# avabag01-ai/spectrogram-midi

Measured on AMD Instinct MI355X. Metric: audio-seconds transcribed/sec (44.1 kHz, n_fft=2048), higher is better.
Workload: dtype f64

## Files before the change

include/aegis_hip.h:

```cpp
#ifndef AEGIS_HIP_H
#define AEGIS_HIP_H

#include <stdint.h>

#ifdef __cplusplus
extern "C" {
#endif

#define AEGIS_ABI_VERSION 2

#define AEGIS_OK 0
#define AEGIS_ERR_INVALID (-22)
#define AEGIS_ERR_NOMEM (-12)
#define AEGIS_ERR_DEVICE (-5)
#define AEGIS_ERR_UNSUPPORTED (-95)

#define AEGIS_STAGE_MEL 0x1
#define AEGIS_STAGE_RAKE 0x2
#define AEGIS_STAGE_PYIN 0x4
#define AEGIS_STAGE_RMS 0x8
#define AEGIS_STAGE_ALL 0xF
#define AEGIS_OPT_CHECK_FINITE 0x10
#define AEGIS_OPT_F0_ZERO 0x20

// ... 101 lines not shown
                             aegis_stream_commit *commit);

#define AEGIS_TREND_SMA 1
#define AEGIS_TREND_EMA 2
#define AEGIS_TREND_BOLLINGER 3
#define AEGIS_TREND_ARTICULATION 4
#define AEGIS_TREND_MACD 5
#define AEGIS_TREND_SLIDES 6
#define AEGIS_TREND_RSI 7
#define AEGIS_TREND_SAVGOL 8
#define AEGIS_TREND_KALMAN 9
#define AEGIS_TREND_HOLT 10
#define AEGIS_TREND_CONSENSUS 11
#define AEGIS_TREND_PITCH_ANALYSIS 12
int aegis_trend(aegis_handle *h, int32_t op, const double *x, const int64_t *offsets, int32_t n_series,
                const double *params, int32_t n_params, void *const *outs, int32_t n_outs);

int aegis_ghost_rsi(aegis_handle *h, const int64_t *ev_a, const int64_t *ev_b, const int64_t *event_off, int32_t n_series,
                    const int64_t *track_len, int32_t period, double *avg_gain, double *avg_loss);

typedef struct aegis_event {
    int32_t clip, note, start, end, velocity;
    uint8_t track;
    uint8_t technique;
    uint8_t reserved0, reserved1;
    float rms_energy;
    int32_t reserved2;
    double confidence, slope;
} aegis_event;
typedef struct aegis_event_params {
    int32_t sample_rate, hop_length;
    double confidence_threshold;
    double sustain_ms, min_note_duration_ms;
} aegis_event_params;
typedef struct aegis_run_fit {
    int32_t clip, start, end;
    int32_t technique;
    double slope;
} aegis_run_fit;
typedef struct aegis_event_batch {
    int32_t n_clips;
    int32_t reserved;
    const int64_t *frame_off;
    const uint8_t *sounding;
    const double *semitones;
    const int16_t *pitch_bin;
    const double *bin_semitones;
    const float *rms_db;
    const double *probs;
    const aegis_run_fit *fits;
    int64_t n_fits;
} aegis_event_batch;
int64_t aegis_extract_events(const aegis_event_params *params, const aegis_event_batch *batch, aegis_event *events, int64_t cap,
                             int64_t *clip_event_off, aegis_run_fit *risky_runs, int64_t risky_cap, int64_t *n_risky);
int64_t aegis_render_smf(int32_t sample_rate, int32_t hop_length, int32_t midi_program, double vibrato_rate,
                         double vibrato_depth, int32_t n_clips, const aegis_event *events, const int64_t *clip_event_off,
                         uint8_t *out, int64_t cap, int64_t *clip_byte_off);
const char *aegis_events_last_error(void);

#define AEGIS_WAVE_SINE 0
#define AEGIS_WAVE_SAWTOOTH 1
#define AEGIS_WAVE_SQUARE 2
#define AEGIS_WAVE_TRIANGLE 3
typedef struct aegis_synth_note {
    double start, duration;
    int32_t note, velocity;
} aegis_synth_note;
typedef struct aegis_adsr_params {
    double attack_ms, decay_ms, sustain_level, release_ms;
    int32_t waveform;
    int32_t reserved;
} aegis_adsr_params;
int64_t aegis_synth_parse_smf(aegis_handle *h, const uint8_t *smf, int64_t n_bytes, aegis_synth_note *notes, int64_t cap,
                              double *length_seconds);
int64_t aegis_synth_samples_for(int32_t sample_rate, double length_seconds, const aegis_adsr_params *params);
int aegis_synth_adsr(aegis_handle *h, int32_t sample_rate, int32_t n_clips, const aegis_synth_note *notes, const int64_t *note_off,
                     const double *length_seconds, const aegis_adsr_params *params, int16_t *const *out, const int64_t *out_cap);

typedef struct aegis_synth_wheel {
    double time;
    int32_t track, value;
} aegis_synth_wheel;
int64_t aegis_synth_parse_smf_wheel(aegis_handle *h, const uint8_t *smf, int64_t n_bytes, aegis_synth_note *notes, int32_t *note_track,
                                    int64_t cap, aegis_synth_wheel *wheel, int64_t wheel_cap, int64_t *n_wheel, double *length_seconds);
int aegis_synth_adsr_bend(aegis_handle *h, int32_t sample_rate, int32_t n_clips, const aegis_synth_note *notes, const int64_t *note_off,
                          const double *length_seconds, const aegis_adsr_params *params, const int32_t *note_track,
                          const aegis_synth_wheel *wheel, const int64_t *wheel_off, const double *bend_range, int16_t *const *out,
                          const int64_t *out_cap);

typedef struct aegis_fit_note {
    int32_t clip, note;
    int64_t lo, hi;
    int32_t velocity, reserved;
    double duration;
} aegis_fit_note;
int aegis_note_fit(aegis_handle *h, int32_t sample_rate, int32_t n_clips, const float *const *audio, const int64_t *n_samples,
                   int32_t n_notes, const aegis_fit_note *notes, const aegis_adsr_params *cands, const int64_t *cand_off,
                   double *score, double *env, double *centroid, double *zcr, int32_t *best);
int aegis_compare_audio(aegis_handle *h, int32_t sample_rate, int32_t n_pairs, const double *const *orig, const int64_t *n_orig,
                        const double *const *synth, const int64_t *n_synth, double *out);
int64_t aegis_synth_one_note(aegis_handle *h, int32_t sample_rate, double freq, double duration, int32_t velocity,
                         const aegis_adsr_params *params, double *out, int64_t cap);
int64_t aegis_synth_notes_samples_for(int32_t sample_rate, double length_seconds, const aegis_adsr_params *params, int64_t n_notes);
int aegis_synth_adsr_notes(aegis_handle *h, int32_t sample_rate, int32_t n_clips, const aegis_synth_note *notes, const int64_t *note_off,
                           const double *length_seconds, const aegis_adsr_params *params, int16_t *const *out, const int64_t *out_cap);

typedef struct aegis_verify_event {
    int32_t clip, reserved;
    int64_t lo, hi;
} aegis_verify_event;
int aegis_verify_techniques(aegis_handle *h, int32_t sample_rate, int32_t n_clips, const float *const *audio,
                            const int64_t *n_samples, int32_t n_events, const aegis_verify_event *events,
                            const aegis_synth_note *notes, const int64_t *note_off, const double *length_seconds,
                            const aegis_adsr_params *params, const int32_t *note_track, const aegis_synth_wheel *wheel,
                            const int64_t *wheel_off, const double *bend_range,
                            double *sim , uint8_t *keep );

typedef struct aegis_salience_params {
    int32_t n_harm;
    double harmonics[8], weights[8];
    int32_t filter_peaks;
    float peak_floor;
    int32_t bin_lo, bin_hi, top_k;
} aegis_salience_params;
int aegis_salience(aegis_handle *h, const float *mag, const int64_t *n_frames, int32_t n_clips, int32_t n_bins, int32_t bins_per_octave,
                   const aegis_salience_params *p, float *sal_out , int32_t *cand_bin, float *cand_sal, float *cand_shift);
int aegis_cqt_salience(aegis_handle *h, const float *const *pcm, const int64_t *n_samples, int32_t n_clips, int32_t n_bins,
                       int32_t bins_per_octave, double fmin, double filter_scale, const aegis_salience_params *p,
                       float *mag_out , float *sal_out , int32_t *cand_bin, float *cand_sal, float *cand_shift);

#define AEGIS_PCM_F64 6
#define AEGIS_FX_DISTORTION 1
#define AEGIS_FX_REVERB     2
#define AEGIS_FX_DELAY      3
#define AEGIS_FX_CHORUS     4
typedef struct aegis_effect { int32_t kind; int32_t n_ir; double p0, p1; const double *ir; } aegis_effect;
int64_t aegis_reverb_ir(double room_size, int32_t sample_rate, double *dst, int64_t cap);
int aegis_effects(aegis_handle *h, int32_t sample_rate, int32_t n_clips, const void *const *in, int32_t in_format,
                  const int64_t *n_samples, const aegis_effect *fx, const int64_t *fx_off,
                  double *const *out_f64, int16_t *const *out_i16);


int64_t aegis_get_table(const aegis_handle *h, const char *name, void *dst, int64_t cap);

int aegis_set_table(aegis_handle *h, const char *name, const double *data, int64_t count);

int64_t aegis_get_param(const aegis_handle *h, const char *name);

int64_t aegis_debug_fetch(aegis_handle *h, const char *name, void *dst, int64_t cap);

int aegis_debug_rake_columns(aegis_handle *h, const float *mel_power, int64_t n_rows, int32_t n_mels, float clip_max,
                             double ratio, int32_t from_power, uint8_t *flags_out);

int aegis_debug_set_observations(aegis_handle *h, const double *logobs, const double *logunv, int64_t F);

int aegis_debug_set_difference(aegis_handle *h, const double *d, int64_t F);

#define AEGIS_PLAN_DEVICE 0
#define AEGIS_PLAN_CALLER_STREAM 1
#define AEGIS_PLAN_HOST_FED 2
#define AEGIS_PLAN_COOLING 4
#define AEGIS_PLAN_NO_PERSIST 8
#define AEGIS_PLAN_F_SPLIT 1
#define AEGIS_PLAN_F_SPLIT_AUTO 2
#define AEGIS_PLAN_F_WANT_HYBRID 4
#define AEGIS_PLAN_F_HYBRID 8
#define AEGIS_PLAN_F_HYBRID_PART 16
#define AEGIS_PLAN_F_BALANCED 32
#define AEGIS_PLAN_F_MAY_PERSIST 64
#define AEGIS_PLAN_F_PERSISTENT 128
#define AEGIS_PLAN_F_DENSE 256
#define AEGIS_PLAN_F_PROPORTIONAL 512
#define AEGIS_PLAN_F_TWO_FRAME_STREAMS 1024
#define AEGIS_PLAN_F_FRAME_B 2048
int64_t aegis_debug_plan(aegis_handle *h, const int64_t *n_samples, int32_t n_clips, int32_t entry, int32_t sync,
                         int32_t n_cus, int64_t *dst, int64_t cap);

int aegis_set_profiling(aegis_handle *h, int32_t on);
double aegis_last_kernel_ms(const aegis_handle *h, const char *name);
int aegis_last_kernel_launches(const aegis_handle *h, const char *name);

#ifdef __cplusplus
}
#endif
#endif
```

spectrogram-midi_amd/_abi.py:

```python
import ctypes as C
import os

import numpy as np

_HERE = os.path.dirname(os.path.abspath(__file__))
LIB_PATH = os.environ.get("AEGIS_HIP_LIB", os.path.join(_HERE, "libaegis_hip.so"))

STAGE_MEL, STAGE_RAKE, STAGE_PYIN, STAGE_RMS, STAGE_ALL = 0x1, 0x2, 0x4, 0x8, 0xF
OPT_CHECK_FINITE, OPT_F0_ZERO = 0x10, 0x20
(TREND_SMA, TREND_EMA, TREND_BOLLINGER, TREND_ARTICULATION, TREND_MACD, TREND_SLIDES, TREND_RSI, TREND_SAVGOL,
 TREND_KALMAN, TREND_HOLT, TREND_CONSENSUS, TREND_PITCH_ANALYSIS) = range(1, 13)
OK, ERR_INVALID, ERR_NOMEM, ERR_DEVICE, ERR_UNSUPPORTED = 0, -22, -12, -5, -95
PYIN_INIT_UNVOICED, PYIN_INIT_UNIFORM = 0, 1
ABI_VERSION = 2
PCM_S16, PCM_F64 = 2, 6
FX_DISTORTION, FX_REVERB, FX_DELAY, FX_CHORUS = 1, 2, 3, 4
EFFECT_KINDS = {"distortion": (FX_DISTORTION, (("drive", 0.5),)), "reverb": (FX_REVERB, (("room_size", 0.5),)),
                "delay": (FX_DELAY, (("delay_ms", 300), ("feedback", 0.3))), "chorus": (FX_CHORUS, (("depth", 0.003), ("rate", 1.5)))}
WAVEFORMS = {"sine": 0, "sawtooth": 1, "square": 2, "triangle": 3}
SYNTH_NOTE_DTYPE = np.dtype([("start", "<f8"), ("duration", "<f8"), ("note", "<i4"), ("velocity", "<i4")])
SYNTH_WHEEL_DTYPE = np.dtype([("time", "<f8"), ("track", "<i4"), ("value", "<i4")])

_P, _S, _I32, _I64, _U32, _F32, _F64 = C.c_void_p, C.c_char_p, C.c_int32, C.c_int64, C.c_uint32, C.c_float, C.c_double
_PP, _PI64 = C.POINTER(_P), C.POINTER(_I64)


class Config(C.Structure):
    _fields_ = [("sample_rate", _I32), ("hop_length", _I32), ("n_fft", _I32), ("n_mels", _I32), ("fmin", _F64), ("fmax", _F64),
                ("device", _I32), ("pyin_init", _I32), ("max_frames_per_pass", _I64)]


class Outputs(C.Structure):
    _fields_ = [("f0", _P), ("voiced_flag", _P), ("voiced_prob", _P), ("rms", _P), ("rake_mask", _P), ("S_dB", _P), ("pitch_bin", _P),
                ("sdb_col_means", _P)]


class PcmClip(C.Structure):
    _fields_ = [("data", _P), ("n_frames", _I64), ("format", _I32), ("channels", _I32), ("sample_rate", _I32), ("n_taps", _I32),
                ("taps", _P)]


class StreamFrames(C.Structure):
    _fields_ = [("rms", _P), ("voiced_prob", _P), ("live_state", _P)]


class StreamCommit(C.Structure):
    _fields_ = [("pitch_bin", _P), ("cap", _I64), ("first", _I64), ("count", _I64), ("frontier", _I64), ("walked", _I64),
                ("walked_wide", _I64)]


class Event(C.Structure):
    _fields_ = [("clip", _I32), ("note", _I32), ("start", _I32), ("end", _I32), ("velocity", _I32),
                ("track", C.c_uint8), ("technique", C.c_uint8), ("reserved0", C.c_uint8), ("reserved1", C.c_uint8),
                ("rms_energy", _F32), ("reserved2", _I32), ("confidence", _F64), ("slope", _F64)]


class EventParams(C.Structure):
    _fields_ = [("sample_rate", _I32), ("hop_length", _I32), ("confidence_threshold", _F64), ("sustain_ms", _F64),
                ("min_note_duration_ms", _F64)]


class RunFit(C.Structure):
    _fields_ = [("clip", _I32), ("start", _I32), ("end", _I32), ("technique", _I32), ("slope", _F64)]


class EventBatch(C.Structure):
    _fields_ = [("n_clips", _I32), ("reserved", _I32), ("frame_off", _P), ("sounding", _P), ("semitones", _P), ("pitch_bin", _P),
                ("bin_semitones", _P), ("rms_db", _P), ("probs", _P), ("fits", _P), ("n_fits", _I64)]


class SynthNote(C.Structure):
    _fields_ = [("start", _F64), ("duration", _F64), ("note", _I32), ("velocity", _I32)]


class AdsrParams(C.Structure):
    _fields_ = [("attack_ms", _F64), ("decay_ms", _F64), ("sustain_level", _F64), ("release_ms", _F64), ("waveform", _I32),
                ("reserved", _I32)]


class FitNote(C.Structure):
    _fields_ = [("clip", _I32), ("note", _I32), ("lo", _I64), ("hi", _I64), ("velocity", _I32), ("reserved", _I32), ("duration", _F64)]


class VerifyEvent(C.Structure):
    _fields_ = [("clip", _I32), ("reserved", _I32), ("lo", _I64), ("hi", _I64)]


class SalienceParams(C.Structure):
    _fields_ = [("n_harm", _I32), ("harmonics", _F64 * 8), ("weights", _F64 * 8), ("filter_peaks", _I32), ("peak_floor", _F32),
                ("bin_lo", _I32), ("bin_hi", _I32), ("top_k", _I32)]


class Effect(C.Structure):
    _fields_ = [("kind", _I32), ("n_ir", _I32), ("p0", _F64), ("p1", _F64), ("ir", _P)]


STRUCTS = {"aegis_config": Config, "aegis_outputs": Outputs, "aegis_pcm_clip": PcmClip, "aegis_stream_frames": StreamFrames,
           "aegis_stream_commit": StreamCommit, "aegis_event": Event, "aegis_event_params": EventParams, "aegis_run_fit": RunFit,
           "aegis_event_batch": EventBatch, "aegis_synth_note": SynthNote, "aegis_adsr_params": AdsrParams,
           "aegis_fit_note": FitNote, "aegis_verify_event": VerifyEvent, "aegis_salience_params": SalienceParams,
           "aegis_effect": Effect}

_OUT, _ADSR, _SAL = C.POINTER(Outputs), C.POINTER(AdsrParams), C.POINTER(SalienceParams)
_FRAMES = C.POINTER(StreamFrames)

PROTOTYPES = {
    "aegis_abi_version": (C.c_int, []),
    "aegis_create": (C.c_int, [C.POINTER(Config), _PP]),
    "aegis_destroy": (None, [_P]),
    "aegis_last_error": (_S, [_P]),
    "aegis_frames_for": (_I64, [_P, _I64]),
    "aegis_analyze_batch": (C.c_int, [_P, _PP, _PI64, _I32, _F64, _U32, _OUT]),
    "aegis_analyze_batch_device": (C.c_int, [_P, _P, _PI64, _I32, _F64, _U32, _OUT, _P, _I32]),
    "aegis_analyze_pcm": (C.c_int, [_P, C.POINTER(PcmClip), _I32, _F64, _U32, _OUT, _P]),
    "aegis_pcm_samples_for": (_I64, [_P, C.POINTER(PcmClip)]),
    "aegis_resample_taps": (_I64, [_I32, _I32, _P, _I64]),
    "aegis_rake_patterns": (C.c_int, [_P, _P, _I32, _I64, _F64, _P]),
    "aegis_cqt": (C.c_int, [_P, _PP, _PI64, _I32, _I32, _I32, _F64, _F64, _P]),
    "aegis_cqt_device": (C.c_int, [_P, _P, _PI64, _I32, _I32, _I32, _F64, _F64, _P, _P, _I32]),
    "aegis_chroma_cqt": (C.c_int, [_P, _PP, _PI64, _I32, _I32, _I32, _F64, _F64, _I32, _P, _P]),
    "aegis_estimate_tuning": (C.c_int, [_P, _PP, _PI64, _I32, _I32, _P, _P, _P]),
    "aegis_stream_open": (C.c_int, [_P, _I64, _PP]),
    "aegis_stream_push": (C.c_int, [_P, _P, _I64, _FRAMES, _PI64]),
    "aegis_stream_close": (C.c_int, [_P, _F64, _OUT, _PI64]),
    "aegis_stream_free": (None, [_P]),
    "aegis_stream_push_commit": (C.c_int, [_P, _P, _I64, _FRAMES, _PI64, C.POINTER(StreamCommit)]),
    "aegis_trend": (C.c_int, [_P, _I32, _P, _P, _I32, _P, _I32, _PP, _I32]),
    "aegis_ghost_rsi": (C.c_int, [_P, _P, _P, _P, _I32, _P, _I32, _P, _P]),
    "aegis_extract_events": (_I64, [C.POINTER(EventParams), C.POINTER(EventBatch), _P, _I64, _P, _P, _I64, _PI64]),
    "aegis_render_smf": (_I64, [_I32, _I32, _I32, _F64, _F64, _I32, _P, _P, _P, _I64, _P]),
    "aegis_events_last_error": (_S, []),
    "aegis_synth_parse_smf": (_I64, [_P, _S, _I64, _P, _I64, C.POINTER(_F64)]),
    "aegis_synth_samples_for": (_I64, [_I32, _F64, _ADSR]),
    "aegis_synth_adsr": (C.c_int, [_P, _I32, _I32, _P, _P, _P, _ADSR, _PP, _P]),
    "aegis_synth_parse_smf_wheel": (_I64, [_P, _S, _I64, _P, _P, _I64, _P, _I64, _PI64, C.POINTER(_F64)]),
    "aegis_synth_adsr_bend": (C.c_int, [_P, _I32, _I32, _P, _P, _P, _ADSR, _P, _P, _P, _P, _PP, _P]),
    "aegis_note_fit": (C.c_int, [_P, _I32, _I32, _PP, _P, _I32, C.POINTER(FitNote), _ADSR, _P, _P, _P, _P, _P, _P]),
    "aegis_compare_audio": (C.c_int, [_P, _I32, _I32, _PP, _P, _PP, _P, _P]),
    "aegis_synth_one_note": (_I64, [_P, _I32, _F64, _F64, _I32, _ADSR, _P, _I64]),
    "aegis_synth_notes_samples_for": (_I64, [_I32, _F64, _ADSR, _I64]),
    "aegis_synth_adsr_notes": (C.c_int, [_P, _I32, _I32, _P, _P, _P, _ADSR, _PP, _P]),
    "aegis_verify_techniques": (C.c_int, [_P, _I32, _I32, _PP, _P, _I32, C.POINTER(VerifyEvent), _P, _P, _P, _ADSR, _P, _P, _P, _P, _P, _P]),
    "aegis_salience": (C.c_int, [_P, _P, _P, _I32, _I32, _I32, _SAL, _P, _P, _P, _P]),
    "aegis_cqt_salience": (C.c_int, [_P, _PP, _PI64, _I32, _I32, _I32, _F64, _F64, _SAL, _P, _P, _P, _P, _P]),
    "aegis_reverb_ir": (_I64, [_F64, _I32, _P, _I64]),
    "aegis_effects": (C.c_int, [_P, _I32, _I32, _PP, _I32, _P, C.POINTER(Effect), _P, _PP, _PP]),
    "aegis_get_table": (_I64, [_P, _S, _P, _I64]),
    "aegis_set_table": (C.c_int, [_P, _S, _P, _I64]),
    "aegis_get_param": (_I64, [_P, _S]),
    "aegis_debug_fetch": (_I64, [_P, _S, _P, _I64]),
    "aegis_debug_rake_columns": (C.c_int, [_P, _P, _I64, _I32, _F32, _F64, _I32, _P]),
    "aegis_debug_set_observations": (C.c_int, [_P, _P, _P, _I64]),
    "aegis_debug_set_difference": (C.c_int, [_P, _P, _I64]),
    "aegis_debug_plan": (_I64, [_P, _PI64, _I32, _I32, _I32, _I32, _P, _I64]),
    "aegis_set_profiling": (C.c_int, [_P, _I32]),
    "aegis_last_kernel_ms": (_F64, [_P, _S]),
    "aegis_last_kernel_launches": (C.c_int, [_P, _S]),
}
EXPORTS = tuple(PROTOTYPES)

_loaded = None


def load():
    global _loaded
    if _loaded is not None:
        return _loaded
    if not os.path.exists(LIB_PATH):
        raise ImportError(
            f"{LIB_PATH} is missing: the HIP extension must be built (make -C {_HERE}/csrc, or "
            "__graft_entry__.build()).  There is no CPU fallback for the analyze path.")
    lib = C.CDLL(LIB_PATH)
    got = int(lib.aegis_abi_version())
    if got != ABI_VERSION:
        raise ImportError(f"{LIB_PATH} has ABI version {got}, this binding was written for {ABI_VERSION} "
                          "(include/aegis_hip.h AEGIS_ABI_VERSION): rebuild the library or update the binding")
    for name, (restype, argtypes) in PROTOTYPES.items():
        fn = getattr(lib, name, None)
        if fn is not None:
            fn.restype = restype
            fn.argtypes = argtypes
    _loaded = lib
    return lib
```

spectrogram-midi_amd/_lib.py:

```python
import atexit
import ctypes as C
import sys
import weakref

import numpy as np

from . import _marshal
from ._abi import *

_PYIN_INIT = {"unvoiced": 0, "uniform": 1, 0: 0, 1: 1}


class AegisError(RuntimeError):
    def __init__(self, code, msg):
        super().__init__(f"libaegis_hip error {code}: {msg}")
        self.code = code


_TABLE_DTYPES = {"mel_dense": np.float32}
_DEBUG_DTYPES = {"persistent_fallbacks": np.int64, "obs_cycles": np.int64, "cqt_cycles": np.int64, "viterbi_cycles": np.int64, "viterbi_spans": np.int64, "split_verify": np.int64, "split_flags": np.int64, "seg_lock": np.int64, "frame_cycles": np.int64, "states": np.int32, "melpow": np.float32, "rake_raw": np.uint8,
                 "tuning_pitch": np.float32, "tuning_mag": np.float32, "tuning_median": np.float32, "tuning_peak_off": np.int64}


_live_handles = weakref.WeakSet()


@atexit.register
def _close_live_handles():
    for h in list(_live_handles):
        try:
            h.close()
        except Exception:
            pass


class Handle:

    def __init__(self, sample_rate=44100, hop_length=512, n_fft=2048, n_mels=128, fmin=0.0, fmax=0.0,
                 device=0, max_frames_per_pass=0, scipy_tables=True, pyin_init="unvoiced"):
        self.lib = load()
        if pyin_init not in _PYIN_INIT:
            raise ValueError("pyin_init must be 'unvoiced' (librosa's p_init) or 'uniform'")
        self.pyin_init = "uniform" if _PYIN_INIT[pyin_init] else "unvoiced"
        cfg = Config(sample_rate, hop_length, n_fft, n_mels, fmin, fmax, device, _PYIN_INIT[pyin_init], max_frames_per_pass)
        h = C.c_void_p()
        rc = self.lib.aegis_create(C.byref(cfg), C.byref(h))
        if rc != OK:
            raise AegisError(rc, self.lib.aegis_last_error(None).decode())
        self._h = h
        _live_handles.add(self)
        self.sr, self.hop, self.n_fft, self.n_mels, self.device = sample_rate, hop_length, n_fft, n_mels, device
        if scipy_tables:
            self._load_scipy_tables()

    def _load_scipy_tables(self):
        import scipy.stats
        thresholds = np.linspace(0, 1, 101)
        self.set_table("beta_probs", np.diff(scipy.stats.beta.cdf(thresholds, 2, 18)))
        n = len(self.table("boltz_fact"))
        lam, idx = 2.0, np.arange(n)
        with np.errstate(divide="ignore", invalid="ignore"):
            fact = (1 - np.exp(-lam)) / (1 - np.exp(-lam * idx))
        fact[0] = 0.0
        self.set_table("boltz_fact", fact)
        self.set_table("boltz_exp", np.exp(-lam * idx))
        fmin, nb = self.table("freqs")[0], self.param("n_pitch_bins")
        self.set_table("freqs", fmin * 2 ** (np.arange(nb) / 120))

    def set_table(self, name, values):
        v = np.ascontiguousarray(values, dtype=np.float64)
        self._check(self.lib.aegis_set_table(self._h, name.encode(), v.ctypes.data, len(v)))

    def close(self):
        if getattr(self, "_h", None):
            h, self._h = self._h, None
            self.lib.aegis_destroy(h)

    def __del__(self):
        if not sys.is_finalizing():
            self.close()

    def _error(self, rc, invalid=None):
        msg = self.lib.aegis_last_error(self._h).decode()
        return invalid(msg) if invalid and rc == ERR_INVALID else AegisError(rc, msg)

    def _check(self, rc, invalid=None):
        if rc != OK:
            raise self._error(rc, invalid)

    def frames_for(self, n_samples):
        return int(self.lib.aegis_frames_for(self._h, int(n_samples)))

    def param(self, name):
        v = int(self.lib.aegis_get_param(self._h, name.encode()))
        if v < 0:
            raise AegisError(v, f"unknown parameter {name}")
        return v

    def table(self, name):
        return _marshal.sized(lambda dst, cap: self.lib.aegis_get_table(self._h, name.encode(), dst, cap),
                              _TABLE_DTYPES.get(name, np.float64), lambda rc: AegisError(rc, f"unknown table {name}"))

    def debug_fetch(self, name):
        return _marshal.sized(lambda dst, cap: self.lib.aegis_debug_fetch(self._h, name.encode(), dst, cap),
                              _DEBUG_DTYPES.get(name, np.float64), self._error)

    def rake_columns(self, mel_power, clip_max, ratio, from_power):
        rows = np.ascontiguousarray(mel_power, dtype=np.float32)
        out = np.empty(rows.shape[0], dtype=np.uint8)
        self._check(self.lib.aegis_debug_rake_columns(self._h, rows.ctypes.data, rows.shape[0], rows.shape[1], float(clip_max),
                                                      float(ratio), int(bool(from_power)), out.ctypes.data))
        return out.astype(bool)

    def set_observations(self, logobs, logunv=None):
        fn = self.lib.aegis_debug_set_observations
        if logobs is None:
            self._check(fn(self._h, None, None, 0))
            return
        rows = np.ascontiguousarray(logobs, dtype=np.float64)
        unv = np.ascontiguousarray(logunv, dtype=np.float64)
        if rows.ndim != 2 or rows.shape[1] != self.param("n_pitch_bins") or unv.shape != (rows.shape[0],):
            raise ValueError("logobs must be [F, n_pitch_bins] and logunv [F]")
        self._check(fn(self._h, rows.ctypes.data, unv.ctypes.data, rows.shape[0]))

    def set_difference(self, d):
        fn = self.lib.aegis_debug_set_difference
        if d is None:
            self._check(fn(self._h, None, 0))
            return
        rows = np.ascontiguousarray(d, dtype=np.float64)
        if rows.ndim != 2 or rows.shape[1] != self.param("max_period") + 1:
            raise ValueError("d must be [F, max_period + 1]")
        self._check(fn(self._h, rows.ctypes.data, rows.shape[0]))

    PLAN_ENTRIES = {"device": 0, "caller_stream": 1, "host_fed": 2}
    PLAN_FLAGS = ("split", "split_auto", "want_hybrid", "hybrid", "hyb_part", "balanced", "may_persist", "persistent",
                  "dense", "proportional", "two_fs", "use_fb")
    PLAN_FIELDS = ("n_clips", "fp", "maxF", "flags", "seglen", "hyb_S", "n_seg", "n_lock", "nk", "ramp_k", "lanes", "hash")

    def plan(self, n_samples, entry="device", sync=1, n_cus=256, cooling=False, persistent=True):
        ns = np.ascontiguousarray(n_samples, dtype=np.int64)
        kind = self.PLAN_ENTRIES[entry] | (4 if cooling else 0) | (0 if persistent else 8)
        args = (self._h, ns.ctypes.data_as(C.POINTER(C.c_int64)), len(ns), kind, int(sync), int(n_cus))
        v = _marshal.sized(lambda dst, cap: self.lib.aegis_debug_plan(*args, dst, cap), np.int64, self._error)
        passes, at = [], 1
        for _ in range(int(v[0])):
            d = {k: int(x) for k, x in zip(self.PLAN_FIELDS, v[at:at + len(self.PLAN_FIELDS)])}
            at += len(self.PLAN_FIELDS)
            d["hash"] &= (1 << 64) - 1
            d.update({f: bool(d["flags"] >> i & 1) for i, f in enumerate(self.PLAN_FLAGS)})
            d["cb"] = [int(x) for x in v[at:at + d["nk"] + 1]]
            at += d["nk"] + 1
            passes.append(d)
        return passes

    def set_profiling(self, on=True):
        self._check(self.lib.aegis_set_profiling(self._h, 1 if on else 0))

    def kernel_ms(self, name):
        return float(self.lib.aegis_last_kernel_ms(self._h, name.encode()))

    def kernel_launches(self, name):
        return int(self.lib.aegis_last_kernel_launches(self._h, name.encode()))

    def viterbi_stats(self, reset=True):
        if self.device < 0:
            return None
        v = np.zeros(3, np.int64)
        n = int(self.lib.aegis_debug_fetch(self._h, b"viterbi_stats" if reset else b"viterbi_stats_peek", v.ctypes.data, 3))
        if n < 0:
            return None
        return {"wave_steps": int(v[0]), "list_only": int(v[1]), "skipped": int(v[2])}

    def analyze_batch(self, clips, rake_sensitivity=0.6, stages=STAGE_ALL, want_sdb=True, check_finite=False,
                      f0_zero=False, views=False, concatenated=False, want_col_means=False):
        clips, ptrs, lens = _marshal.clips(clips, np.float32)
        n = len(clips)
        if n == 0:
            return ([], {}, np.zeros(1, np.int64)) if concatenated else []
        frames = [1 + len(c) // self.hop for c in clips]
        bufs, out, flags = self._outputs(frames, stages, want_sdb, check_finite, f0_zero, concatenated, want_col_means)
        rc = self.lib.aegis_analyze_batch(self._h, ptrs, lens, n, float(rake_sensitivity), flags, C.byref(out))
        self._check_analyze(rc, check_finite)
        return self._split(bufs, frames, views, concatenated)

    def _outputs(self, frames, stages, want_sdb, check_finite, f0_zero, concatenated, want_col_means):
        F = sum(frames)
        if stages & STAGE_RAKE:
            stages |= STAGE_MEL
        bufs = {}
        out = Outputs()
        if stages & STAGE_PYIN:
            bufs["f0"] = np.empty(F, np.float64)
            bufs["voiced_flag"] = np.empty(F, np.uint8)
            bufs["voiced_prob"] = np.empty(F, np.float64)
            if concatenated:
                bufs["pitch_bin"] = np.empty(F, np.int16)
        if stages & STAGE_RMS:
            bufs["rms"] = np.empty(F, np.float32)
        if stages & STAGE_RAKE:
            bufs["rake_mask"] = np.empty(F, np.uint8)
        if (stages & STAGE_MEL) and want_sdb:
            bufs["S_dB"] = np.empty(F * self.n_mels, np.float32)
        if (stages & STAGE_MEL) and want_col_means:
            bufs["sdb_col_means"] = np.empty(3 * F, np.float32)
        for k, v in bufs.items():
            setattr(out, k, v.ctypes.data)
        flags = int(stages) | (OPT_CHECK_FINITE if check_finite else 0) | (OPT_F0_ZERO if f0_zero else 0)
        return bufs, out, flags

    def _check_analyze(self, rc, check_finite):
        if rc == ERR_INVALID and check_finite:
            msg = self.lib.aegis_last_error(self._h).decode()
            if msg.startswith("Audio buffer is not finite"):
                raise ValueError(msg)
        self._check(rc)

    def _split(self, bufs, frames, views, concatenated):
        for k in ("voiced_flag", "rake_mask"):
            if k in bufs:
                bufs[k] = bufs[k].view(bool)
        res, fo = [], 0
        for Fc in frames:
            d = {}
            for k, v in bufs.items():
                if k in ("pitch_bin", "sdb_col_means"):
                    continue
                if k == "S_dB":
                    a = v[fo * self.n_mels:(fo + Fc) * self.n_mels].reshape(self.n_mels, Fc)
                else:
                    a = v[fo:fo + Fc]
                d[k] = a if views else a.copy()
            res.append(d)
            fo += Fc
        if concatenated:
            return res, bufs, _marshal.offsets(frames)
        return res

    def pcm_clips(self, sources, builtin_taps=False):
        from . import audio_io
        arr = (PcmClip * max(len(sources), 1))()
        keep, taps = [], {}
        for i, src in enumerate(sources):
            data = np.ascontiguousarray(src.data, dtype=np.uint8)
            keep.append(data)
            fb = audio_io.PCM_WIDTH[src.format] * src.channels
            c = arr[i]
            c.data, c.n_frames, c.format, c.channels, c.sample_rate = data.ctypes.data, len(data) // fb, src.format, src.channels, src.sample_rate
            if src.sample_rate != self.sr and not builtin_taps:
                if src.sample_rate not in taps:
                    taps[src.sample_rate] = audio_io.resample_taps(src.sample_rate, self.sr)[2]
                h = taps[src.sample_rate]
                c.n_taps, c.taps = len(h), h.ctypes.data
        keep.append(taps)
        return arr, keep

    def pcm_samples_for(self, source):
        arr, keep = self.pcm_clips([source], builtin_taps=True)
        n = int(self.lib.aegis_pcm_samples_for(self._h, arr))
        if n < 0:
            raise AegisError(n, "invalid PCM clip")
        return n

    def analyze_pcm(self, sources, rake_sensitivity=0.6, stages=STAGE_ALL, want_sdb=True, check_finite=False, f0_zero=False,
                    views=False, concatenated=False, want_col_means=False, want_y=True, builtin_taps=False):
# ... 417 lines not shown
```

spectrogram-midi_amd/csrc/aegis_api.hip:

```cpp
#include "aegis_internal.h"

#include <climits>
#include <cmath>
#include <numeric>

#include "pcm.h"

using namespace aegis;

RakeBounds aegis::rake_frame_bounds(const Tables &t) {
    const double ms_per_frame = ((double)t.hop / (double)t.sr) * 1000;
    return {(int)(10 / ms_per_frame), (int)(30 / ms_per_frame)};
}

PassParams aegis::base_params(const Tables &t) {
    PassParams p{};
    p.sr = t.sr; p.hop = t.hop; p.n_mels = t.n_mels;
    p.min_period = t.min_period; p.max_period = t.max_period; p.n_lags = t.n_lags;
    p.n_bins = t.n_bins; p.half_width = t.half_width; p.width = t.width; p.n_cls = t.n_cls;
    p.f0_unvoiced = NAN;
    p.fmin = t.fmin; p.log_tiny = t.log_tiny; p.log_pinit_v = t.log_pinit[0]; p.log_pinit_u = t.log_pinit[1];
    const RakeBounds rb = rake_frame_bounds(t);
    p.rake_min_frames = rb.min_frames; p.rake_max_frames = rb.max_frames;
    return p;
}

int aegis::cmnd_in_frame(const aegis_handle *h) {
    return (!h->cmnd_off && !h->debug_stages && frame_cmnd_supported(h->tab.max_period)) ? 1 : 0;
}
int aegis::troughs_in_frame(const aegis_handle *h) { return (cmnd_in_frame(h) && !h->troughs_off) ? 1 : 0; }

const OutField aegis::kOutFields[8] = {
    {AEGIS_STAGE_PYIN, 8, false, offsetof(aegis_outputs, f0), &aegis_handle::io_f0, &aegis_stream::o_f0},
    {AEGIS_STAGE_PYIN, 1, false, offsetof(aegis_outputs, voiced_flag), &aegis_handle::io_voiced, &aegis_stream::o_voiced},
    {AEGIS_STAGE_MEL, 12, false, offsetof(aegis_outputs, sdb_col_means), &aegis_handle::io_colmean, nullptr},
    {AEGIS_STAGE_PYIN, 2, false, offsetof(aegis_outputs, pitch_bin), &aegis_handle::io_bin, nullptr},
    {AEGIS_STAGE_PYIN, 8, false, offsetof(aegis_outputs, voiced_prob), &aegis_handle::io_vprob, &aegis_stream::o_vprob},
    {AEGIS_STAGE_RMS, 4, false, offsetof(aegis_outputs, rms), &aegis_handle::io_rms, &aegis_stream::o_rms},
    {AEGIS_STAGE_RAKE, 1, false, offsetof(aegis_outputs, rake_mask), &aegis_handle::io_rake, &aegis_stream::o_rake},
    {AEGIS_STAGE_MEL, 4, true, offsetof(aegis_outputs, S_dB), &aegis_handle::io_sdb, &aegis_stream::o_sdb},
};

DevTables aegis::rule_tables(const aegis_handle *h) {
    DevTables dt = h->dt;
    if (h->device < 0 && !h->tab.log_trans_pack.empty()) dt.lt_pack = h->tab.log_trans_pack.data();
    return dt;
}

PlanInput aegis::plan_input(aegis_handle *h, const int64_t *sample_offsets, int32_t n_clips, uint32_t stages, bool feed,
                            bool caller_stream, int32_t sync, int n_cus, std::function<bool(int)> masked) {
    const Tables &t = h->tab;
    PlanInput in;
    in.sample_offsets.assign(sample_offsets, sample_offsets + n_clips + 1);
    in.max_frames_per_pass = h->max_frames_per_pass;
    in.n_cus = n_cus; in.hop = t.hop; in.half_width = t.half_width;
    in.py = stages & AEGIS_STAGE_PYIN;
    in.feed = feed; in.caller_stream = caller_stream; in.sync = sync;
    const DevTables dt = rule_tables(h);
    in.band_applies = viterbi_band_applies(base_params(t), dt);
    in.split_applies = viterbi_split_applies(base_params(t), dt);
    in.masked_streams = std::move(masked);
    in.knobs = h->knobs;
    in.persistent = h->persist.on;
    if (split_allowed(in) && in.knobs.split_seglen < 0 && h->tsplit.cooldown > 0) in.cooling = true;
    return in;
}

static int64_t pcm_width(int32_t fmt) {
    return fmt == AEGIS_PCM_U8 ? 1 : fmt == AEGIS_PCM_S16 ? 2 : fmt == AEGIS_PCM_S24 ? 3 : fmt == AEGIS_PCM_S32 || fmt == AEGIS_PCM_F32 ? 4 : 0;
}

extern "C" {

struct PcmFeed {
    const aegis_pcm_clip *src;
    std::vector<PcmClipDev> clips;
    std::vector<int64_t> done_in;
    std::vector<std::vector<PcmRange>> tables;
    int64_t range_cap = 0, range_used = 0;
    float *y_out = nullptr;
};

struct HostFeed {
    const float *const *pcm;
    float *dst;
    std::vector<int64_t> copied;
    PcmFeed *raw = nullptr;
};

static int pcm_feed(aegis_handle *h, HostFeed &feed, const std::vector<int32_t> &cis, const std::vector<int64_t> &need) {
    PcmFeed &pf = *feed.raw;
    std::vector<PcmRange> tab;
    int64_t tiles = 0;
    for (size_t i = 0; i < cis.size(); ++i) {
        const int ci = cis[i];
        int64_t &done = feed.copied[(size_t)ci];
        if (need[i] <= done) continue;
        const PcmClipDev &c = pf.clips[(size_t)ci];
        const int64_t fb = (int64_t)c.ch * pcm_width(c.fmt);
        const int64_t in_hi = pcm_inputs_needed(c, need[i]);
        int64_t &din = pf.done_in[(size_t)ci];
        if (in_hi > din) {
            HIPCHK(h, hipMemcpyAsync(static_cast<uint8_t *>(h->pcm_raw.p) + c.byte_off + din * fb,
                                     static_cast<const uint8_t *>(pf.src[ci].data) + din * fb, (size_t)((in_hi - din) * fb),
                                     hipMemcpyHostToDevice, h->stream3));
            din = in_hi;
        }
        tab.push_back(PcmRange{done, need[i], tiles, ci, 0});
        tiles += (need[i] - done + c.tile - 1) / c.tile;
        done = need[i];
    }
    if (tab.empty()) return AEGIS_OK;
    if (pf.range_used + (int64_t)tab.size() > pf.range_cap) {
        HIPCHK(h, hipStreamSynchronize(h->stream3));
        pf.range_used = 0;
    }
    PcmRange *d_tab = static_cast<PcmRange *>(h->pcm_ranges.p) + pf.range_used;
    pf.range_used += (int64_t)tab.size();
    pf.tables.push_back(std::move(tab));
    const std::vector<PcmRange> &t = pf.tables.back();
    HIPCHK(h, hipMemcpyAsync(d_tab, t.data(), t.size() * sizeof(PcmRange), hipMemcpyHostToDevice, h->stream3));
    launch_pcm_decode(static_cast<const uint8_t *>(h->pcm_raw.p), static_cast<const PcmClipDev *>(h->pcm_clips.p), d_tab,
                      (int)t.size(), tiles, static_cast<const float *>(h->pcm_taps.p), feed.dst, h->stream3);
    HIPCHK(h, hipGetLastError());
    return AEGIS_OK;
}

static int persistent_check(aegis_handle *h) {
    if (!h->persist.pending) return AEGIS_OK;
    h->persist.pending = false;
    uint32_t aborted = 0;
    HIPCHK(h, hipMemcpy(&aborted, h->abort_flag.p, 4, hipMemcpyDeviceToHost));
    if (aborted) {
        HIPCHK(h, hipMemset(h->abort_flag.p, 0, 4));
        h->err = "the Viterbi kernel gave up waiting for the frame stage (AEGIS_VITERBI_PERSISTENT=0 launches it per chunk)";
        h->persist.gave_up = true;
        return AEGIS_ERR_DEVICE;
    }
    return AEGIS_OK;
}

static int finite_result(aegis_handle *h, uint32_t opts, const int64_t *sample_offsets, int32_t n_clips) {
    if (!(opts & AEGIS_OPT_CHECK_FINITE) || !h->finite_flag.p) return AEGIS_OK;
    unsigned long long bad = ~0ull;
    HIPCHK(h, hipMemcpy(&bad, h->finite_flag.p, 8, hipMemcpyDeviceToHost));
    if (bad == ~0ull) return AEGIS_OK;
    const int64_t idx = sample_offsets[0] + (int64_t)bad;
    int clip = 0;
    while (clip + 1 < n_clips && sample_offsets[clip + 1] <= idx) ++clip;
    h->err = "Audio buffer is not finite everywhere (clip " + std::to_string(clip) + ", sample " + std::to_string(idx - sample_offsets[clip]) + ")";
    return AEGIS_ERR_INVALID;
}

static int split_check(aegis_handle *h, const aegis_handle::SplitCheck &sc, hipStream_t s) {
    const Tables &t = h->tab;
    const PassPlan &m = h->plan.passes[sc.pass];
    const int nc = m.nc();
    std::vector<uint32_t> flags((size_t)nc);
    HIPCHK(h, hipMemcpy(flags.data(), sc.p.clip_flag, (size_t)nc * 4, hipMemcpyDeviceToHost));
    std::vector<int32_t> redo;
    h->tsplit.last_flags.assign(flags.begin(), flags.end());
    for (int i = 0; i < nc; ++i)
        if (flags[i]) { redo.push_back(i); if (flags[i] & 1u) ++h->tsplit.stats[3]; }
    uint32_t counts[2] = {0, 0};
    HIPCHK(h, hipMemcpy(counts, sc.p.tube_count, 8, hipMemcpyDeviceToHost));
    h->tsplit.last_carried_steps = counts[1];
    bool last_split = true;
    for (size_t j = (size_t)sc.pass + 1; j < h->plan.passes.size(); ++j) last_split = last_split && !h->plan.passes[j].tsplit;
    if (m.split_auto && last_split) {
        float ms = 0.f;
        if (hipEventElapsedTime(&ms, h->split_ev[0], h->split_ev[1]) == hipSuccess) {
            h->tsplit.last_viterbi_ms = ms;
            if (!split_clock_pays(h->plan, ms)) { if (++h->tsplit.bad >= 2) { h->tsplit.cooldown = 32; h->tsplit.bad = 0; } }
            else h->tsplit.bad = 0;
        }
    }
    if (redo.empty()) return AEGIS_OK;
    h->tsplit.stats[2] += (int64_t)redo.size();
    if (m.split_auto) {
        int64_t redoF = 0;
        for (int i : redo) redoF = std::max(redoF, m.frames(i));
        if (!split_redo_pays(m, redoF, t.half_width)) h->tsplit.cooldown = 32;
    }
    aegis_handle::Work &w = h->work[sc.pass & 1];
    HIPCHK(h, hipMemcpy(w.flag_order.p, redo.data(), redo.size() * 4, hipMemcpyHostToDevice));
    PassParams q = sc.p;
    q.order = static_cast<const int32_t *>(w.flag_order.p);
    q.n_clips = (int32_t)redo.size();
    q.vt_begin = 0; q.vt_end = INT64_MAX; q.clip_t0 = nullptr; q.clip_t1 = nullptr; q.chunk_flag = nullptr; q.dense = 0;
    hipError_t ve = launch_viterbi(q, h->dt, t.log_trans_band.data(), s);
    if (ve != hipSuccess) { h->err = std::string("viterbi launch: ") + hipGetErrorString(ve); return AEGIS_ERR_DEVICE; }
    launch_decode(sc.p, h->dt, s);
    HIPCHK(h, hipStreamSynchronize(s));
    return AEGIS_OK;
}

static aegis_handle::SplitSet *split_streams(aegis_handle *h, int n_clips) {
    if (!masked_streams_fit(h->knobs, h->n_cus, n_clips)) return nullptr;
    const int idx = n_clips <= 64 ? 0 : 1;
    aegis_handle::SplitSet &ss = h->split[idx];
    if (!ss.tried) {
        ss.tried = true;
        const int v = idx == 0 ? 64 : 128;
        uint32_t fm[8], vm[8];
        for (int w = 0; w < 8; ++w) { fm[w] = 0; vm[w] = 0; }
        for (int i = 0; i < 256; ++i) {
            if (i < 256 - v) fm[i >> 5] |= 1u << (i & 31);
            if (i >= 256 - v) vm[i >> 5] |= 1u << (i & 31);
        }
        if (hipExtStreamCreateWithCUMask(&ss.frame_a, 8, fm) != hipSuccess || hipExtStreamCreateWithCUMask(&ss.frame_b, 8, fm) != hipSuccess ||
            hipExtStreamCreateWithCUMask(&ss.viterbi, 8, vm) != hipSuccess) {
            (void)hipGetLastError();
            for (hipStream_t *q : {&ss.frame_a, &ss.frame_b, &ss.viterbi}) { if (*q) (void)hipStreamDestroy(*q); *q = nullptr; }
        }
    }
    return ss.viterbi ? &ss : nullptr;
}

static int ensure_pass(aegis_handle *h, aegis_handle::Work &w, const PassPlan &m, uint32_t stages) {
    const int64_t nc = m.nc(), nk = m.nk(), fp = m.fp, S = 2 * h->tab.n_bins, nchunks = m.chunk_off[nc];
    int rc;
#define ENS(buf, bytes) if ((rc = ensure(h, w.buf, (size_t)(bytes))) != AEGIS_OK) return rc
    ENS(sample_off, nc * 8); ENS(sample_len, nc * 8); ENS(out_off, nc * 8); ENS(frame_off, (nc + 1) * 8);
    ENS(order, nc * 4); ENS(chunk_off, (nc + 1) * 8); ENS(sel_off, (size_t)nk * (nc + 1) * 8);
    if (stages & AEGIS_STAGE_PYIN) {
        ENS(dfn, fp * h->lag_stride * 8); if (h->debug_stages) ENS(yin, fp * h->yin_stride * 8);
        ENS(logobs, fp * h->obs_stride * 8); ENS(logunv, fp * 8); ENS(obs_seg, fp * 4);
        ENS(ptr, fp * S * 2); ENS(cmap, (nchunks + 1) * S * 2); ENS(bnd, (nchunks + 1) * 4);
        ENS(states, fp * 4); ENS(vstate, (size_t)nc * S * 8);
        ENS(chunk_lo, (size_t)nk * 8); ENS(chunk_flag, (size_t)nk * 4);
        if (m.proportional) ENS(clip_tb, (size_t)(nk + 1) * nc * 8);
        if (m.tsplit) {
            const int64_t n_seg = m.n_seg;
            ENS(seg64, m.seg64.size() * 8); ENS(seg32, m.seg32.size() * 4);
            ENS(seg_col, (size_t)2 * n_seg * S * 8); ENS(seg_map, (size_t)n_seg * S * 2); ENS(seg_i32, ((size_t)n_seg * 3 + 2 * nc) * 4);
            ENS(colhist, (size_t)fp * S * 8); ENS(colG, (size_t)fp * 8); ENS(colkg, (size_t)fp * 4); ENS(clip_flag, (size_t)nc * 4);
            ENS(flag_order, (size_t)nc * 4);
            ENS(tube_buf, (size_t)m.tube_cap * viterbi_tube_record_ints() * 4); ENS(tube_at, (size_t)fp * 4); ENS(tube_count, 8);
        }
    }
    if (stages & AEGIS_STAGE_MEL) { ENS(melpow, fp * h->tab.n_mels * 4); ENS(clipmax, nc * 4); ENS(rake_raw, fp); }
#undef ENS
    return AEGIS_OK;
}

static int upload_pass(aegis_handle *h, aegis_handle::Work &w, const PassPlan &m, uint32_t stages, hipStream_t fa) {
    const size_t nc = m.nc(), nk = m.nk();
    auto up = [&](DevBuf &b, const auto &v) { return hipMemcpyAsync(b.p, v.data(), v.size() * sizeof(v[0]), hipMemcpyHostToDevice, fa); };
    HIPCHK(h, up(w.sample_off, m.sample_off)); HIPCHK(h, up(w.sample_len, m.sample_len)); HIPCHK(h, up(w.out_off, m.out_off));
    HIPCHK(h, up(w.frame_off, m.frame_off)); HIPCHK(h, up(w.chunk_off, m.chunk_off)); HIPCHK(h, up(w.order, m.order));
    HIPCHK(h, up(w.sel_off, m.sel_off));
    if (m.proportional) HIPCHK(h, up(w.clip_tb, m.clip_tb));
    if (stages & AEGIS_STAGE_MEL) HIPCHK(h, hipMemsetAsync(w.clipmax.p, 0, nc * 4, fa));
    if (m.tsplit) {
        HIPCHK(h, up(w.seg64, m.seg64)); HIPCHK(h, up(w.seg32, m.seg32));
        HIPCHK(h, hipMemsetAsync(w.seg_i32.p, 0, ((size_t)m.n_seg * 3 + 2 * nc) * 4, fa));
        HIPCHK(h, hipMemsetAsync(w.clip_flag.p, 0, nc * 4, fa));
        HIPCHK(h, hipMemsetAsync(w.tube_at.p, 0, (size_t)m.fp * 4, fa));
        HIPCHK(h, hipMemsetAsync(w.tube_count.p, 0, 8, fa));
    }
    if (m.persistent) {
        if (!h->abort_flag.p) {
            int rc;
            if ((rc = ensure(h, h->abort_flag, 4)) != AEGIS_OK) return rc;
            HIPCHK(h, hipMemsetAsync(h->abort_flag.p, 0, 4, fa));
        }
        HIPCHK(h, up(w.chunk_lo, m.chunk_lo));
        HIPCHK(h, hipMemsetAsync(w.chunk_flag.p, 0, nk * 4, fa));
    }
    return AEGIS_OK;
}

static PassParams bind_pass(const aegis_handle *h, const PassPlan &m, const aegis_handle::Work &w, const float *d_pcm,
                            uint32_t stages, uint32_t opts, const aegis_outputs *dout, double rake_sensitivity) {
    const Tables &t = h->tab;
    const bool py = stages & AEGIS_STAGE_PYIN, mel = stages & AEGIS_STAGE_MEL;
    const int nc = m.nc(), n_seg = m.n_seg, S = 2 * t.n_bins;
    PassParams p = base_params(t);
    p.stages = stages;
    p.pcm = d_pcm;
    p.sample_off = static_cast<const int64_t *>(w.sample_off.p);
    p.sample_len = static_cast<const int64_t *>(w.sample_len.p);
    p.frame_off = static_cast<const int64_t *>(w.frame_off.p);
    p.out_off = static_cast<const int64_t *>(w.out_off.p);
    p.order = static_cast<const int32_t *>(w.order.p);
    p.n_clips = nc; p.n_frames = m.fp;
    p.dfn = static_cast<double *>(w.dfn.p); p.lag_stride = h->lag_stride;
    p.yin = (py && h->debug_stages) ? static_cast<double *>(w.yin.p) : nullptr; p.yin_stride = h->yin_stride;
    p.cmnd_in_frame = cmnd_in_frame(h); p.troughs = troughs_in_frame(h);
    p.logobs = static_cast<double *>(w.logobs.p); p.obs_stride = h->obs_stride;
    p.logunv = static_cast<double *>(w.logunv.p);
    p.obs_seg = static_cast<int32_t *>(w.obs_seg.p);
    p.ptr = static_cast<uint16_t *>(w.ptr.p);
    p.cmap = static_cast<uint16_t *>(w.cmap.p);
    p.chunk_off = static_cast<int64_t *>(w.chunk_off.p);
    p.bnd = static_cast<int32_t *>(w.bnd.p);
    p.states = static_cast<int32_t *>(w.states.p);
    p.melpow = static_cast<float *>(w.melpow.p);
    p.clipmax = static_cast<uint32_t *>(w.clipmax.p);
    p.rake_raw = static_cast<uint8_t *>(w.rake_raw.p);
    p.vstate = static_cast<double *>(w.vstate.p);
    p.vstats = static_cast<unsigned long long *>(h->vstats.p);
    p.out_f0 = py ? dout->f0 : nullptr;
    p.out_voiced = py ? dout->voiced_flag : nullptr;
    p.out_vprob = py ? dout->voiced_prob : nullptr;
    p.out_bin = py ? dout->pitch_bin : nullptr;
    p.out_rms = (stages & AEGIS_STAGE_RMS) ? dout->rms : nullptr;
    p.out_rake = (stages & AEGIS_STAGE_RAKE) ? dout->rake_mask : nullptr;
    p.out_sdb = mel ? dout->S_dB : nullptr;
    p.out_colmean = mel ? dout->sdb_col_means : nullptr;
    p.out_total = h->plan.total_frames;
    p.rake_ratio = rake_sensitivity;
    if (opts & AEGIS_OPT_F0_ZERO) p.f0_unvoiced = 0.0;
    p.dense = m.dense ? 1 : 0;
    if (m.tsplit) {
        const int64_t *g64 = static_cast<const int64_t *>(w.seg64.p);
        const int32_t *g32 = static_cast<const int32_t *>(w.seg32.p);
        p.seg_f0 = g64; p.seg_ch0 = g64 + n_seg;
        p.vf_off = g64 + 2 * n_seg; p.vf_total = m.seg64.back();
        p.seg_T = g32; p.seg_store = g32 + n_seg; p.seg_prev = g32 + 2 * n_seg; p.seg_clip = g32 + 3 * n_seg;
        p.clip_seg0 = g32 + 4 * n_seg;
        p.seg_col = static_cast<double *>(w.seg_col.p); p.seg_col2 = p.seg_col + (size_t)n_seg * S;
        p.seg_map = static_cast<uint16_t *>(w.seg_map.p);
        p.seg_kg = static_cast<int32_t *>(w.seg_i32.p); p.seg_lock = p.seg_kg + n_seg; p.seg_end = p.seg_kg + 2 * n_seg; p.clip_first = p.seg_kg + 3 * n_seg; p.clip_dirty = p.clip_first + nc;
        p.colhist = static_cast<double *>(w.colhist.p); p.colG = static_cast<double *>(w.colG.p); p.colkg = static_cast<int32_t *>(w.colkg.p);
        p.clip_flag = static_cast<uint32_t *>(w.clip_flag.p);
        p.tube_buf = static_cast<int32_t *>(w.tube_buf.p); p.tube_cap = m.tube_cap; p.tube_count = static_cast<uint32_t *>(w.tube_count.p);
        p.tube_at = static_cast<int32_t *>(w.tube_at.p);
        p.n_seg = n_seg;
    }
    if (m.persistent) {
        p.chunk_flag = static_cast<const uint32_t *>(w.chunk_flag.p);
        p.chunk_lo = static_cast<const int64_t *>(w.chunk_lo.p);
        p.n_chunks = m.nk();
        if (m.hybrid) { int ks = 0; while (ks < m.nk() && m.cb[ks] <= m.hyb_S) ++ks; p.n_chunks = ks; }
        p.abort_flag = static_cast<uint32_t *>(h->abort_flag.p);
        p.wait_ticks = (uint64_t)std::min<int64_t>(150000000, 10000000 + m.fp * 10);
    }
    return p;
}

static hipStream_t lane_stream(const aegis_handle *h, Lane l, hipStream_t s, const aegis_handle::SplitSet *ss) {
    switch (l) {
    case Lane::main: return s;
    case Lane::frame2: return h->stream4;
    case Lane::viterbi2: return h->stream2;
    case Lane::masked_frame_a: return ss->frame_a;
    case Lane::masked_frame_b: return ss->frame_b;
    case Lane::masked_viterbi: return ss->viterbi;
    default: return nullptr;
    }
}

#define VCHK(expr) do { hipError_t ve__ = (expr); if (ve__ != hipSuccess) { h->err = std::string("viterbi launch: ") + hipGetErrorString(ve__); return AEGIS_ERR_DEVICE; } } while (0)

static int analyze_device_locked(aegis_handle *h, const float *d_pcm, const int64_t *sample_offsets,
                                 int32_t n_clips, double rake_sensitivity, uint32_t stages,
                                 aegis_outputs *dout, void *stream_v, int32_t sync, HostFeed *feed = nullptr) {
    if (!h) return AEGIS_ERR_INVALID;
    if (n_clips < 0 || (n_clips > 0 && (!sample_offsets || !dout))) { h->err = "null argument"; return AEGIS_ERR_INVALID; }
    if (n_clips == 0) return AEGIS_OK;
    if (stages & AEGIS_STAGE_RAKE) stages |= AEGIS_STAGE_MEL;
    const uint32_t opts = stages & (AEGIS_OPT_CHECK_FINITE | AEGIS_OPT_F0_ZERO);
    stages &= AEGIS_STAGE_ALL;
    if ((opts & AEGIS_OPT_CHECK_FINITE) && sync == 0) {
        h->err = "AEGIS_OPT_CHECK_FINITE needs sync != 0 (the verdict is reported by the call that synchronises)";
        return AEGIS_ERR_INVALID;
    }
    const Tables &t = h->tab;
    DEVICE_ONLY(h);
    HIPCHK(h, hipSetDevice(h->device));
    hipStream_t s = stream_v ? static_cast<hipStream_t>(stream_v) : h->stream;
    for (int i = 0; i < n_clips; ++i) {
        const int64_t n = sample_offsets[i + 1] - sample_offsets[i];
        if (n < 0) { h->err = "sample_offsets must be non-decreasing"; return AEGIS_ERR_INVALID; }
        if (n > 0 && !d_pcm) { h->err = "d_pcm == NULL"; return AEGIS_ERR_INVALID; }
        if (1 + n / t.hop > h->max_frames_per_pass) {
            h->err = "clip of " + std::to_string(1 + n / t.hop) + " frames exceeds max_frames_per_pass=" +
                     std::to_string(h->max_frames_per_pass);
            return AEGIS_ERR_INVALID;
        }
    }
    if (h->inject.armed) {
        int64_t F = 0;
        for (int i = 0; i < n_clips; ++i) F += 1 + (sample_offsets[i + 1] - sample_offsets[i]) / t.hop;
        if (!(stages & AEGIS_STAGE_PYIN) || F != h->inject.F) {
            h->err = "injected observations: the call needs the PYIN stage and exactly " + std::to_string(h->inject.F) + " frames (it has " +
                     std::to_string(F) + ")";
            return AEGIS_ERR_INVALID;
        }
    }
    if (h->inject_d.armed) {
        int64_t F = 0;
        for (int i = 0; i < n_clips; ++i) F += 1 + (sample_offsets[i + 1] - sample_offsets[i]) / t.hop;
        if (!(stages & AEGIS_STAGE_PYIN) || F != h->inject_d.F) {
            h->err = "injected difference rows: the call needs the PYIN stage and exactly " + std::to_string(h->inject_d.F) + " frames (it has " +
                     std::to_string(F) + ")";
            return AEGIS_ERR_INVALID;
        }
    }
    if (h->plan_in_flight) { HIPCHK(h, hipStreamSynchronize(s)); h->plan_in_flight = false; }
    h->tsplit.checks.clear();
    drop_events(h);

    const PlanInput in = plan_input(h, sample_offsets, n_clips, stages, feed != nullptr, stream_v != nullptr, sync, h->n_cus,
                                    [h](int n) { return split_streams(h, n) != nullptr; });
    if (in.cooling) --h->tsplit.cooldown;
    h->plan = plan_call(in);
    h->plan_in_flight = true;
    const bool py = in.py;

    enum { EV_START = 0, EV_DONE0 = 1, EV_DONE1 = 2, EV_FB = 3, EV_FA = 4, EV_META = 5, EV_CHUNK0 = 6 };
    for (const PassPlan &m : h->plan.passes)
        while ((int)h->sync_events.size() < EV_CHUNK0 + m.nk()) {
            hipEvent_t e;
            const int rc = new_event(h, &e, hipEventDisableTiming);
            if (rc != AEGIS_OK) return rc;
            h->sync_events.push_back(e);
        }
    bool done_recorded[2] = {false, false}, split_started = false;
    std::vector<hipStream_t> joined;
    for (int pi = 0; pi < (int)h->plan.passes.size(); ++pi) {
        const PassPlan &m = h->plan.passes[pi];
        const int nc = m.nc(), nk = m.nk();
        aegis_handle::Work &w = h->work[pi & 1];
        int rc;
        if (!h->tsplit.checks.empty() && h->tsplit.checks.front().pass == pi - 2) {
            HIPCHK(h, hipEventSynchronize(h->sync_events[EV_DONE0 + (pi & 1)]));
            const aegis_handle::SplitCheck sc = h->tsplit.checks.front();
            h->tsplit.checks.erase(h->tsplit.checks.begin());
            if ((rc = split_check(h, sc, s)) != AEGIS_OK) return rc;
        }
        const aegis_handle::SplitSet *ss = m.fa == Lane::masked_frame_a ? split_streams(h, nc) : nullptr;
        hipStream_t fa = lane_stream(h, m.fa, s, ss), fb = lane_stream(h, m.fb, s, ss), sv = lane_stream(h, m.sv, s, ss);
        hipStream_t sd = lane_stream(h, m.sd, s, ss), sa = lane_stream(h, m.sa, s, ss);
        auto join_later = [&](hipStream_t q) { if (q != s && std::find(joined.begin(), joined.end(), q) == joined.end()) joined.push_back(q); };
        if (pi == 0) HIPCHK(h, hipEventRecord(h->sync_events[EV_START], s));
        for (hipStream_t q : {fa, fb, sv, sd, sa}) {
            if (q == s || q == nullptr) continue;
            if (std::find(joined.begin(), joined.end(), q) == joined.end())
                HIPCHK(h, hipStreamWaitEvent(q, h->sync_events[EV_START], 0));
            if (done_recorded[pi & 1]) HIPCHK(h, hipStreamWaitEvent(q, h->sync_events[EV_DONE0 + (pi & 1)], 0));
// ... 387 lines not shown
```

spectrogram-midi_amd/csrc/aegis_handle.hip:

```cpp
#include "aegis_internal.h"
#include "effects.h"

#include <chrono>
#include <cmath>
#include <cstdio>
#include <cstdlib>
#include <new>
#include <stdexcept>
#include <thread>

using namespace aegis;

static std::string g_create_error;

int aegis::grow_buf(aegis_handle *h, std::vector<DevBuf *> &owner, DevBuf &b, size_t bytes) {
    if (h->fail_allocs > 0) {
        --h->fail_allocs;
        h->err = "hipMalloc(" + std::to_string(bytes) + " bytes): out of memory (test hook)";
        return AEGIS_ERR_NOMEM;
    }
    if (b.p) {
        HIPCHK(h, hipDeviceSynchronize());
        HIPCHK(h, hipFree(b.p));
        b.p = nullptr; b.cap = 0;
    }
    if (!b.listed) { owner.push_back(&b); b.listed = true; }
    const size_t want = bytes + bytes / 8 + 256;
    hipError_t e = hipMalloc(&b.p, want);
    if (e != hipSuccess) {
        b.p = nullptr;
        h->err = "hipMalloc(" + std::to_string(want) + " bytes): " + hipGetErrorString(e);
        return AEGIS_ERR_NOMEM;
    }
    b.cap = want;
    return AEGIS_OK;
}

void aegis::free_bufs(std::vector<DevBuf *> &owner) noexcept {
    for (DevBuf *b : owner) {
        if (b->p) (void)hipFree(b->p);
        *b = DevBuf{};
    }
    owner.clear();
}

int aegis::new_event(aegis_handle *h, hipEvent_t *e, unsigned flags) {
    HIPCHK(h, hipEventCreateWithFlags(e, flags));
    h->owned_events.push_back(*e);
    return AEGIS_OK;
}

static int create_events(aegis_handle *h) {
    int rc = new_event(h, &h->copy_event, hipEventDisableTiming);
    h->sync_events.assign(8, nullptr);
    for (hipEvent_t &e : h->sync_events) if (rc == AEGIS_OK) rc = new_event(h, &e, hipEventDisableTiming);
    for (hipEvent_t &e : h->split_ev) if (rc == AEGIS_OK) rc = new_event(h, &e, hipEventDefault);
    for (hipEvent_t &e : h->hyb_ev) if (rc == AEGIS_OK) rc = new_event(h, &e, hipEventDisableTiming);
    for (hipEvent_t &e : h->fin_ev) if (rc == AEGIS_OK) rc = new_event(h, &e, hipEventDisableTiming);
    return rc;
}

template <typename T>
static int upload_table(aegis_handle *h, const std::vector<T> &v, const T **dst) {
    void *d = nullptr;
    const size_t bytes = std::max<size_t>(v.size() * sizeof(T), 16);
    HIPCHK(h, hipMalloc(&d, bytes));
    h->table_allocs.push_back(d);
    if (!v.empty()) HIPCHK(h, hipMemcpy(d, v.data(), v.size() * sizeof(T), hipMemcpyHostToDevice));
    *dst = static_cast<const T *>(d);
    return AEGIS_OK;
}

void aegis::begin_event(aegis_handle *h, const char *name, hipStream_t s) {
    if (!h->profiling) return;
    hipEvent_t a, b;
    if (hipEventCreate(&a) != hipSuccess || hipEventCreate(&b) != hipSuccess) return;
    (void)hipEventRecord(a, s);
    h->events.push_back({name, {a, b}});
}
void aegis::end_event(aegis_handle *h, hipStream_t s) {
    if (!h->profiling || h->events.empty()) return;
    (void)hipEventRecord(h->events.back().second.second, s);
}
void aegis::drop_events(aegis_handle *h) noexcept {
    for (auto &ev : h->events) { (void)hipEventDestroy(ev.second.first); (void)hipEventDestroy(ev.second.second); }
    h->events.clear();
}
void aegis::collect_events(aegis_handle *h) {
    h->last_ms.clear();
    h->last_count.clear();
    double total = 0;
    for (auto &ev : h->events) {
        float ms = 0;
        if (hipEventElapsedTime(&ms, ev.second.first, ev.second.second) == hipSuccess) {
            h->last_ms[ev.first] += ms;
            h->last_count[ev.first] += 1;
            total += ms;
        }
    }
    drop_events(h);
    h->last_ms["total"] = total;
}

int aegis::abi_fail(aegis_handle *h) noexcept {
    int code = AEGIS_ERR_DEVICE;
    const char *msg = "unknown C++ exception";
    std::string what;
    try { throw; }
    catch (const std::bad_alloc &) { code = AEGIS_ERR_NOMEM; msg = "out of host memory"; }
    catch (const std::length_error &) { code = AEGIS_ERR_NOMEM; msg = "request too large for a host container"; }
    catch (const std::exception &e) { try { what = e.what(); msg = what.c_str(); } catch (...) {} }
    catch (...) {}
    try { (h ? h->err : g_create_error) = msg; } catch (...) {}
    return code;
}

static const PassPlan *last_pass(const aegis_handle *h) { return h->plan.passes.empty() ? nullptr : &h->plan.passes.back(); }
static int last_work(const aegis_handle *h) { return h->plan.passes.empty() ? 0 : (int)((h->plan.passes.size() - 1) & 1); }

extern "C" {

int aegis_abi_version(void) { return AEGIS_ABI_VERSION; }

const char *aegis_last_error(const aegis_handle *h) { return h ? h->err.c_str() : g_create_error.c_str(); }

int aegis_create(const aegis_config *cfg, aegis_handle **out) {
    aegis_handle *h = nullptr;
    try {
    if (!out) { g_create_error = "out == NULL"; return AEGIS_ERR_INVALID; }
    *out = nullptr;
    aegis_config c{};
    if (cfg) c = *cfg;
    if (c.sample_rate == 0) c.sample_rate = 44100;
    if (c.hop_length == 0) c.hop_length = 512;
    if (c.n_fft == 0) c.n_fft = 2048;
    if (c.n_mels == 0) c.n_mels = 128;
    if (!(c.fmin > 0)) c.fmin = 82.4068892282175;
    if (!(c.fmax > 0)) c.fmax = 1046.5022612023945;
    const bool auto_pass = c.max_frames_per_pass <= 0;
    if (auto_pass) c.max_frames_per_pass = (int64_t)1 << 21;

    h = new (std::nothrow) aegis_handle();
    if (!h) { g_create_error = "out of host memory"; return AEGIS_ERR_NOMEM; }
    const std::string terr = h->tab.build(c.sample_rate, c.hop_length, c.n_fft, c.n_mels, c.fmin, c.fmax);
    if (!terr.empty()) { g_create_error = terr; delete h; return AEGIS_ERR_INVALID; }
    if (!h->tab.set_pyin_init(c.pyin_init)) { g_create_error = "pyin_init must be AEGIS_PYIN_INIT_UNVOICED (0) or AEGIS_PYIN_INIT_UNIFORM (1)"; delete h; return AEGIS_ERR_INVALID; }
    h->device = c.device;
    h->max_frames_per_pass = c.max_frames_per_pass;
    h->knobs.read_env();
    h->persist.on = h->knobs.persistent_wanted;

    h->lag_stride = (h->tab.max_period + 1 + 7) & ~7;
    h->lag_stride = std::max<int32_t>(h->lag_stride, (trough_row_doubles_host(h->tab.n_lags) + 7) & ~7);
    h->yin_stride = (h->tab.n_lags + 7) & ~7;
    h->obs_stride = (h->tab.n_bins + 7) & ~7;
    if (const char *e = std::getenv("AEGIS_DEBUG_STAGES")) h->debug_stages = (e[0] == '1');
    if (const char *e = std::getenv("AEGIS_CMND_IN_FRAME")) h->cmnd_off = (e[0] == '0');
    if (const char *e = std::getenv("AEGIS_TROUGHS_IN_FRAME")) h->troughs_off = (e[0] == '0');
    if (const char *e = std::getenv("AEGIS_CQT_BANKS")) { const int v = std::atoi(e); if (v >= 1 && v <= 32) h->cqt_bank_cap = v; }
    h->tuning_edges.resize(kTunCells + 1);
    tuning_edges(h->tuning_edges.data());
    if (c.device == -1) { *out = h; return AEGIS_OK; }

    int ndev = 0;
    hipError_t e = hipGetDeviceCount(&ndev);
    if (e != hipSuccess || ndev <= 0) {
        g_create_error = std::string("no HIP device available: ") + hipGetErrorString(e);
        delete h; return AEGIS_ERR_DEVICE;
    }
    if (c.device < 0 || c.device >= ndev) { g_create_error = "device ordinal out of range"; delete h; return AEGIS_ERR_INVALID; }
    auto fail = [&](int code) { g_create_error = h->err; aegis_destroy(h); return code; };
#define CRT(expr) do { int rc__ = (expr); if (rc__ != AEGIS_OK) return fail(rc__); } while (0)
#define CRTHIP(expr) do { hipError_t e__ = (expr); if (e__ != hipSuccess) { h->err = std::string(#expr) + ": " + hipGetErrorString(e__); return fail(AEGIS_ERR_DEVICE); } } while (0)
    CRTHIP(hipSetDevice(c.device));
    CRTHIP(hipStreamCreateWithFlags(&h->stream, hipStreamNonBlocking));
    CRTHIP(hipStreamCreateWithFlags(&h->stream4, hipStreamNonBlocking));
    CRTHIP(hipStreamCreateWithFlags(&h->stream2, hipStreamNonBlocking));
    CRTHIP(hipStreamCreateWithFlags(&h->stream3, hipStreamNonBlocking));
    if (const char *e = std::getenv("AEGIS_NOTEFIT_STORE")) h->notefit_store = (e[0] == '1');
    if (const char *e = std::getenv("AEGIS_TEST_DROP_CHUNK_SIGNAL")) h->test_drop_signal = std::atoi(e);
    CRTHIP(hipDeviceGetAttribute(&h->n_cus, hipDeviceAttributeMultiprocessorCount, c.device));
    if (auto_pass) {
        size_t free_b = 0, total_b = 0;
        if (hipMemGetInfo(&free_b, &total_b) == hipSuccess) {
            const int64_t per_frame = (int64_t)h->lag_stride * 8 + (int64_t)h->obs_stride * 8 + 8 + 2 * h->tab.n_bins * 2 +
                                      2 * h->tab.n_bins * 2 / kViterbiChunk + h->tab.n_mels * 4 + 16;
            const int64_t fit = (int64_t)(free_b / 3) / per_frame;
            h->max_frames_per_pass = std::min<int64_t>((int64_t)1 << 24, std::max<int64_t>((int64_t)1 << 21, fit));
        }
    }
    CRT(create_events(h));
    CRTHIP(configure_lds_limits());
    CRT(ensure(h, h->vstats, 32));
    CRTHIP(hipMemset(h->vstats.p, 0, 32));
    CRTHIP(cqt_configure());

    const Tables &t = h->tab;
    CRT(upload_table(h, t.hann, &h->dt.hann));
    CRT(upload_table(h, t.mel_start, &h->dt.mel_start));
    CRT(upload_table(h, t.mel_len, &h->dt.mel_len));
    CRT(upload_table(h, t.mel_off, &h->dt.mel_off));
    CRT(upload_table(h, t.mel_w, &h->dt.mel_w));
    CRT(upload_table(h, t.mel_chunk_bin, &h->dt.mel_chunk_bin));
    CRT(upload_table(h, t.mel_chunk_w, &h->dt.mel_chunk_w));
    CRT(upload_table(h, t.mel_band_chunk, &h->dt.mel_band_chunk));
    h->dt.mel_chunks = (int32_t)t.mel_chunk_bin.size();
    CRT(upload_table(h, t.thresholds, &h->dt.thresholds));
    CRT(upload_table(h, t.beta_probs, &h->dt.beta_probs));
    CRT(upload_table(h, t.beta_cumsum, &h->dt.beta_cumsum));
    CRT(upload_table(h, t.beta_suffix, &h->dt.beta_suffix));
    CRT(upload_table(h, t.boltz_fact, &h->dt.boltz_fact));
    CRT(upload_table(h, t.boltz_exp, &h->dt.boltz_exp));
    CRT(upload_table(h, t.log_trans_band, &h->dt.lt_band));
    if (!t.log_trans_pack.empty()) CRT(upload_table(h, t.log_trans_pack, &h->dt.lt_pack));
    CRT(upload_table(h, t.freqs, &h->dt.freqs));
    {
        const double *tw = nullptr;
        CRT(upload_table(h, t.twiddle, &tw));
        h->dt.twiddle = reinterpret_cast<const double2 *>(tw);
    }
    CRT(upload_table(h, h->tuning_edges, &h->d_tuning_edges));
#undef CRT
#undef CRTHIP
    *out = h;
    return AEGIS_OK;
    } catch (...) {
        const int code = abi_fail(nullptr);
        if (h) { if (out) *out = nullptr; aegis_destroy(h); }
        return code;
    }
}

void aegis_destroy(aegis_handle *h) {
    if (!h) return;
    {
        std::lock_guard<std::mutex> lock(h->mu);
        if (h->open_streams > 0) { h->destroy_requested = true; return; }
    }
    destroy_now(h);
}

}

void aegis::destroy_now(aegis_handle *h) noexcept {
    if (h->device < 0) { delete h; return; }
    const bool trace = std::getenv("AEGIS_TRACE_DESTROY") != nullptr;
    auto T = [&](const char *what) { if (trace) { std::fprintf(stderr, "[aegis destroy] %s\n", what); std::fflush(stderr); } };
    T("hipSetDevice");
    (void)hipSetDevice(h->device);
    {
        std::vector<hipStream_t> all{h->stream, h->stream2, h->stream3, h->stream4};
        for (auto &ss : h->split) for (hipStream_t q : {ss.frame_a, ss.frame_b, ss.viterbi}) all.push_back(q);
        const auto t0 = std::chrono::steady_clock::now();
        for (;;) {
            bool busy = false;
            for (hipStream_t q : all) if (q && hipStreamQuery(q) == hipErrorNotReady) busy = true;
            if (!busy) break;
            if (std::chrono::steady_clock::now() - t0 > std::chrono::seconds(10)) {
                std::fprintf(stderr, "libaegis_hip: aegis_destroy: work still running on the handle's streams after 10 s; its device memory and streams are leaked\n");
                (void)hipGetLastError();
                delete h;
                return;
            }
            std::this_thread::sleep_for(std::chrono::milliseconds(1));
        }
        (void)hipGetLastError();
    }
    T("device sync");
    (void)hipDeviceSynchronize();
    for (auto &ss : h->split)
        for (hipStream_t q : {ss.frame_a, ss.frame_b, ss.viterbi})
            if (q) { T("destroy masked stream"); (void)hipStreamDestroy(q); }
    T("sync stream"); if (h->stream) (void)hipStreamSynchronize(h->stream);
    T("sync stream2"); if (h->stream2) (void)hipStreamSynchronize(h->stream2);
    T("sync stream3"); if (h->stream3) (void)hipStreamSynchronize(h->stream3);
    T("sync stream4"); if (h->stream4) (void)hipStreamSynchronize(h->stream4);
    T("events");
    drop_events(h);
    for (hipEvent_t e : h->owned_events) (void)hipEventDestroy(e);
    T("free tables");
    for (void *p : h->table_allocs) (void)hipFree(p);
    for (auto &cb : h->cqt_banks) if (cb.bank.dev) (void)hipFree(cb.bank.dev);
    h->cqt_banks.clear();
    T("free workspaces and staging");
    free_bufs(h->bufs);
    T("destroy streams");
    for (hipStream_t q : {h->stream, h->stream2, h->stream3, h->stream4}) if (q) (void)hipStreamDestroy(q);
    T("done");
    delete h;
}

extern "C" {

int64_t aegis_frames_for(const aegis_handle *h, int64_t n_samples) {
    try {
    if (!h || n_samples < 0) return AEGIS_ERR_INVALID;
    return 1 + n_samples / h->tab.hop;
    } catch (...) { return abi_fail(const_cast<aegis_handle *>(h)); }
}

int aegis_set_profiling(aegis_handle *h, int32_t on) {
    try {
    if (!h) return AEGIS_ERR_INVALID;
    h->profiling = on != 0;
    return AEGIS_OK;
    } catch (...) { return abi_fail(h); }
}

int aegis_last_kernel_launches(const aegis_handle *h, const char *name) {
    if (!h || !name) return -1;
    auto it = h->last_count.find(name);
    return it == h->last_count.end() ? 0 : it->second;
}

double aegis_last_kernel_ms(const aegis_handle *h, const char *name) {
    if (!h || !name) return -1.0;
    auto it = h->last_ms.find(name);
    return it == h->last_ms.end() ? -1.0 : it->second;
}

int aegis_set_table(aegis_handle *h, const char *name, const double *data, int64_t count) {
    try {
    if (!h || !name || !data) return AEGIS_ERR_INVALID;
    Tables &t = h->tab;
    const std::string n(name);
    struct Slot { std::vector<double> *host; const double *dev; };
    auto slot = [&](const std::string &nm) -> Slot {
        if (nm == "beta_probs") return {&t.beta_probs, h->dt.beta_probs};
        if (nm == "beta_cumsum") return {&t.beta_cumsum, h->dt.beta_cumsum};
        if (nm == "beta_suffix") return {&t.beta_suffix, h->dt.beta_suffix};
        if (nm == "boltz_fact") return {&t.boltz_fact, h->dt.boltz_fact};
        if (nm == "boltz_exp") return {&t.boltz_exp, h->dt.boltz_exp};
        if (nm == "freqs") return {&t.freqs, h->dt.freqs};
        return {nullptr, nullptr};
    };
    auto push = [&](const std::string &nm) -> int {
        Slot s = slot(nm);
        if (h->device < 0) return AEGIS_OK;
        HIPCHK(h, hipSetDevice(h->device));
        HIPCHK(h, hipStreamSynchronize(h->stream));
        HIPCHK(h, hipMemcpy(const_cast<double *>(s.dev), s.host->data(), s.host->size() * 8, hipMemcpyHostToDevice));
        return AEGIS_OK;
    };
    Slot s = slot(n);
    if (!s.host || n == "beta_cumsum" || n == "beta_suffix") { h->err = "unknown or derived table: " + n; return AEGIS_ERR_INVALID; }
    if (count != (int64_t)s.host->size()) {
        h->err = "table " + n + " needs " + std::to_string(s.host->size()) + " entries";
        return AEGIS_ERR_INVALID;
    }
    std::copy(data, data + count, s.host->begin());
    int rc = push(n);
    if (rc != AEGIS_OK) return rc;
    if (n == "beta_probs") {
        for (int k = 0; k <= kNThresholds; ++k) t.beta_cumsum[k] = np_pairwise_sum(t.beta_probs.data(), k);
        t.beta_suffix.assign(kNThresholds + 1, 0.0);
        for (int k = kNThresholds - 1; k >= 0; --k) t.beta_suffix[k] = t.beta_suffix[k + 1] + t.beta_probs[k];
        if ((rc = push("beta_cumsum")) != AEGIS_OK) return rc;
        if ((rc = push("beta_suffix")) != AEGIS_OK) return rc;
    }
    return AEGIS_OK;
    } catch (...) { return abi_fail(h); }
}

int64_t aegis_get_param(const aegis_handle *h, const char *name) {
    try {
    if (!h || !name) return AEGIS_ERR_INVALID;
    const Tables &t = h->tab;
    const std::string n(name);
    if (n == "min_period") return t.min_period;
    if (n == "max_period") return t.max_period;
    if (n == "n_lags") return t.n_lags;
    if (n == "n_pitch_bins") return t.n_bins;
    if (n == "transition_width") return t.width;
    if (n == "n_trans_classes") return t.n_cls;
    if (n == "max_frames_per_pass") return h->max_frames_per_pass;
    if (n == "lag_stride") return h->lag_stride;
    if (n == "yin_stride") return h->yin_stride;
    if (n == "obs_stride") return h->obs_stride;
    const PassPlan *lp = last_pass(h);
    if (n == "last_frames") return lp ? lp->fp : 0;
    if (n == "last_passes") return (int64_t)h->plan.passes.size();
    if (n == "last_split_segments") { int64_t v = 0; for (const PassPlan &q : h->plan.passes) v += q.tsplit ? q.n_seg : 0; return v; }
    if (n == "split_passes") return h->tsplit.stats[0];
    if (n == "split_segments") return h->tsplit.stats[1];
    if (n == "split_flagged_clips") return h->tsplit.stats[2];
    if (n == "split_unlocked_clips") return h->tsplit.stats[3];
    if (n == "split_rounds") return h->tsplit.last_carried_steps;
    if (n == "split_viterbi_us") return (int64_t)(h->tsplit.last_viterbi_ms * 1e3);
    if (n == "split_cooldown") return h->tsplit.cooldown;
    if (n == "last_chunks") return lp ? lp->nk() : 0;
    if (n == "last_dense") return lp ? lp->dense : 0;
    if (n == "last_proportional") return lp ? lp->proportional : 0;
    if (n == "last_balanced") return lp ? lp->balanced : 0;
    if (n == "last_hybrid_step") return lp ? lp->hyb_S : 0;
    if (n == "last_persistent") return lp ? lp->persistent : 0;
    if (n == "pyin_init") return t.pyin_init;
    if (n == "cqt_bank_builds") return h->cqt_bank_builds;
    if (n == "cqt_banks") return (int64_t)h->cqt_banks.size();
    if (n == "cqt_bank_cap") return h->cqt_bank_cap;
    if (n == "cqt_bank_bytes") return h->cqt_bank_bytes;
    if (n == "cqt_bank_build_us") return h->cqt_bank_build_us;
    if (n == "cmnd_in_frame") return cmnd_in_frame(h);
    if (n == "troughs_in_frame") return troughs_in_frame(h);
    if (n == "frame_fpw") return frame_batch_fpw(t.max_period);
    if (n == "obs_waves") { PassParams q = base_params(t); q.n_sel = 4096; return pyin_obs_waves(q); }
    if (n == "viterbi_kernel") { const int k = viterbi_kernel_choice(base_params(t), rule_tables(h)); return k < 0 ? AEGIS_ERR_UNSUPPORTED : k; }
    if (n == "split_applies") return viterbi_split_applies(base_params(t), rule_tables(h)) ? 1 : 0;
    if (n == "fx_tile") return kFxRevTile;
    if (n == "fx_chunk") return kFxChunk;
    if (n == "fx_max_taps") return kFxMaxTaps;
    return AEGIS_ERR_INVALID;
    } catch (...) { return abi_fail(const_cast<aegis_handle *>(h)); }
}

int64_t aegis_get_table(const aegis_handle *h, const char *name, void *dst, int64_t cap) {
    try {
    if (!h || !name) return AEGIS_ERR_INVALID;
    const Tables &t = h->tab;
    const std::string n(name);
    const void *src = nullptr;
    int64_t count = 0;
    size_t esz = 8;
    auto setd = [&](const std::vector<double> &v) { src = v.data(); count = (int64_t)v.size(); esz = 8; };
    if (n == "hann") setd(t.hann);
    else if (n == "thresholds") setd(t.thresholds);
    else if (n == "beta_probs") setd(t.beta_probs);
    else if (n == "beta_cumsum") setd(t.beta_cumsum);
    else if (n == "beta_suffix") setd(t.beta_suffix);
    else if (n == "boltz_fact") setd(t.boltz_fact);
    else if (n == "boltz_exp") setd(t.boltz_exp);
    else if (n == "log_trans_band") setd(t.log_trans_band);
    else if (n == "log_trans_pack") setd(t.log_trans_pack);
    else if (n == "freqs") setd(t.freqs);
    else if (n == "twiddle") setd(t.twiddle);
    else if (n == "tuning_edges") setd(h->tuning_edges);
    else if (n == "mel_dense") { src = t.mel_dense.data(); count = (int64_t)t.mel_dense.size(); esz = 4; }
    else return AEGIS_ERR_INVALID;
    if (dst && cap > 0) std::memcpy(dst, src, (size_t)std::min(count, cap) * esz);
    return count;
    } catch (...) { return abi_fail(const_cast<aegis_handle *>(h)); }
}

int64_t aegis_debug_plan(aegis_handle *h, const int64_t *n_samples, int32_t n_clips, int32_t entry, int32_t sync,
                         int32_t n_cus, int64_t *dst, int64_t cap) {
    try {
    if (!h || n_clips < 0 || (n_clips > 0 && !n_samples) || cap < 0 || (cap > 0 && !dst)) return AEGIS_ERR_INVALID;
    std::lock_guard<std::mutex> lock(h->mu);
    std::vector<int64_t> off((size_t)n_clips + 1, 0);
    for (int i = 0; i < n_clips; ++i) {
        if (n_samples[i] < 0 || 1 + n_samples[i] / h->tab.hop > h->max_frames_per_pass) { h->err = "bad clip " + std::to_string(i); return AEGIS_ERR_INVALID; }
        off[i + 1] = off[i] + n_samples[i];
    }
    const int kind = entry & 3;
    const PlanKnobs &kn = h->knobs;
    PlanInput in = plan_input(h, off.data(), n_clips, AEGIS_STAGE_ALL, kind == AEGIS_PLAN_HOST_FED, kind == AEGIS_PLAN_CALLER_STREAM,
                              sync, n_cus, [&kn, n_cus](int n) { return masked_streams_fit(kn, n_cus, n); });
    if (entry & AEGIS_PLAN_COOLING) in.cooling = split_allowed(in) && kn.split_seglen < 0;
    if (entry & AEGIS_PLAN_NO_PERSIST) in.persistent = false;
    const CallPlan c = plan_call(in);
    std::vector<int64_t> v{(int64_t)c.passes.size()};
    for (const PassPlan &m : c.passes) {
        const int64_t flags = m.tsplit * AEGIS_PLAN_F_SPLIT | m.split_auto * AEGIS_PLAN_F_SPLIT_AUTO | m.want_hybrid * AEGIS_PLAN_F_WANT_HYBRID |
                              m.hybrid * AEGIS_PLAN_F_HYBRID | m.hyb_part * AEGIS_PLAN_F_HYBRID_PART | m.balanced * AEGIS_PLAN_F_BALANCED |
                              m.may_persist * AEGIS_PLAN_F_MAY_PERSIST | m.persistent * AEGIS_PLAN_F_PERSISTENT | m.dense * AEGIS_PLAN_F_DENSE |
                              m.proportional * AEGIS_PLAN_F_PROPORTIONAL | m.two_fs * AEGIS_PLAN_F_TWO_FRAME_STREAMS | m.use_fb * AEGIS_PLAN_F_FRAME_B;
        const int64_t lanes = (int64_t)m.fa | (int64_t)m.fb << 4 | (int64_t)m.sv << 8 | (int64_t)m.sd << 12 | (int64_t)m.sa << 16;
        uint64_t hash = 1469598103934665603ull;
        auto mix = [&hash](const void *p, size_t n) {
            for (size_t i = 0; i < n; ++i) { hash ^= static_cast<const unsigned char *>(p)[i]; hash *= 1099511628211ull; }
        };
        auto table = [&mix](const auto &t) { const uint64_t n = t.size(); mix(&n, 8); mix(t.data(), n * sizeof(t[0])); };
        table(m.seg32); table(m.seg64); table(m.sel_off); table(m.clip_tb);
        for (int64_t x : {(int64_t)m.nc(), m.fp, m.maxF, flags, m.seglen, m.hyb_S, (int64_t)m.n_seg, (int64_t)m.n_lock, (int64_t)m.nk(),
                          (int64_t)m.ramp_k, lanes, (int64_t)hash}) v.push_back(x);
        v.insert(v.end(), m.cb.begin(), m.cb.end());
    }
    if (cap > 0) std::memcpy(dst, v.data(), (size_t)std::min<int64_t>(cap, (int64_t)v.size()) * 8);
    return (int64_t)v.size();
    } catch (...) { return abi_fail(h); }
}

struct Counter { const char *name; int count; hipError_t (*fetch)(long long *); bool always_sync; };
static const Counter kCounters[] = {
    {"obs_cycles", 16, obs_debug_fetch, false},
    {"frame_cycles", 24, frame_debug_fetch, false},
    {"split_verify", 16, [](long long *v) { return viterbi_verify_fetch(v, true); }, false},
    {"viterbi_cycles", 128, [](long long *v) { return viterbi_debug_fetch(v, true); }, false},
    {"viterbi_spans", 272, viterbi_span_fetch, false},
    {"cqt_cycles", 16, cqt_debug_fetch, true},
};

int64_t aegis_debug_fetch(aegis_handle *h, const char *name, void *dst, int64_t cap) {
    try {
    if (!h || !name) return AEGIS_ERR_INVALID;
    const std::string n(name);
    if (n == "throw_bad_alloc") throw std::bad_alloc();
    if (n == "throw_length_error") throw std::length_error("test hook");
    if (n == "throw_runtime_error") throw std::runtime_error("test hook: runtime_error");
    if (n == "throw_int") throw 42;
    if (n == "fail_allocs") { h->fail_allocs = (int)std::max<int64_t>(0, cap); return 0; }
    for (const Counter &c : kCounters) {
        if (n != c.name) continue;
        if (h->device < 0) return AEGIS_ERR_INVALID;
        if (c.always_sync || (dst && cap > 0)) {
            long long v[272];
            HIPCHK(h, hipSetDevice(h->device));
            HIPCHK(h, hipDeviceSynchronize());
            HIPCHK(h, c.fetch(v));
            if (dst && cap > 0) std::memcpy(dst, v, (size_t)std::min<int64_t>(cap, c.count) * 8);
        }
        return c.count;
    }
    const PassPlan *lp = last_pass(h);
    const int64_t F = lp ? lp->fp : 0;
    const int last_pass_segments = lp && lp->tsplit ? lp->n_seg : 0;
    const void *src = nullptr;
    int64_t count = 0;
    size_t esz = 8;
    const aegis_handle::Work &lw = h->work[last_work(h)];
    if (n == "dfn") { src = lw.dfn.p; count = F * h->lag_stride; }
    else if (n == "yin") { src = lw.yin.p; count = F * h->yin_stride; }
    else if (n == "logobs") {
        count = F * h->obs_stride;
        if (h->device < 0 || !lw.logobs.p || !lw.obs_seg.p) { h->err = "stage was not run"; return AEGIS_ERR_INVALID; }
        if (dst && cap > 0) {
            HIPCHK(h, hipSetDevice(h->device));
            HIPCHK(h, hipStreamSynchronize(h->stream));
            std::vector<double> rows((size_t)count);
            std::vector<int32_t> seg((size_t)F);
            HIPCHK(h, hipMemcpy(rows.data(), lw.logobs.p, (size_t)count * 8, hipMemcpyDeviceToHost));
            HIPCHK(h, hipMemcpy(seg.data(), lw.obs_seg.p, (size_t)F * 4, hipMemcpyDeviceToHost));
            const double log_tiny = h->tab.log_tiny;
            for (int64_t f = 0; f < F; ++f)
                for (int b = 0; b < h->obs_stride; ++b)
                    if (!(seg[(size_t)f] & (0x40000000 | (1 << (b >> 6))))) rows[(size_t)(f * h->obs_stride + b)] = log_tiny;
            std::memcpy(dst, rows.data(), (size_t)std::min(count, cap) * 8);
        }
        return count;
    }
    else if (n == "logunv") { src = lw.logunv.p; count = F; }
    else if (n == "states") { src = lw.states.p; count = F; esz = 4; }
    else if (n == "melpow") { src = lw.melpow.p; count = F * h->tab.n_mels; esz = 4; }
    else if (n == "rake_raw") { src = lw.rake_raw.p; count = F; esz = 1; }
    else if (n == "tuning_peak_off") {
        const std::vector<int64_t> &po = h->tn_last_peak_off;
        if (dst && cap > 0) std::memcpy(dst, po.data(), (size_t)std::min<int64_t>(cap, (int64_t)po.size()) * 8);
        return (int64_t)po.size();
    }
    else if (n == "tuning_pitch" || n == "tuning_mag" || n == "tuning_median") {
        if (h->tn_last_peak_off.empty()) return 0;
        if (n == "tuning_median") { src = h->tn_median.p; count = (int64_t)h->tn_last_peak_off.size() - 1; }
        else { src = n == "tuning_pitch" ? h->tn_pitch.p : h->tn_mag.p; count = h->tn_last_peak_off.back(); }
        esz = 4;
    }
    else if (n == "persistent_fallbacks") {
        if (dst && cap > 0) *static_cast<int64_t *>(dst) = h->persist.fallbacks;
        return 1;
    }
    else if (n == "viterbi_stats" || n == "viterbi_stats_peek") {
        if (h->device < 0 || !h->vstats.p) return AEGIS_ERR_INVALID;
        if (dst && cap > 0) {
            long long v[3];
            std::lock_guard<std::mutex> lock(h->mu);
            HIPCHK(h, hipSetDevice(h->device));
            HIPCHK(h, hipDeviceSynchronize());
            HIPCHK(h, hipMemcpy(v, h->vstats.p, 24, hipMemcpyDeviceToHost));
            if (n == "viterbi_stats") HIPCHK(h, hipMemset(h->vstats.p, 0, 24));
            std::memcpy(dst, v, (size_t)std::min<int64_t>(cap, 3) * 8);
        }
        return 3;
    }
    else if (n == "seg_lock") {
        if (h->device < 0 || last_pass_segments <= 0) return 0;
        const int ns = last_pass_segments;
        if (dst && cap > 0) {
            std::vector<int32_t> v((size_t)ns), st((size_t)ns);
            HIPCHK(h, hipSetDevice(h->device));
            HIPCHK(h, hipDeviceSynchronize());
            HIPCHK(h, hipMemcpy(v.data(), static_cast<const int32_t *>(lw.seg_i32.p) + ns, (size_t)ns * 4, hipMemcpyDeviceToHost));
            HIPCHK(h, hipMemcpy(st.data(), static_cast<const int32_t *>(lw.seg32.p) + ns, (size_t)ns * 4, hipMemcpyDeviceToHost));
            int64_t *o = static_cast<int64_t *>(dst);
            for (int i = 0; i < std::min<int64_t>(cap, ns); ++i) o[i] = v[i] > 0 ? v[i] - st[i] : v[i];
        }
        return ns;
    }
    else if (n == "split_flags") {
        if (dst && cap > 0) std::memcpy(dst, h->tsplit.last_flags.data(), (size_t)std::min<int64_t>(cap, (int64_t)h->tsplit.last_flags.size()) * 8);
        return (int64_t)h->tsplit.last_flags.size();
    }
    else return AEGIS_ERR_INVALID;
    if (h->device < 0 || !src) { h->err = "stage was not run"; return AEGIS_ERR_INVALID; }
    if (dst && cap > 0) {
        HIPCHK(h, hipSetDevice(h->device));
        HIPCHK(h, hipStreamSynchronize(h->stream));
        HIPCHK(h, hipMemcpy(dst, src, (size_t)std::min(count, cap) * esz, hipMemcpyDeviceToHost));
    }
    return count;
    } catch (...) { return abi_fail(h); }
}

int aegis_debug_rake_columns(aegis_handle *h, const float *mel_power, int64_t n_rows, int32_t n_mels, float clip_max,
                             double ratio, int32_t from_power, uint8_t *flags_out) {
    try {
    if (!h) return AEGIS_ERR_INVALID;
    if (n_rows < 0 || n_mels <= 0 || n_mels > 128 || (n_rows > 0 && (!mel_power || !flags_out))) { h->err = "bad argument"; return AEGIS_ERR_INVALID; }
    if (n_rows == 0) return AEGIS_OK;
    DEVICE_ONLY(h);
    std::lock_guard<std::mutex> lock(h->mu);
    HIPCHK(h, hipSetDevice(h->device));
    int rc;
    const size_t bytes = (size_t)n_rows * n_mels * 4;
    if ((rc = ensure(h, h->io_sdb, bytes)) != AEGIS_OK) return rc;
    if ((rc = ensure(h, h->rk_raw, n_rows)) != AEGIS_OK) return rc;
    if ((rc = ensure(h, h->io_rake, 32)) != AEGIS_OK) return rc;
    hipStream_t s = h->stream;
    struct { int64_t frame_off[2]; uint32_t clipmax; } geo = {{0, n_rows}, 0};
    std::memcpy(&geo.clipmax, &clip_max, 4);
    HIPCHK(h, hipMemcpyAsync(h->io_sdb.p, mel_power, bytes, hipMemcpyHostToDevice, s));
    HIPCHK(h, hipMemcpyAsync(h->io_rake.p, &geo, sizeof geo, hipMemcpyHostToDevice, s));
    PassParams p{};
    p.n_mels = n_mels; p.n_clips = 1; p.n_frames = n_rows; p.stages = AEGIS_STAGE_MEL;
    p.frame_off = static_cast<const int64_t *>(h->io_rake.p);
    p.clipmax = reinterpret_cast<uint32_t *>(static_cast<char *>(h->io_rake.p) + 16);
    p.melpow = static_cast<float *>(h->io_sdb.p);
    p.rake_raw = static_cast<uint8_t *>(h->rk_raw.p);
    p.rake_ratio = ratio;
    launch_rake_columns(p, from_power != 0, s);
    HIPCHK(h, hipGetLastError());
    HIPCHK(h, hipMemcpyAsync(flags_out, h->rk_raw.p, n_rows, hipMemcpyDeviceToHost, s));
    HIPCHK(h, hipStreamSynchronize(s));
    return AEGIS_OK;
    } catch (...) { return abi_fail(h); }
}

int aegis_debug_set_observations(aegis_handle *h, const double *logobs, const double *logunv, int64_t F) {
    try {
    if (!h) return AEGIS_ERR_INVALID;
    std::lock_guard<std::mutex> lock(h->mu);
    h->inject.armed = false;
    if (!logobs) return AEGIS_OK;
    if (!logunv || F <= 0) { h->err = "bad argument"; return AEGIS_ERR_INVALID; }
    if (h->inject_d.armed) { h->err = "injected observations: injected difference rows are armed already (one hook per call)"; return AEGIS_ERR_INVALID; }
    const int B = h->tab.n_bins;
    const double log_tiny = h->tab.log_tiny, easy_min = std::log(std::ldexp(1.0, -53) / B);
    auto reject = [&](int64_t f, const char *why) {
        h->err = "injected observations, frame " + std::to_string(f) + ": " + why;
        return AEGIS_ERR_INVALID;
    };
    for (int64_t f = 0; f < F; ++f) {
        const double u = logunv[f];
        const bool hard = u == log_tiny;
        if (u != u) return reject(f, "logunv is NaN");
        if (!hard && !(u >= easy_min && u <= 0.0)) return reject(f, "logunv must be log(tiny) or within [log(2^-53 / n_pitch_bins), 0]");
        const double *row = logobs + f * B;
        bool observed = false;
        for (int b = 0; b < B; ++b) {
            if (row[b] != row[b]) return reject(f, "logobs is NaN");
            if (!(row[b] >= log_tiny && row[b] <= 0.0)) return reject(f, "logobs must be within [log(tiny), 0]");
            observed = observed || row[b] != log_tiny;
        }
        if (hard && !observed) return reject(f, "a hard frame (logunv == log(tiny)) needs a bin above log(tiny)");
    }
    DEVICE_ONLY(h);
    HIPCHK(h, hipSetDevice(h->device));
    HIPCHK(h, hipDeviceSynchronize());
    int rc;
    if ((rc = ensure(h, h->inject.obs, (size_t)F * B * 8)) != AEGIS_OK) return rc;
    if ((rc = ensure(h, h->inject.unv, (size_t)F * 8)) != AEGIS_OK) return rc;
    HIPCHK(h, hipMemcpy(h->inject.obs.p, logobs, (size_t)F * B * 8, hipMemcpyHostToDevice));
    HIPCHK(h, hipMemcpy(h->inject.unv.p, logunv, (size_t)F * 8, hipMemcpyHostToDevice));
    h->inject.F = F;
    h->inject.armed = true;
    return AEGIS_OK;
    } catch (...) { return abi_fail(h); }
}

int aegis_debug_set_difference(aegis_handle *h, const double *d, int64_t F) {
    try {
    if (!h) return AEGIS_ERR_INVALID;
    std::lock_guard<std::mutex> lock(h->mu);
    h->inject_d.armed = false;
    if (!d) return AEGIS_OK;
    if (F <= 0) { h->err = "bad argument"; return AEGIS_ERR_INVALID; }
    if (h->inject.armed) { h->err = "injected difference rows: injected observations are armed already (one hook per call)"; return AEGIS_ERR_INVALID; }
    const int64_t W = (int64_t)h->tab.max_period + 1;
    for (int64_t f = 0; f < F; ++f)
        for (int64_t tau = 0; tau < W; ++tau)
            if (!std::isfinite(d[f * W + tau])) {
                h->err = "injected difference rows, frame " + std::to_string(f) + ": d[" + std::to_string(tau) + "] is not finite";
                return AEGIS_ERR_INVALID;
            }
    DEVICE_ONLY(h);
    HIPCHK(h, hipSetDevice(h->device));
    HIPCHK(h, hipDeviceSynchronize());
    int rc;
    if ((rc = ensure(h, h->inject_d.d, (size_t)F * W * 8)) != AEGIS_OK) return rc;
    HIPCHK(h, hipMemcpy(h->inject_d.d.p, d, (size_t)F * W * 8, hipMemcpyHostToDevice));
    h->inject_d.F = F;
    h->inject_d.armed = true;
    return AEGIS_OK;
    } catch (...) { return abi_fail(h); }
}

}
```

spectrogram-midi_amd/csrc/aegis_internal.h:

```cpp
#pragma once
#include <hip/hip_runtime.h>

#include <algorithm>
#include <cstdint>
#include <cstring>
#include <functional>
#include <list>
#include <map>
#include <mutex>
#include <string>
#include <vector>

#include "../../include/aegis_hip.h"
#include "kernels.h"
#include "plan.h"
#include "cqt.h"
#include "tables.h"
#include "tuning.h"

struct DevBuf {
    void *p = nullptr;
    size_t cap = 0;
    bool listed = false;
};

struct aegis_handle {
    aegis::Tables tab;
    aegis::DevTables dt{};
    int device = 0;
    hipStream_t stream = nullptr;
    hipStream_t stream2 = nullptr;
    bool troughs_off = false;
    bool cmnd_off = false;
    bool debug_stages = false;
    hipStream_t stream4 = nullptr;
    hipStream_t stream3 = nullptr;
    struct SplitSet { hipStream_t frame_a = nullptr, frame_b = nullptr, viterbi = nullptr; bool tried = false; } split[2];
    int n_cus = 0;
    std::vector<hipEvent_t> owned_events;
    hipEvent_t copy_event = nullptr;
    std::vector<hipEvent_t> sync_events;
    hipEvent_t split_ev[2] = {nullptr, nullptr};
    hipEvent_t hyb_ev[3] = {nullptr, nullptr, nullptr};
    hipEvent_t fin_ev[2] = {nullptr, nullptr};
    int64_t max_frames_per_pass = 0;
    int fail_allocs = 0;
    mutable std::string err;
    std::vector<void *> table_allocs;
    std::vector<DevBuf *> bufs;
    struct Work {
        DevBuf dfn, yin, logobs, logunv, obs_seg, ptr, cmap, chunk_off, bnd, states, melpow, clipmax, rake_raw;
        DevBuf sample_off, sample_len, out_off, frame_off, order, sel_off, vstate, chunk_lo, chunk_flag, clip_tb;
        DevBuf seg64, seg32, seg_col, seg_map, seg_i32, colhist, colG, colkg, clip_flag, flag_order, tube_buf, tube_at, tube_count;
    } work[2];
    DevBuf vstats, rk_raw, abort_flag, finite_flag;
    struct Inject { bool armed = false; int64_t F = 0; DevBuf obs, unv; } inject;
    struct InjectD { bool armed = false; int64_t F = 0; DevBuf d; } inject_d;
    uint32_t chunk_gen = 0;
    int test_drop_signal = -1;
    struct Persistent {
        bool on = true;
        bool pending = false;
        bool gave_up = false;
        int cooldown = 0;
        int64_t fallbacks = 0;
    } persist;
    struct SplitCheck { int pass; aegis::PassParams p; };
    struct TimeSplit {
        std::vector<SplitCheck> checks;
        int bad = 0;
        int cooldown = 0;
        int64_t stats[4] = {0, 0, 0, 0};
        double last_viterbi_ms = 0.0;
        int64_t last_carried_steps = 0;
        std::vector<int64_t> last_flags;
    } tsplit;
    aegis::PlanKnobs knobs;
    struct CachedBank { aegis::CqtBank bank; size_t bytes = 0; };
    std::list<CachedBank> cqt_banks;
    int cqt_bank_cap = 8;
    int64_t cqt_bank_builds = 0;
    int64_t cqt_bank_bytes = 0, cqt_bank_build_us = 0;
    DevBuf q_pcm, q_soff, q_foff, q_toff, q_out, q_chroma, q_cls;
    std::vector<double> tuning_edges;
    const double *d_tuning_edges = nullptr;
    DevBuf tn_meta, tn_pitch, tn_mag, tn_count, tn_median, tn_cells, tn_tuning;
    std::vector<int64_t> tn_last_peak_off;
    DevBuf t_x, t_off, t_a, t_b, t_c, t_d, t_e, t_i8, t_i64a, t_i64b;
    DevBuf t_pa;
    DevBuf io_pcm, io_f0, io_voiced, io_vprob, io_rms, io_rake, io_sdb, io_bin, io_colmean;
    DevBuf pcm_raw, pcm_clips, pcm_ranges, pcm_taps;
    DevBuf sy_oscs, sy_notes, sy_tiles, sy_tile_notes, sy_osc_peak, sy_clip_peak, sy_mix, sy_out;
    DevBuf sy_bends, sy_segs;
    DevBuf fx_a, fx_b, fx_recs, fx_tiles, fx_peak, fx_taps, fx_i16;
    DevBuf nf_audio, nf_oscs, nf_cands, nf_notes, nf_boff, nf_peak, nf_cnum, nf_cden, nf_zc, nf_rms, nf_out, nf_best;
    DevBuf nf_sig, nf_sigoff, nf_cands2;
    DevBuf vf_audio, vf_events, vf_boff, vf_mel, vf_max, vf_sim, vf_keep;
    struct VerifyBank { aegis::MelBank host; int32_t n_used = 0; bool uploaded = false; DevBuf start, len, off, w; };
    std::map<int32_t, VerifyBank> vf_banks;
    DevBuf sl_mag, sl_foff, sl_img, sl_bin, sl_sal, sl_shift;
    bool notefit_store = false;
    int32_t lag_stride = 0, yin_stride = 0, obs_stride = 0;
    aegis::CallPlan plan;
    bool plan_in_flight = false;
    bool profiling = false;
    std::vector<std::pair<std::string, std::pair<hipEvent_t, hipEvent_t>>> events;
    std::map<std::string, double> last_ms;
    std::map<std::string, int> last_count;
    std::mutex mu;
    int open_streams = 0;
    bool destroy_requested = false;
};

struct aegis_stream {
    aegis_handle *h = nullptr;
    int64_t cap_samples = 0, cap_frames = 0;
    int64_t n_samples = 0;
    int64_t frames_done = 0;
    bool closed = false;
    std::vector<DevBuf *> bufs;
    DevBuf pcm, dfn, logobs, logunv, obs_seg, ptr, cmap, bnd, states, live, melpow, clipmax, rake_raw, vstate, meta;
    DevBuf o_f0, o_voiced, o_vprob, o_rms, o_rake, o_sdb;
    std::vector<int64_t> host_meta;
    DevBuf ctl, g_staging, g_result;
    float *pin_samples = nullptr;
    unsigned char *pin_result = nullptr;
    hipGraph_t graph[2] = {nullptr, nullptr};
    hipGraphExec_t graph_exec[2] = {nullptr, nullptr};
    int64_t graph_push[2] = {0, 0};
    bool graph_failed = false;
    DevBuf c_bins, c_result;
    unsigned char *pin_commit = nullptr;
    unsigned char commit_host[aegis::kCommitResultBytes] = {};
    int64_t c_frontier = -1;
    int64_t c_newest = -1;
    int64_t c_delivered = 0;
    int64_t c_walked = 0, c_walked_wide = 0;
};

#define HIPCHK(h, expr)                                                                         \
    do {                                                                                        \
        hipError_t e__ = (expr);                                                                \
        if (e__ != hipSuccess) {                                                                \
            (h)->err = std::string(#expr) + ": " + hipGetErrorString(e__);                      \
            return AEGIS_ERR_DEVICE;                                                            \
        }                                                                                       \
    } while (0)
#define HIPCHK_SYNC(h, s, expr)                                                                 \
    do {                                                                                        \
        hipError_t e__ = (expr);                                                                \
        if (e__ != hipSuccess) {                                                                \
            (h)->err = std::string(#expr) + ": " + hipGetErrorString(e__);                      \
            (void)hipStreamSynchronize(s);                                                      \
            return AEGIS_ERR_DEVICE;                                                            \
        }                                                                                       \
    } while (0)
#define ENSURE(h, buf, bytes)                                                                               \
    do {                                                                                                    \
        const int rc__ = aegis::ensure(h, (h)->buf, std::max<size_t>((size_t)(bytes), 8));                 \
        if (rc__ != AEGIS_OK) return rc__;                                                                  \
    } while (0)
#define DEVICE_ONLY(h) \
    do { if ((h)->device < 0) { (h)->err = "handle was created with device=-1 (host tables only)"; return AEGIS_ERR_DEVICE; } } while (0)

namespace aegis {

int grow_buf(aegis_handle *h, std::vector<DevBuf *> &owner, DevBuf &b, size_t bytes);
inline int ensure(aegis_handle *h, DevBuf &b, size_t bytes) { return bytes <= b.cap ? AEGIS_OK : grow_buf(h, h->bufs, b, bytes); }
inline int ensure(aegis_stream *st, DevBuf &b, size_t bytes) { return bytes <= b.cap ? AEGIS_OK : grow_buf(st->h, st->bufs, b, bytes); }
inline hipError_t upload(DevBuf &b, const void *src, size_t bytes, hipStream_t s) {
    return bytes ? hipMemcpyAsync(b.p, src, bytes, hipMemcpyHostToDevice, s) : hipSuccess;
}
void free_bufs(std::vector<DevBuf *> &owner) noexcept;
int new_event(aegis_handle *h, hipEvent_t *e, unsigned flags);
void destroy_now(aegis_handle *h) noexcept;
int abi_fail(aegis_handle *h) noexcept;

void begin_event(aegis_handle *h, const char *name, hipStream_t s);
void end_event(aegis_handle *h, hipStream_t s);
void drop_events(aegis_handle *h) noexcept;
void collect_events(aegis_handle *h);

template <class F>
int run_halving(aegis_handle *h, int32_t n, F &&group) {
    int32_t size = n;
    for (int32_t i0 = 0; i0 < n;) {
        const int32_t i1 = std::min(n, i0 + size);
        const int rc = group(i0, i1);
        if (rc == AEGIS_ERR_NOMEM && size > 1) {
            (void)hipDeviceSynchronize();
            (void)hipGetLastError();
            size = (size + 1) / 2;
            continue;
        }
        if (rc != AEGIS_OK) { drop_events(h); return rc; }
        i0 = i1;
    }
    return AEGIS_OK;
}

struct AdsrBatch;
int check_bend_request(aegis_handle *h, int32_t sample_rate, int32_t n_clips, const aegis_synth_note *notes, const int64_t *note_off,
                       const double *length_seconds, const aegis_adsr_params *params, const int32_t *note_track,
                       const aegis_synth_wheel *wheel, const int64_t *wheel_off, const double *bend_range, int16_t *const *out,
                       const int64_t *out_cap);
int fill_bend_batch(aegis_handle *h, int32_t sr, int32_t c0, int32_t c1, const aegis_synth_note *notes, const int64_t *note_off,
                    const double *length_seconds, const aegis_adsr_params *params, const int32_t *note_track,
                    const aegis_synth_wheel *wheel, const int64_t *wheel_off, const double *bend_range, AdsrBatch &B);
// ... 29 lines not shown
```

spectrogram-midi_amd/csrc/aegis_stream.hip:

```cpp
#include "aegis_internal.h"

#include <cstdlib>
#include <new>

using namespace aegis;

extern "C" {

static PassParams stream_params(aegis_stream *st, const int64_t *dm) {
    aegis_handle *h = st->h;
    const Tables &t = h->tab;
    PassParams p = base_params(t);
    p.stages = AEGIS_STAGE_ALL;
    p.pcm = static_cast<const float *>(st->pcm.p);
    p.sample_off = dm; p.sample_len = dm + 1; p.frame_off = dm + 2; p.out_off = dm + 2; p.sel_off = dm + 4;
    p.chunk_off = const_cast<int64_t *>(dm + 6);
    p.order = reinterpret_cast<const int32_t *>(dm + 8);
    p.n_clips = 1;
    p.dfn = static_cast<double *>(st->dfn.p); p.lag_stride = h->lag_stride;
    p.yin = nullptr; p.yin_stride = h->yin_stride;
    p.cmnd_in_frame = cmnd_in_frame(h); p.troughs = troughs_in_frame(h);
    p.logobs = static_cast<double *>(st->logobs.p); p.obs_stride = h->obs_stride;
    p.logunv = static_cast<double *>(st->logunv.p);
    p.obs_seg = static_cast<int32_t *>(st->obs_seg.p);
    p.ptr = static_cast<uint16_t *>(st->ptr.p); p.cmap = static_cast<uint16_t *>(st->cmap.p);
    p.bnd = static_cast<int32_t *>(st->bnd.p); p.states = static_cast<int32_t *>(st->states.p);
    p.live_states = static_cast<int32_t *>(st->live.p);
    p.melpow = static_cast<float *>(st->melpow.p); p.clipmax = static_cast<uint32_t *>(st->clipmax.p);
    p.rake_raw = static_cast<uint8_t *>(st->rake_raw.p);
    p.vstate = static_cast<double *>(st->vstate.p);
    p.out_vprob = static_cast<double *>(st->o_vprob.p);
    p.out_rms = static_cast<float *>(st->o_rms.p);
    p.out_f0 = static_cast<double *>(st->o_f0.p); p.out_voiced = static_cast<uint8_t *>(st->o_voiced.p);
    p.out_rake = static_cast<uint8_t *>(st->o_rake.p); p.out_sdb = static_cast<float *>(st->o_sdb.p);
    p.rake_ratio = 0.6;
    return p;
}

static StreamCommitCtl *stream_commit_ctl(aegis_stream *st) {
    return reinterpret_cast<StreamCommitCtl *>(static_cast<unsigned char *>(st->ctl.p) + sizeof(StreamCtl));
}

static bool stream_build_graph(aegis_stream *st, int64_t n_push, hipStream_t s, int commit) {
    aegis_handle *h = st->h;
    const Tables &t = h->tab;
    if (!st->pin_samples || !st->pin_result || (commit && !st->pin_commit) || n_push > 8192 || n_push % t.hop != 0 || n_push / t.hop + 1 > 8) return false;
    StreamCtl *ctl = static_cast<StreamCtl *>(st->ctl.p);
    PassParams p = stream_params(st, ctl->meta);
    p.ctl = ctl;
    p.n_frames = st->cap_frames;
    p.n_sel = n_push / t.hop + 1;
    if (hipStreamBeginCapture(s, hipStreamCaptureModeThreadLocal) != hipSuccess) return false;
    bool ok = true;
    ok &= hipMemcpyAsync(st->g_staging.p, st->pin_samples, n_push * 4, hipMemcpyHostToDevice, s) == hipSuccess;
    launch_stream_advance(ctl, static_cast<const float *>(st->g_staging.p), (int)n_push, static_cast<float *>(st->pcm.p), t.hop, s);
    launch_frame(p, h->dt, s);
    launch_pyin_obs(p, h->dt, s);
    ok &= launch_viterbi(p, h->dt, t.log_trans_band.data(), s) == hipSuccess;
    if (commit)
        ok &= launch_stream_commit(ctl, 0, stream_commit_ctl(st), p.ptr, p.vstate, t.n_bins, static_cast<int16_t *>(st->c_bins.p),
                                   st->c_result.p, s) == hipSuccess;
    launch_stream_gather(ctl, p.out_rms, p.out_vprob, p.live_states, st->g_result.p, s);
    ok &= hipMemcpyAsync(st->pin_result, st->g_result.p, 256, hipMemcpyDeviceToHost, s) == hipSuccess;
    if (commit) ok &= hipMemcpyAsync(st->pin_commit, st->c_result.p, kCommitResultBytes, hipMemcpyDeviceToHost, s) == hipSuccess;
    hipGraph_t g = nullptr;
    ok &= hipStreamEndCapture(s, &g) == hipSuccess && g != nullptr;
    if (!ok) { if (g) (void)hipGraphDestroy(g); (void)hipGetLastError(); return false; }
    hipGraphExec_t ex = nullptr;
    if (hipGraphInstantiate(&ex, g, nullptr, nullptr, 0) != hipSuccess) { (void)hipGraphDestroy(g); (void)hipGetLastError(); return false; }
    st->graph[commit] = g; st->graph_exec[commit] = ex; st->graph_push[commit] = n_push;
    return true;
}

static int stream_run(aegis_stream *st, int64_t f_lo, int64_t f_hi, bool final_pass, hipStream_t s) {
    aegis_handle *h = st->h;
    const Tables &t = h->tab;
    const int S = 2 * t.n_bins;
    const int64_t Ftot = final_pass ? f_hi : st->cap_frames;
    st->host_meta.assign(9, 0);
    st->host_meta[1] = st->n_samples;
    st->host_meta[3] = Ftot;
    st->host_meta[5] = f_hi - f_lo;
    st->host_meta[7] = (Ftot - 1 + kViterbiChunk - 1) / kViterbiChunk;
    HIPCHK(h, hipMemcpyAsync(st->meta.p, st->host_meta.data(), 9 * 8, hipMemcpyHostToDevice, s));
    const int64_t *dm = static_cast<const int64_t *>(st->meta.p);
    PassParams p = stream_params(st, dm);
    p.n_frames = Ftot;
    p.t_begin = f_lo; p.n_sel = f_hi - f_lo;
    p.vt_begin = f_lo; p.vt_end = final_pass ? INT64_MAX : f_hi;
    (void)S;
    if (p.n_sel > 0) {
        launch_frame(p, h->dt, s);
        launch_pyin_obs(p, h->dt, s);
    }
    if (p.n_sel > 0 || final_pass) {
        hipError_t ve = launch_viterbi(p, h->dt, t.log_trans_band.data(), s);
        if (ve != hipSuccess) { h->err = std::string("viterbi launch: ") + hipGetErrorString(ve); return AEGIS_ERR_DEVICE; }
    }
    HIPCHK(h, hipGetLastError());
    return AEGIS_OK;
}

static void stream_release(aegis_stream *st) noexcept {
    if (st->h && st->h->device >= 0) { (void)hipSetDevice(st->h->device); (void)hipStreamSynchronize(st->h->stream); }
    for (int k = 0; k < 2; ++k) {
        if (st->graph_exec[k]) (void)hipGraphExecDestroy(st->graph_exec[k]);
        if (st->graph[k]) (void)hipGraphDestroy(st->graph[k]);
    }
    if (st->pin_samples) (void)hipHostFree(st->pin_samples);
    if (st->pin_result) (void)hipHostFree(st->pin_result);
    if (st->pin_commit) (void)hipHostFree(st->pin_commit);
    free_bufs(st->bufs);
    delete st;
}

static int stream_open_locked(aegis_handle *h, int64_t max_samples, aegis_stream *st) {
    HIPCHK(h, hipSetDevice(h->device));
    st->h = h;
    const Tables &t = h->tab;
    st->cap_samples = max_samples;
    st->cap_frames = 1 + max_samples / t.hop;
    const int64_t F = st->cap_frames, S = 2 * t.n_bins;
    const int64_t nch = (F - 1 + kViterbiChunk - 1) / kViterbiChunk + 1;
    int rc = AEGIS_OK;
    auto need = [&](DevBuf &b, size_t bytes) { if (rc == AEGIS_OK) rc = ensure(st, b, bytes); };
    need(st->pcm, max_samples * 4); need(st->dfn, F * h->lag_stride * 8);
    need(st->logobs, F * h->obs_stride * 8); need(st->logunv, F * 8); need(st->obs_seg, F * 4); need(st->ptr, F * S * 2);
    need(st->cmap, nch * S * 2); need(st->bnd, nch * 4); need(st->states, F * 4); need(st->live, F * 4);
    need(st->melpow, F * t.n_mels * 4); need(st->clipmax, 16); need(st->rake_raw, F); need(st->vstate, S * 8);
    need(st->meta, 9 * 8); need(st->ctl, sizeof(StreamCtl) + sizeof(StreamCommitCtl)); need(st->g_staging, 8192 * 4); need(st->g_result, 256);
    need(st->c_bins, F * 2); need(st->c_result, kCommitResultBytes);
    need(st->o_f0, F * 8); need(st->o_voiced, F); need(st->o_vprob, F * 8); need(st->o_rms, F * 4); need(st->o_rake, F);
    need(st->o_sdb, F * t.n_mels * 4);
    if (rc != AEGIS_OK) return rc;
    HIPCHK(h, hipMemsetAsync(st->clipmax.p, 0, 16, h->stream));
    HIPCHK(h, hipMemsetAsync(st->ptr.p, 0, (size_t)F * S * 2, h->stream));
    {
        struct { StreamCtl ctl; StreamCommitCtl commit; } c0{};
        static_assert(sizeof(c0) == sizeof(StreamCtl) + sizeof(StreamCommitCtl), "the commit block sits right behind the control block");
        c0.ctl.meta[3] = st->cap_frames;
        c0.ctl.meta[7] = (st->cap_frames - 1 + kViterbiChunk - 1) / kViterbiChunk;
        c0.commit.frontier = -1; c0.commit.newest = -1;
        HIPCHK(h, hipMemcpyAsync(st->ctl.p, &c0, sizeof(c0), hipMemcpyHostToDevice, h->stream));
    }
    HIPCHK(h, hipStreamSynchronize(h->stream));
    if (hipHostMalloc(reinterpret_cast<void **>(&st->pin_samples), 8192 * 4, hipHostMallocDefault) != hipSuccess) st->pin_samples = nullptr;
    if (hipHostMalloc(reinterpret_cast<void **>(&st->pin_result), 256, hipHostMallocDefault) != hipSuccess) st->pin_result = nullptr;
    if (hipHostMalloc(reinterpret_cast<void **>(&st->pin_commit), kCommitResultBytes, hipHostMallocDefault) != hipSuccess) st->pin_commit = nullptr;
    if (const char *e = std::getenv("AEGIS_STREAM_GRAPH")) st->graph_failed = (e[0] == '0');
    else {
        const char *tool = std::getenv("ROCP_TOOL_LIBRARIES"), *pre = std::getenv("LD_PRELOAD");
        if ((tool && tool[0]) || (pre && std::strstr(pre, "rocprofiler"))) st->graph_failed = true;
    }
    return AEGIS_OK;
}

int aegis_stream_open(aegis_handle *h, int64_t max_samples, aegis_stream **out) {
    aegis_stream *st = nullptr;
    try {
    if (!h || !out || max_samples <= 0) { if (h) h->err = "bad argument"; return AEGIS_ERR_INVALID; }
    *out = nullptr;
    DEVICE_ONLY(h);
    std::lock_guard<std::mutex> lock(h->mu);
    if (h->destroy_requested) { h->err = "handle was destroyed"; return AEGIS_ERR_INVALID; }
    st = new (std::nothrow) aegis_stream();
    if (!st) { h->err = "out of host memory"; return AEGIS_ERR_NOMEM; }
    const int rc = stream_open_locked(h, max_samples, st);
    if (rc != AEGIS_OK) { stream_release(st); st = nullptr; return rc; }
    ++h->open_streams;
    *out = st;
    return AEGIS_OK;
    } catch (...) {
        const int code = abi_fail(h);
        if (st) stream_release(st);
// ... 181 lines not shown
```

spectrogram-midi_amd/csrc/kernels.h:

```cpp
#pragma once
#include <hip/hip_runtime.h>

#include <cstdint>

#include "plan.h"

namespace aegis {

struct DevTables {
    const double *hann;
    const int32_t *mel_start;
    const int32_t *mel_len;
    const int32_t *mel_off;
    const float *mel_w;
    const int32_t *mel_chunk_bin;
    const float *mel_chunk_w;
    const int32_t *mel_band_chunk;
    int32_t mel_chunks;
    const double *thresholds;
    const double *beta_probs;
    const double *beta_cumsum;
    const double *beta_suffix;
    const double *boltz_fact;
    const double *boltz_exp;
    const double *lt_band;
    const double *lt_pack;
    const double *freqs;
    const double2 *twiddle;
};

struct StreamCtl {
    int64_t n_samples;
    int64_t frames_done;
    int64_t t_begin, n_sel;
    int64_t vt_begin, vt_end;
    int64_t meta[9];
};

struct StreamCommitCtl {
    int64_t frontier;
    int64_t newest;
};
constexpr int kCommitStage = 240;
constexpr int kCommitResultBytes = 32 + 2 * kCommitStage;

struct PassParams {
    int32_t sr, hop, n_mels;
    int32_t min_period, max_period, n_lags;
    int32_t n_bins, half_width, width, n_cls;
    double fmin;
    double log_tiny;
    double log_pinit_v, log_pinit_u;
    uint32_t stages;
    const float *pcm;
    const int64_t *sample_off;
    const int64_t *sample_len;
    const int64_t *frame_off;
    const int64_t *out_off;
    const int32_t *order;
    int32_t n_clips;
    int64_t n_frames;
    const int64_t *sel_off;
    int64_t t_begin;
    const int64_t *clip_t0, *clip_t1;
    int32_t dense;
    int64_t n_sel;
    int64_t vt_begin, vt_end;
    double *vstate;
    int32_t *live_states;
    const StreamCtl *ctl;
    unsigned long long *vstats;
    const uint32_t *chunk_flag;
    const int64_t *chunk_lo;
    int32_t n_chunks;
    uint32_t chunk_gen;
    uint32_t *abort_flag;
    uint64_t wait_ticks;
    const int64_t *seg_f0;
    const int32_t *seg_T;
    const int64_t *seg_ch0;
    const int32_t *seg_store;
    const int32_t *seg_prev;
    const int32_t *seg_clip;
    const int32_t *clip_seg0;
    double *seg_col;
    double *seg_col2;
    int32_t *clip_first;
    int32_t *clip_dirty;
    const int64_t *vf_off;
    int64_t vf_total;
    int32_t clip_sel;
    int32_t *seg_kg;
    int32_t *seg_lock;
    int32_t *seg_end;
    uint16_t *seg_map;
    double *colhist;
    double *colG; int32_t *colkg;
    int32_t *tube_buf; int32_t tube_cap; uint32_t *tube_count;
    int32_t *tube_at;
    uint32_t *clip_flag;
    int32_t split_phase;
    int32_t n_seg;
    int32_t split_hybrid;
    int32_t hybrid_step;
    double *dfn;   int32_t lag_stride;
    int32_t cmnd_in_frame;
    int32_t troughs;
    double *yin;   int32_t yin_stride;
    double *logobs; int32_t obs_stride;
    double *logunv;
    int32_t *obs_seg;
    uint16_t *ptr;
    uint16_t *cmap;
    int64_t *chunk_off;
    int32_t *bnd;
    int32_t *states;
    float *melpow;
    uint32_t *clipmax;
    uint8_t *rake_raw;
    double *out_f0; uint8_t *out_voiced; double *out_vprob; float *out_rms;
    uint8_t *out_rake; float *out_sdb;
    int16_t *out_bin;
    float *out_colmean; int64_t out_total;
    double rake_ratio;
    int32_t rake_min_frames, rake_max_frames;
    double f0_unvoiced;
};

void launch_frame(const PassParams &p, const DevTables &t, hipStream_t s, const double *inject_d = nullptr);
bool frame_cmnd_supported(int max_period);
int frame_batch_fpw(int max_period);
int trough_row_doubles_host(int n_lags);
void launch_pyin_obs(const PassParams &p, const DevTables &t, hipStream_t s);
void launch_inject_obs(const PassParams &p, const double *src_obs, const double *src_unv, hipStream_t s);
int pyin_obs_waves(const PassParams &p);
hipError_t launch_viterbi(const PassParams &p, const DevTables &t, const double *host_lt_band, hipStream_t s);
hipError_t launch_viterbi_split(const PassParams &p, const DevTables &t, const double *host_lt_band, const int32_t *seg_order, int n_spec,
                                const int32_t *lock_order, int n_lock, hipStream_t s, hipStream_t aux = nullptr, hipEvent_t *ev = nullptr);
hipError_t launch_viterbi_split_spec(const PassParams &p, const DevTables &t, const double *host_lt_band, const int32_t *seg_order, int n_spec, hipStream_t s);
bool viterbi_split_applies(const PassParams &p, const DevTables &t);
hipError_t viterbi_verify_fetch(long long *dst, bool reset);
int viterbi_tube_record_ints();
int viterbi_kernel_choice(const PassParams &p, const DevTables &t);
bool viterbi_band_applies(const PassParams &p, const DevTables &t);
void launch_chunk_signal(uint32_t *flag, uint32_t gen, hipStream_t s);
void launch_decode(const PassParams &p, const DevTables &t, hipStream_t s);
void launch_finite_check(const float *pcm, int64_t n, unsigned long long *first_bad, hipStream_t s);
void launch_finalize_mel(const PassParams &p, const DevTables &t, hipStream_t s);
void launch_rake_columns(const PassParams &p, bool from_power, hipStream_t s);
void launch_rake_from_db(const float *sdb, int n_mels, int64_t F, double ratio, int min_frames, int max_frames,
                         uint8_t *raw, uint8_t *out, hipStream_t s);
void launch_stream_advance(StreamCtl *ctl, const float *staging, int n_push, float *pcm, int hop, hipStream_t s);
void launch_stream_gather(const StreamCtl *ctl, const float *rms, const double *vprob, const int32_t *live, void *result,
                          hipStream_t s);
hipError_t launch_stream_commit(const StreamCtl *ctl, int64_t frames_done, StreamCommitCtl *cc, const uint16_t *ptr,
                                const double *vstate, int n_bins, int16_t *bins, void *result, hipStream_t s);
hipError_t obs_debug_fetch(long long *dst);
hipError_t frame_debug_fetch(long long *dst);
hipError_t viterbi_debug_fetch(long long *dst, bool reset);
hipError_t viterbi_span_fetch(long long *dst);
hipError_t frame_set_lds_limits(), obs_set_lds_limits(), viterbi_set_lds_limits();
inline hipError_t configure_lds_limits() {
    hipError_t e = frame_set_lds_limits();
    if (e == hipSuccess) e = obs_set_lds_limits();
    return e == hipSuccess ? viterbi_set_lds_limits() : e;
}

}
```

spectrogram-midi_amd/csrc/obs.hip:

```cpp
#include "kernels.h"
#include "frame_walk.h"
#include "pass_geometry.h"
#include "wave_ops.h"

#include <algorithm>
#include <cfloat>
#include <cmath>
#include <type_traits>

namespace aegis {

constexpr int kKMax = 512;
constexpr int kMaxRounds = 8;

#define AEGIS_OBS_LDS_LAYOUT(nl, B, mp, MAX)                                \
    const int KM = (nl) / 2 + 2;                                            \
    const int YN = (MAX(nl, B) + 1) & ~1;                                   \
    const int DN = ((mp) + 1 + 32 + 1) & ~1;                                \
    const int UN = (MAX(DN, 2 * KM + (4 * KM + 7) / 8) + 1) & ~1;           \
    const int TN = (2 * (KM + 1) + 101 + 1) & ~1;
#if defined(AEGIS_ABLATE) && (AEGIS_ABLATE & 256)
__device__ long long g_obs_dbg[16];
#define OBS_TICK(k) { const long long now__ = clock64(); oacc[k] += now__ - olast; olast = now__; }
#else
#define OBS_TICK(k)
#endif
__global__ __launch_bounds__(512, 4) void pyin_obs_kernel(PassParams p, DevTables tb, int frames_per_wave) {
    extern __shared__ __align__(16) unsigned char osm[];
    const int nl = p.n_lags, B = p.n_bins;
    AEGIS_OBS_LDS_LAYOUT(nl, B, p.max_period, max)
    const int lane = threadIdx.x & 63;
    const int wid = __builtin_amdgcn_readfirstlane((int)(threadIdx.x >> 6)), nwaves = (int)(blockDim.x >> 6);
    double *bfact = reinterpret_cast<double *>(osm);
    double *bexp = bfact + (KM + 1);
    double *bcum = bexp + (KM + 1);
    double *y = bfact + TN + (size_t)wid * (YN + UN);
    double *row = y;
    double *dd = y + YN;
    double *th = dd;
    double *tp = th + KM;
    int16_t *ti = reinterpret_cast<int16_t *>(tp + KM);
    int16_t *tbin = ti + KM;
    __shared__ double beta_s[104];

#if defined(AEGIS_ABLATE) && (AEGIS_ABLATE & 256)
    long long oacc[12] = {0, 0, 0, 0, 0, 0, 0, 0, 0, 0, 0, 0}, olast = clock64();
#endif
    for (int i = threadIdx.x; i < 100; i += blockDim.x) beta_s[i] = tb.beta_probs[i];
    for (int i = threadIdx.x; i <= KM; i += blockDim.x) { bfact[i] = tb.boltz_fact[i]; bexp[i] = tb.boltz_exp[i]; }
    for (int i = threadIdx.x; i <= 100; i += blockDim.x) bcum[i] = tb.beta_cumsum[i];
    __syncthreads();

    int64_t f = 0, fo = 0, sel_end = 0;
    int Kn = -1;
    const int64_t n_sel = geo_n_sel(p);
    for (int it = 0; it < frames_per_wave; ++it) {
    const int64_t fsel = ((int64_t)blockIdx.x * nwaves + wid) * frames_per_wave + it;
    if (fsel >= n_sel) break;
    if (it > 0 && fsel < sel_end) { ++f; ++fo; }
    else {
        int c;
        int64_t t;
        map_frame(p, fsel, c, t, f);
        fo = out_index(p, c, t);
        sel_end = p.sel_off[c + 1];
    }
    const int mp = p.max_period, minp = p.min_period;
    const double *__restrict__ dr = p.dfn + f * (int64_t)p.lag_stride;
    wave_sync();
    int K = 0;
    double *tsh = y;
    if (p.troughs) {
        const int KMt = trough_km(nl);
        if (Kn >= 0) K = Kn;
        else {
        K = __builtin_amdgcn_readfirstlane((int)__double_as_longlong(dr[0]));
        const int16_t *__restrict__ tiv = reinterpret_cast<const int16_t *>(dr + 8 + 2 * KMt);
        for (int k = lane; k < K; k += 64) {
            const double h = dr[8 + k], sh = dr[8 + KMt + k];
            const int16_t ix = tiv[k];
            th[k] = h; tsh[k] = sh; ti[k] = ix;
        }
        }
        wave_sync();
        OBS_TICK(0)
    } else {
    if (p.cmnd_in_frame) {
        for (int base = lane; base < nl; base += 320) {
            double t5[5];
#pragma unroll
            for (int u = 0; u < 5; ++u) t5[u] = dr[minp + min(base + 64 * u, nl - 1)];
#pragma unroll
            for (int u = 0; u < 5; ++u) if (base + 64 * u < nl) y[base + 64 * u] = t5[u];
        }
        wave_sync();
        OBS_TICK(0)
    } else {
    for (int base = lane; base <= mp; base += 320) {
        double t5[5];
#pragma unroll
        for (int u = 0; u < 5; ++u) t5[u] = dr[min(base + 64 * u, mp)];
#pragma unroll
        for (int u = 0; u < 5; ++u) if (base + 64 * u <= mp) dd[base + 64 * u] = t5[u];
    }
    wave_sync();
    OBS_TICK(0)
    if (lane == 0) {
        double cs = dd[1];
        if (minp <= 1) y[1 - minp] = cs;
        int tau = 2;
        constexpr int GL = 8;
        double2 ra[GL / 2], rb[GL / 2];
        auto request = [&](double2 (&r)[GL / 2], int t0) {
#pragma unroll
            for (int i = 0; i < GL / 2; ++i) r[i] = *reinterpret_cast<const double2 *>(dd + t0 + 2 * i);
        };
        auto group = [&](auto all_tag, double2 (&cur)[GL / 2], double2 (&nxt)[GL / 2], int t0) {
            constexpr bool ALL = decltype(all_tag)::value;
            request(nxt, t0 + GL);
            double *yo = y + (t0 - minp);
#pragma unroll
            for (int i = 0; i < GL / 2; ++i) {
                cs = cs + cur[i].x; if (ALL || t0 + 2 * i >= minp) yo[2 * i] = cs;
                cs = cs + cur[i].y; if (ALL || t0 + 2 * i + 1 >= minp) yo[2 * i + 1] = cs;
            }
        };
        request(ra, tau);
        bool in_a = true;
        for (; tau < minp && tau + GL - 1 <= mp; tau += GL, in_a = !in_a) {
            if (in_a) group(std::false_type{}, ra, rb, tau); else group(std::false_type{}, rb, ra, tau);
        }
        if (!in_a && tau + GL - 1 <= mp) { group(std::true_type{}, rb, ra, tau); tau += GL; }
        for (; tau + 2 * GL - 1 <= mp; tau += 2 * GL) { group(std::true_type{}, ra, rb, tau); group(std::true_type{}, rb, ra, tau + GL); }
        if (tau + GL - 1 <= mp) { group(std::true_type{}, ra, rb, tau); tau += GL; }
        for (; tau <= mp; ++tau) { cs = cs + dd[tau]; if (tau >= minp) y[tau - minp] = cs; }
    }
    wave_sync();
    OBS_TICK(1)
    for (int i = lane; i < nl; i += 64) {
        const int tau = i + minp;
        y[i] = dd[tau] / (y[i] / (double)tau + DBL_MIN);
    }
    if (p.yin != nullptr) {
        wave_sync();
        double *__restrict__ yo = p.yin + f * (int64_t)p.yin_stride;
        for (int i = lane; i < nl; i += 64) yo[i] = y[i];
    }
    wave_sync();
    }

    OBS_TICK(2)
    const int CH = (nl + 63) >> 6;
    unsigned mask = 0;
    int cnt = 0;
    for (int r = 0; r < CH; ++r) {
        const int i = lane * CH + r;
        if (i < nl) {
            const double yi = y[i];
            bool tr;
            if (i == 0) tr = yi < y[1];
            else if (i == nl - 1) tr = yi < y[i - 1];
            else tr = (yi < y[i - 1]) && (yi <= y[i + 1]);
            if (tr) { mask |= 1u << r; ++cnt; }
        }
    }
    const int incl = wave_incl_scan(cnt, lane);
    K = __shfl(incl, 63);
    {
        int k = incl - cnt;
        for (int r = 0; r < CH; ++r)
            if (mask & (1u << r)) { const int i = lane * CH + r; th[k] = y[i]; ti[k] = (int16_t)i; ++k; }
    }
    wave_sync();
    }

    OBS_TICK(3)
    double vp = 0.0;
    unsigned segm = 0;
    const int rounds = (K + 63) >> 6;
    const bool ahead = p.troughs && it + 1 < frames_per_wave && fsel + 1 < sel_end;
    double nK = 0.0, nh[2] = {0.0, 0.0}, nsh[2] = {0.0, 0.0};
    int16_t nix[2] = {0, 0};
    auto tail = [&](auto maxr_tag) {
        constexpr int MAXR = decltype(maxr_tag)::value;
        if (K > 0) {
            int jk[MAXR];
            double acc[MAXR];
            const double blo = beta_s[lane], bhi = beta_s[min(64 + lane, 99)];
    #pragma unroll
            for (int q = 0; q < MAXR; ++q) {
                jk[q] = 101; acc[q] = 0.0;
                if (q < rounds) {
                    const int k = q * 64 + lane;
                    if (k < K) {
                        const double h = th[k];
                        int g;
                        if (!(h < 1.0)) g = 100;
                        else if (h <= 0.0) g = 0;
                        else g = (int)(h * 100.0);
                        auto thr = [](int i) { return i >= 100 ? 1.0 : (double)i * 0.01; };
                        while (g < 100 && !(h < thr(g + 1))) ++g;
                        while (g > 0 && h < thr(g)) --g;
                        jk[q] = g;
                    }
                }
            }
            OBS_TICK(4)

            constexpr bool AHEAD = MAXR == 2;
            const int blo_l = __double2loint(blo), blo_h = __double2hiint(blo), bhi_l = __double2loint(bhi), bhi_h = __double2hiint(bhi);
            unsigned long long left_lo, left_hi;
            {
                unsigned w[4] = {0u, 0u, 0u, 0u};
    #pragma unroll
                for (int q = 0; q < MAXR; ++q) {
                    const unsigned bit = jk[q] < 100 ? 1u << (jk[q] & 31) : 0u;
    #pragma unroll
                    for (int i = 0; i < 4; ++i) w[i] |= (jk[q] >> 5) == i ? bit : 0u;
                }
    #pragma unroll
                for (int i = 0; i < 4; ++i) w[i] = wave_or_u32(w[i]);
                left_lo = ((unsigned long long)w[1] << 32) | w[0];
                left_hi = ((unsigned long long)w[3] << 32) | w[2];
            }
            auto take_next = [&]() {
                const bool in_lo = left_lo != 0ull;
                const unsigned long long m = in_lo ? left_lo : left_hi, rest = m & (m - 1ull);
                const int r = m ? (in_lo ? 0 : 64) + (int)__builtin_ctzll(m) : 100;
                left_lo = in_lo ? rest : 0ull;
                left_hi = in_lo ? left_hi : rest;
                return r;
            };
            auto change = [&](int j0, int &nxt, double &fact, double (&e)[MAXR]) {
                unsigned long long M[MAXR];
                int nj = 0;
    #pragma unroll
                for (int q = 0; q < MAXR; ++q) {
                    M[q] = __ballot(jk[q] <= j0);
                    nj += __popcll(M[q]);
                }
                fact = bfact[nj];
                int before = 0;
    #pragma unroll
                for (int q = 0; q < MAXR; ++q) {
                    e[q] = bexp[before + (int)__builtin_amdgcn_mbcnt_hi((unsigned)(M[q] >> 32), __builtin_amdgcn_mbcnt_lo((unsigned)M[q], 0u))];
                    before += __popcll(M[q]);
                }
                nxt = take_next();
            };
            auto stretch = [&](const double (&prior)[MAXR], int lo_l, int lo_h, int jj, int jend, int off) {
                for (; jj < jend; ++jj) {
                    const double bj = __hiloint2double(__builtin_amdgcn_readlane(lo_h, jj - off), __builtin_amdgcn_readlane(lo_l, jj - off));
    #pragma unroll
                    for (int q = 0; q < MAXR; ++q)
                        if (MAXR == 2 || q < rounds) acc[q] = acc[q] + prior[q] * bj;
                }
            };
            int j = take_next(), nxt = 100;
            double fact = 0.0, e[MAXR];
            change(j, nxt, fact, e);
            while (j < 100) {
                double prior[MAXR];
    #pragma unroll
                for (int q = 0; q < MAXR; ++q) prior[q] = jk[q] <= j ? fact * e[q] : 0.0;
                const int j1 = nxt;
                if (AHEAD) change(j1, nxt, fact, e);
                stretch(prior, blo_l, blo_h, j, min(j1, 64), 0);
                stretch(prior, bhi_l, bhi_h, max(j, 64), j1, 64);
                if (!AHEAD) change(j1, nxt, fact, e);
                j = j1;
            }

            OBS_TICK(5)
            double bh = INFINITY;
            int bk = kKMax;
    #pragma unroll
            for (int q = 0; q < MAXR; ++q) {
                const int k = q * 64 + lane;
                if (q < rounds && k < K) { const double h = th[k]; if (h < bh) { bh = h; bk = k; } }
            }
    #pragma unroll
            for (int o = 32; o >= 1; o >>= 1) {
                const double oh = __shfl_xor(bh, o);
                const int ok = __shfl_xor(bk, o);
                if (oh < bh || (oh == bh && ok < bk)) { bh = oh; bk = ok; }
            }
    #pragma unroll
            for (int q = 0; q < MAXR; ++q) {
                if (q < rounds && q * 64 + lane == bk) {
                    const int nb = jk[q] > 100 ? 100 : jk[q];
                    acc[q] = acc[q] + 0.01 * bcum[nb];
                }
            }

    #pragma unroll
            for (int q = 0; q < MAXR; ++q) {
                const int k = q * 64 + lane;
                if (q < rounds && k < K) {
                    const double pr = acc[q];
                    int bin = -1;
                    if (pr != 0.0) {
                        const int i = ti[k];
                        double shift = 0.0;
                        if (p.troughs) shift = tsh[k];
                        else if (i > 0 && i < nl - 1) {
                            const double ym = y[i - 1], y0 = y[i], yp = y[i + 1];
                            const double a = yp + ym - 2.0 * y0;
                            const double b = (yp - ym) / 2.0;
                            if (fabs(b) < fabs(a)) shift = -b / a;
                        }
                        const double period = (double)(p.min_period + i) + shift;
                        const double f0c = (double)p.sr / period;
                        double r = rint(120.0 * log2(f0c / p.fmin));
                        r = !(r >= 0.0) ? 0.0 : (r > (double)B ? (double)B : r);
                        bin = (int)r;
                    }
                    tp[k] = pr;
                    tbin[k] = (int16_t)bin;
                }
            }
        }
        OBS_TICK(6)
        if (ahead) {
            const int KMt = trough_km(nl);
            const double *__restrict__ drn = dr + p.lag_stride;
            const int16_t *__restrict__ tivn = reinterpret_cast<const int16_t *>(drn + 8 + 2 * KMt);
            nK = drn[0];
    #pragma unroll
            for (int q = 0; q < 2; ++q) {
                const int k = min(q * 64 + lane, KMt - 1);
                nh[q] = drn[8 + k]; nsh[q] = drn[8 + KMt + k]; nix[q] = tivn[k];
            }
        }
        wave_sync();
        for (int b = lane; b < B; b += 64) row[b] = p.log_tiny;
        wave_sync();
        if (K > 0) {
            bool winq[MAXR];
            double prq[MAXR];
            unsigned lseg = 0;
            int binq[MAXR];
            unsigned long long hasm[MAXR];
    #pragma unroll
            for (int q = 0; q < MAXR; ++q) {
                const int k = q * 64 + lane;
                binq[q] = (q < rounds && k < K) ? (int)tbin[k] : -1;
                hasm[q] = __ballot(binq[q] >= 0);
            }
    #pragma unroll
            for (int q = 0; q < MAXR; ++q) {
                winq[q] = false; prq[q] = 0.0;
                const int bin = binq[q];
                if (bin >= 0 && bin < B) {
                    const unsigned long long above = lane < 63 ? hasm[q] >> (lane + 1) : 0ull;
                    int k2 = -1;
                    if (above) k2 = q * 64 + lane + (int)__ffsll((long long)above);
                    else {
    #pragma unroll
                        for (int q2 = MAXR - 1; q2 > q; --q2)
                            if (hasm[q2]) k2 = q2 * 64 + (int)__ffsll((long long)hasm[q2]) - 1;
                    }
                    const bool win = (k2 < 0) || ((int)tbin[k2 < 0 ? 0 : k2] != bin);
                    if (win) { prq[q] = tp[q * 64 + lane]; row[bin] = log(prq[q] + DBL_MIN); lseg |= 1u << (bin >> 6); }
                    winq[q] = win;
                }
            }
            double s = 0.0;
    #pragma unroll
            for (int q = MAXR - 1; q >= 0; --q) {
                if (q < rounds) {
                    unsigned long long m = __ballot(winq[q]);
                    while (m) {
                        const int l = 63 - __clzll((long long)m);
                        const double v = __hiloint2double(__builtin_amdgcn_readlane(__double2hiint(prq[q]), l),
                                                          __builtin_amdgcn_readlane(__double2loint(prq[q]), l));
                        s = s + v;
                        m &= ~(1ull << l);
                    }
                }
            }
            vp = s < 0.0 ? 0.0 : (s > 1.0 ? 1.0 : s);
            for (int sg = 0; sg * 64 < B; ++sg)
                if (__ballot((lseg >> sg) & 1u)) segm |= 1u << sg;
        }
    };
    if (rounds <= 2) tail(std::integral_constant<int, 2>{});
    else tail(std::integral_constant<int, kMaxRounds>{});
    wave_sync();
    OBS_TICK(7)
    Kn = -1;
    if (ahead) {
        __builtin_amdgcn_s_waitcnt(kWaitVmcnt0);
        Kn = __builtin_amdgcn_readfirstlane((int)__double_as_longlong(nK));
        if (Kn > 128) Kn = -1;
    #pragma unroll
        for (int q = 0; q < 2; ++q) {
            const int k = q * 64 + lane;
            if (k < Kn) { th[k] = nh[q]; ti[k] = nix[q]; }
        }
    }
    const double unv = (1.0 - vp) / (double)B;
    if (unv == 0.0) segm = 0x40000000u | ((1u << ((B + 63) >> 6)) - 1u);
    double *__restrict__ orow = p.logobs + f * (int64_t)p.obs_stride;
    for (int b = lane, sg = 0; b < B; b += 64, ++sg)
        if ((segm >> sg) & 1u) orow[b] = row[b];
    if (lane == 0) {
        p.obs_seg[f] = (int32_t)segm;
        p.logunv[f] = log(unv + DBL_MIN);
        if (p.out_vprob != nullptr) p.out_vprob[fo] = vp;
    }
    #pragma unroll
    for (int q = 0; q < 2; ++q) {
        const int k = q * 64 + lane;
        if (k < Kn) y[k] = nsh[q];
    }
    OBS_TICK(8)
    }
#if defined(AEGIS_ABLATE) && (AEGIS_ABLATE & 256)
    if (blockIdx.x == 100 && threadIdx.x == 0) { for (int k = 0; k < 9; ++k) g_obs_dbg[k] = oacc[k]; g_obs_dbg[9] = frames_per_wave; }
#endif
}
#if defined(AEGIS_ABLATE) && (AEGIS_ABLATE & 256)
hipError_t obs_debug_fetch(long long *dst) { return hipMemcpyFromSymbol(dst, HIP_SYMBOL(g_obs_dbg), sizeof(long long) * 16); }
#else
hipError_t obs_debug_fetch(long long *dst) { for (int i = 0; i < 16; ++i) dst[i] = 0; return hipSuccess; }
#endif
hipError_t obs_set_lds_limits() {
    return hipFuncSetAttribute(reinterpret_cast<const void *>(pyin_obs_kernel),
                               hipFuncAttributeMaxDynamicSharedMemorySize, 96 * 1024);
}
struct ObsLds { int TN, per_wave; };
static ObsLds pyin_obs_lds(const PassParams &p) {
    AEGIS_OBS_LDS_LAYOUT(p.n_lags, p.n_bins, p.max_period, std::max)
    return {TN, YN + UN};
}
int pyin_obs_waves(const PassParams &p) {
    const ObsLds l = pyin_obs_lds(p);
    int waves = (int)std::min<int64_t>(p.dense ? 4 : 8, p.n_sel);
    while (waves > 1 && (size_t)(l.TN + waves * l.per_wave) * 8 + 1024 > 80 * 1024) --waves;
    return waves;
}
void launch_pyin_obs(const PassParams &p, const DevTables &t, hipStream_t s) {
    if (p.n_sel == 0) return;
    const ObsLds l = pyin_obs_lds(p);
    const int waves = pyin_obs_waves(p);
    const int fpw = p.n_sel >= 4096 ? (p.dense ? 8 : 4) : 1;
    const size_t lds = (size_t)(l.TN + waves * l.per_wave) * 8;
    const int64_t per_wg = (int64_t)waves * fpw;
    hipLaunchKernelGGL(pyin_obs_kernel, dim3((unsigned)((p.n_sel + per_wg - 1) / per_wg)), dim3(64 * waves), lds, s, p, t, fpw);
}
__global__ __launch_bounds__(256) void inject_obs_kernel(PassParams p, const double *__restrict__ src_obs, const double *__restrict__ src_unv) {
    const int lane = threadIdx.x & 63, B = p.n_bins, nseg = (B + 63) >> 6;
    const int64_t fs = (int64_t)blockIdx.x * 4 + (threadIdx.x >> 6);
    if (fs >= geo_n_sel(p)) return;
    int c;
    int64_t t, f;
    map_frame(p, fs, c, t, f);
    const int64_t fo = out_index(p, c, t);
    const double *__restrict__ row = src_obs + fo * (int64_t)B;
    const double unv = src_unv[fo];
    unsigned segm = 0;
    for (int sg = 0; sg < nseg; ++sg) {
        const int b = sg * 64 + lane;
        if (__ballot(b < B && row[b] != p.log_tiny)) segm |= 1u << sg;
    }
    if (unv == p.log_tiny) segm = 0x40000000u | ((1u << nseg) - 1u);
    double *__restrict__ orow = p.logobs + f * (int64_t)p.obs_stride;
    for (int b = lane, sg = 0; b < B; b += 64, ++sg)
        if ((segm >> sg) & 1u) orow[b] = row[b];
    if (lane == 0) {
        p.obs_seg[f] = (int32_t)segm;
        p.logunv[f] = unv;
    }
}
void launch_inject_obs(const PassParams &p, const double *src_obs, const double *src_unv, hipStream_t s) {
    if (p.n_sel == 0) return;
    hipLaunchKernelGGL(inject_obs_kernel, dim3((unsigned)((p.n_sel + 3) / 4)), dim3(256), 0, s, p, src_obs, src_unv);
}

}
```

spectrogram-midi_amd/csrc/tables.cpp:

```cpp
#include "tables.h"

#include <cfloat>
#include <cmath>

namespace aegis {

double np_pairwise_sum(const double *a, int64_t n) {
    if (n < 8) {
        double res = 0.0;
        for (int64_t i = 0; i < n; ++i) res += a[i];
        return res;
    }
    if (n <= 128) {
        double r[8];
        for (int k = 0; k < 8; ++k) r[k] = a[k];
        int64_t i;
        for (i = 8; i < n - (n % 8); i += 8)
            for (int k = 0; k < 8; ++k) r[k] += a[i + k];
        double res = ((r[0] + r[1]) + (r[2] + r[3])) + ((r[4] + r[5]) + (r[6] + r[7]));
        for (; i < n; ++i) res += a[i];
        return res;
    }
    int64_t n2 = n / 2;
    n2 -= n2 % 8;
// ... 45 lines not shown
    bank.w.clear();
    for (int i = 0; i < n_mels; ++i) {
        int lo = -1, hi = -1;
        for (int k = 0; k < n_bins_fft; ++k)
            if (bank.dense[(size_t)i * n_bins_fft + k] != 0.0f) { if (lo < 0) lo = k; hi = k; }
        bank.off[i] = (int32_t)bank.w.size();
        if (lo >= 0) {
            bank.start[i] = lo; bank.len[i] = hi - lo + 1;
            for (int k = lo; k <= hi; ++k) bank.w.push_back(bank.dense[(size_t)i * n_bins_fft + k]);
        }
    }
}

bool Tables::set_pyin_init(int mode) {
    if (mode != 0 && mode != 1) return false;
    pyin_init = mode;
    if (mode == 0) {
        log_pinit[0] = std::log(0.0 + DBL_MIN);
        log_pinit[1] = std::log(1.0 / n_bins + DBL_MIN);
    } else {
        log_pinit[0] = log_pinit[1] = std::log(1.0 / (2 * n_bins) + DBL_MIN);
    }
    return true;
}

std::string Tables::build(int sr_, int hop_, int n_fft_, int n_mels_, double fmin_, double fmax_) {
    sr = sr_; hop = hop_; n_fft = n_fft_; n_mels = n_mels_; fmin = fmin_; fmax = fmax_;
    if (n_fft != kFrameLength) return "only n_fft=2048 is built (the reference's value, aegis_engine.py:17)";
    if (sr <= 0 || hop <= 0 || n_mels <= 0 || n_mels > 128) return "bad sample_rate/hop_length/n_mels";
    if (!(fmin > 0) || !(fmax > fmin) || fmax > sr / 2.0) return "bad fmin/fmax";

    min_period = (int)std::floor(sr / fmax);
    max_period = std::min((int)std::ceil(sr / fmin), kFrameLength - kWinLength - 1);
    n_lags = max_period - min_period + 1;
    if (min_period < 1 || n_lags < 3) return "fmin/fmax leave fewer than 3 lags";
    const int bps = (int)std::ceil(1.0 / 0.1);
    n_bins = (int)std::floor(12 * bps * std::log2(fmax / fmin)) + 1;
    if (n_bins < 2 || 2 * n_bins > 1024) return "pitch grid needs 2..512 bins (one thread per HMM state)";
    const int max_semitones = (int)std::nearbyint(35.92 * 12 * hop / sr);
    width = max_semitones * bps + 1;
    half_width = width / 2;
    n_cls = width;
    if (width < 3 || n_bins <= 2 * half_width + 1) return "transition width does not fit the pitch grid";
    log_tiny = std::log(0.0 + DBL_MIN);
    set_pyin_init(0);

    {
        std::vector<double> fac = np_linspace(-M_PI, M_PI, n_fft + 1);
        hann.resize(n_fft);
        for (int i = 0; i < n_fft; ++i) {
            double w = 0.0;
            w += 0.5 * std::cos(0 * fac[i]);
            w += 0.5 * std::cos(1 * fac[i]);
            hann[i] = w;
        }
    }

    {
        MelBank bank;
        build_mel_bank(sr, n_fft, n_mels, sr / 2.0, bank);
        mel_dense = std::move(bank.dense);
        mel_start = std::move(bank.start); mel_len = std::move(bank.len); mel_off = std::move(bank.off);
        mel_w = std::move(bank.w);
    }

    {
        mel_chunk_bin.clear(); mel_chunk_w.clear(); mel_band_chunk.assign(n_mels + 1, 0);
        for (int i = 0; i < n_mels; ++i) {
            mel_band_chunk[i] = (int32_t)mel_chunk_bin.size();
            for (int o = 0; o < mel_len[i]; o += 16) {
                mel_chunk_bin.push_back(mel_start[i] + o);
                for (int q = 0; q < 16; ++q) mel_chunk_w.push_back(o + q < mel_len[i] ? mel_w[mel_off[i] + o + q] : 0.0f);
            }
        }
        mel_band_chunk[n_mels] = (int32_t)mel_chunk_bin.size();
        if (mel_chunk_bin.size() > 256) return "mel filterbank needs more than 256 chunks of 16 bins";
    }

    {
        thresholds = np_linspace(0.0, 1.0, kNThresholds + 1);
        std::vector<double> cdf(kNThresholds + 1);
        for (int i = 0; i <= kNThresholds; ++i) {
            const long double x = (long double)thresholds[i];
            cdf[i] = (double)(1.0L - powl(1.0L - x, 18.0L) * (1.0L + 18.0L * x));
        }
        cdf[0] = 0.0; cdf[kNThresholds] = 1.0;
        beta_probs.resize(kNThresholds);
        for (int i = 0; i < kNThresholds; ++i) beta_probs[i] = cdf[i + 1] - cdf[i];
        beta_cumsum.resize(kNThresholds + 1);
        for (int n = 0; n <= kNThresholds; ++n) beta_cumsum[n] = np_pairwise_sum(beta_probs.data(), n);
        beta_suffix.assign(kNThresholds + 1, 0.0);
        for (int n = kNThresholds - 1; n >= 0; --n) beta_suffix[n] = beta_suffix[n + 1] + beta_probs[n];
        const int nb = n_lags / 2 + 2;
        boltz_fact.assign(nb + 1, 0.0); boltz_exp.assign(nb + 1, 0.0);
        const double lam = 2.0;
        for (int N = 0; N <= nb; ++N) {
            boltz_fact[N] = N == 0 ? 0.0 : (1 - std::exp(-lam)) / (1 - std::exp(-lam * N));
            boltz_exp[N] = std::exp(-lam * N);
        }
    }

    {
        const int B = n_bins, W = width, H = half_width;
        std::vector<double> tri(W);
        for (int n = 1; n <= (W + 1) / 2; ++n) {
            const double w = 2.0 * n / (W + 1.0);
            tri[n - 1] = w; tri[W - n] = w;
        }
        const double p_stay = 1.0 - 0.01;
        const double sw[2][2] = {{p_stay, (1.0 - p_stay) / 1}, {(1.0 - p_stay) / 1, p_stay}};
        log_trans_band.assign((size_t)4 * n_cls * W, log_tiny);
        std::vector<double> row(B);
        for (int c = 0; c < n_cls; ++c) {
            const int b = c < H ? c : (c == H ? B / 2 : B - 1 - 2 * H + c);
            for (int j = 0; j < B; ++j) {
                const int dd = j - b + H;
                row[j] = (dd >= 0 && dd < W) ? tri[dd] : 0.0;
            }
            const double Z = 0.0 + np_pairwise_sum(row.data(), B);
            for (int dd = 0; dd < W; ++dd) {
                const int j = b + dd - H;
                if (j < 0 || j >= B) continue;
                const double loc = row[j] / Z;
                for (int v = 0; v < 2; ++v)
                    for (int v2 = 0; v2 < 2; ++v2)
                        log_trans_band[((size_t)(v * 2 + v2) * n_cls + c) * W + dd] =
                            std::log(sw[v][v2] * loc + DBL_MIN);
            }
        }
        log_trans_pack.clear();
        if (n_cls == W) {
            bool sym = true;
            const size_t blk = (size_t)n_cls * W;
            for (size_t i = 0; i < blk && sym; ++i)
                sym = log_trans_band[i] == log_trans_band[3 * blk + i] && log_trans_band[blk + i] == log_trans_band[2 * blk + i];
            if (sym) {
                const int NP = 3 * H * H + 3 * H + 2;
                log_trans_pack.assign((size_t)2 * NP, log_tiny);
                for (int q = 0; q < 2; ++q) {
                    const double *src = log_trans_band.data() + (size_t)q * blk;
                    double *dst = log_trans_pack.data() + (size_t)q * NP;
                    int o = 1;
                    for (int e = 0; e < H; ++e)
                        for (int dd = H - e; dd < W; ++dd) dst[o++] = src[(size_t)e * W + dd];
                    for (int dd = 0; dd < W; ++dd) dst[o++] = src[(size_t)H * W + dd];
                    for (int e = 0; e < H; ++e)
                        for (int dd = 0; dd <= 2 * H - 1 - e; ++dd) dst[o++] = src[(size_t)(H + 1 + e) * W + dd];
                    if (o != NP) { log_trans_pack.clear(); break; }
                }
            }
        }
        freqs.resize(B);
        for (int i = 0; i < B; ++i) freqs[i] = fmin * std::pow(2.0, (double)i / (12 * bps));
    }

    twiddle.resize((size_t)2 * n_fft);
    for (int m = 0; m < n_fft; ++m) {
        const long double ang = -2.0L * 3.14159265358979323846264338327950288L * m / n_fft;
        twiddle[2 * m] = (double)cosl(ang);
        twiddle[2 * m + 1] = (double)sinl(ang);
    }
    return "";
}

}
```

spectrogram-midi_amd/csrc/tables.h:

```cpp
#pragma once
#include <cstdint>
#include <string>
#include <vector>

namespace aegis {

constexpr int kFrameLength = 2048;
constexpr int kWinLength = 1024;
constexpr int kNThresholds = 100;

struct Tables {
    int sr = 44100, hop = 512, n_fft = 2048, n_mels = 128;
    double fmin = 0, fmax = 0;
    int min_period = 0, max_period = 0, n_lags = 0;
    int n_bins = 0;
    int half_width = 0;
    int width = 0;
    int n_cls = 0;
    double log_tiny = 0;
    double log_pinit[2] = {0, 0};
    int pyin_init = 0;
    std::vector<double> hann;
    std::vector<float> mel_dense;
    std::vector<int32_t> mel_start;
    std::vector<int32_t> mel_len;
    std::vector<int32_t> mel_off;
    std::vector<float> mel_w;
    std::vector<int32_t> mel_chunk_bin;
    std::vector<float> mel_chunk_w;
    std::vector<int32_t> mel_band_chunk;
    std::vector<double> thresholds;
    std::vector<double> beta_probs;
    std::vector<double> beta_cumsum;
    std::vector<double> beta_suffix;
    std::vector<double> boltz_fact;
    std::vector<double> boltz_exp;
    std::vector<double> log_trans_band;
    std::vector<double> log_trans_pack;
    std::vector<double> freqs;
    std::vector<double> twiddle;

    std::string build(int sr, int hop, int n_fft, int n_mels, double fmin, double fmax);
    bool set_pyin_init(int mode);
};

struct MelBank {
    int n_mels = 0, n_bins = 0;
    std::vector<float> dense;
    std::vector<int32_t> start, len, off;
    std::vector<float> w;
};
void build_mel_bank(int sr, int n_fft, int n_mels, double fmax, MelBank &bank);

double np_pairwise_sum(const double *a, int64_t n);

}
```

Baseline: 311,700.

## Replace f64 log2 pitch binning with fp32 guess plus edge-table verification

The pYIN observation kernel computed each candidate's pitch bin with a double-precision log2 and rint. It now makes a fast fp32 guess with hardware log/rcp and checks it against a precomputed table of period bin edges held in LDS. Only candidates the guard band rejects fall back to the exact f64 path, in a rarely taken per-wave loop. The change also drops the while loops in threshold indexing and merges the per-winner log with the unvoiced log into one masked pass. It costs more LDS per block and adds a debug entry point and env toggle. Bit-exactness depends on the guard-band test.

Measured after the change: 316,900 (median of 6 runs). +1.7%, better.

```diff
diff --git a/include/aegis_hip.h b/include/aegis_hip.h
--- a/include/aegis_hip.h
+++ b/include/aegis_hip.h
@@ -277,6 +277,9 @@
 int aegis_debug_rake_columns(aegis_handle *h, const float *mel_power, int64_t n_rows, int32_t n_mels, float clip_max,
                              double ratio, int32_t from_power, uint8_t *flags_out);
 
+int aegis_debug_pitch_bins(aegis_handle *h, const double *periods, int64_t n, int16_t *bin_table, int16_t *bin_exact,
+                           uint8_t *fell_through);
+
 int aegis_debug_set_observations(aegis_handle *h, const double *logobs, const double *logunv, int64_t F);
 
 int aegis_debug_set_difference(aegis_handle *h, const double *d, int64_t F);
diff --git a/spectrogram-midi_amd/_abi.py b/spectrogram-midi_amd/_abi.py
--- a/spectrogram-midi_amd/_abi.py
+++ b/spectrogram-midi_amd/_abi.py
@@ -150,6 +150,7 @@
     "aegis_get_param": (_I64, [_P, _S]),
     "aegis_debug_fetch": (_I64, [_P, _S, _P, _I64]),
     "aegis_debug_rake_columns": (C.c_int, [_P, _P, _I64, _I32, _F32, _F64, _I32, _P]),
+    "aegis_debug_pitch_bins": (C.c_int, [_P, _P, _I64, _P, _P, _P]),
     "aegis_debug_set_observations": (C.c_int, [_P, _P, _P, _I64]),
     "aegis_debug_set_difference": (C.c_int, [_P, _P, _I64]),
     "aegis_debug_plan": (_I64, [_P, _PI64, _I32, _I32, _I32, _I32, _P, _I64]),
diff --git a/spectrogram-midi_amd/_lib.py b/spectrogram-midi_amd/_lib.py
--- a/spectrogram-midi_amd/_lib.py
+++ b/spectrogram-midi_amd/_lib.py
@@ -18,7 +18,7 @@
 
 
 _TABLE_DTYPES = {"mel_dense": np.float32}
-_DEBUG_DTYPES = {"persistent_fallbacks": np.int64, "obs_cycles": np.int64, "cqt_cycles": np.int64, "viterbi_cycles": np.int64, "viterbi_spans": np.int64, "split_verify": np.int64, "split_flags": np.int64, "seg_lock": np.int64, "frame_cycles": np.int64, "states": np.int32, "melpow": np.float32, "rake_raw": np.uint8,
+_DEBUG_DTYPES = {"persistent_fallbacks": np.int64, "obs_cycles": np.int64, "cqt_cycles": np.int64, "viterbi_cycles": np.int64, "viterbi_spans": np.int64, "split_verify": np.int64, "split_flags": np.int64, "seg_lock": np.int64, "frame_cycles": np.int64, "states": np.int32, "obs_seg": np.int32, "melpow": np.float32, "rake_raw": np.uint8,
                  "tuning_pitch": np.float32, "tuning_mag": np.float32, "tuning_median": np.float32, "tuning_peak_off": np.int64}
 
 
@@ -111,6 +111,12 @@
         self._check(self.lib.aegis_debug_rake_columns(self._h, rows.ctypes.data, rows.shape[0], rows.shape[1], float(clip_max),
                                                       float(ratio), int(bool(from_power)), out.ctypes.data))
         return out.astype(bool)
+
+    def pitch_bins(self, periods):
+        per = np.ascontiguousarray(periods, dtype=np.float64).ravel()
+        table, exact, fell = np.empty(len(per), np.int16), np.empty(len(per), np.int16), np.empty(len(per), np.uint8)
+        self._check(self.lib.aegis_debug_pitch_bins(self._h, per.ctypes.data, len(per), table.ctypes.data, exact.ctypes.data, fell.ctypes.data))
+        return table, exact, fell.astype(bool)
 
     def set_observations(self, logobs, logunv=None):
         fn = self.lib.aegis_debug_set_observations
diff --git a/spectrogram-midi_amd/csrc/aegis_api.hip b/spectrogram-midi_amd/csrc/aegis_api.hip
--- a/spectrogram-midi_amd/csrc/aegis_api.hip
+++ b/spectrogram-midi_amd/csrc/aegis_api.hip
@@ -4,6 +4,7 @@
 #include <cmath>
 #include <numeric>
 
+#include "bin_decide.h"
 #include "pcm.h"
 
 using namespace aegis;
@@ -19,7 +20,7 @@
     p.min_period = t.min_period; p.max_period = t.max_period; p.n_lags = t.n_lags;
     p.n_bins = t.n_bins; p.half_width = t.half_width; p.width = t.width; p.n_cls = t.n_cls;
     p.f0_unvoiced = NAN;
-    p.fmin = t.fmin; p.log_tiny = t.log_tiny; p.log_pinit_v = t.log_pinit[0]; p.log_pinit_u = t.log_pinit[1];
+    p.fmin = t.fmin; p.bin_scale = bin_guess_scale(t.sr, t.fmin); p.log_tiny = t.log_tiny; p.log_pinit_v = t.log_pinit[0]; p.log_pinit_u = t.log_pinit[1];
     const RakeBounds rb = rake_frame_bounds(t);
     p.rake_min_frames = rb.min_frames; p.rake_max_frames = rb.max_frames;
     return p;
@@ -287,7 +288,7 @@
     p.n_clips = nc; p.n_frames = m.fp;
     p.dfn = static_cast<double *>(w.dfn.p); p.lag_stride = h->lag_stride;
     p.yin = (py && h->debug_stages) ? static_cast<double *>(w.yin.p) : nullptr; p.yin_stride = h->yin_stride;
-    p.cmnd_in_frame = cmnd_in_frame(h); p.troughs = troughs_in_frame(h);
+    p.cmnd_in_frame = cmnd_in_frame(h); p.troughs = troughs_in_frame(h); p.bin_table = h->bin_table_off ? 0 : 1;
     p.logobs = static_cast<double *>(w.logobs.p); p.obs_stride = h->obs_stride;
     p.logunv = static_cast<double *>(w.logunv.p);
     p.obs_seg = static_cast<int32_t *>(w.obs_seg.p);
diff --git a/spectrogram-midi_amd/csrc/aegis_handle.hip b/spectrogram-midi_amd/csrc/aegis_handle.hip
--- a/spectrogram-midi_amd/csrc/aegis_handle.hip
+++ b/spectrogram-midi_amd/csrc/aegis_handle.hip
@@ -157,6 +157,7 @@
     if (const char *e = std::getenv("AEGIS_DEBUG_STAGES")) h->debug_stages = (e[0] == '1');
     if (const char *e = std::getenv("AEGIS_CMND_IN_FRAME")) h->cmnd_off = (e[0] == '0');
     if (const char *e = std::getenv("AEGIS_TROUGHS_IN_FRAME")) h->troughs_off = (e[0] == '0');
+    if (const char *e = std::getenv("AEGIS_OBS_BIN_TABLE")) h->bin_table_off = (e[0] == '0');
     if (const char *e = std::getenv("AEGIS_CQT_BANKS")) { const int v = std::atoi(e); if (v >= 1 && v <= 32) h->cqt_bank_cap = v; }
     h->tuning_edges.resize(kTunCells + 1);
     tuning_edges(h->tuning_edges.data());
@@ -214,6 +215,7 @@
     CRT(upload_table(h, t.log_trans_band, &h->dt.lt_band));
     if (!t.log_trans_pack.empty()) CRT(upload_table(h, t.log_trans_pack, &h->dt.lt_pack));
     CRT(upload_table(h, t.freqs, &h->dt.freqs));
+    CRT(upload_table(h, t.bin_edges, &h->dt.bin_edges));
     {
         const double *tw = nullptr;
         CRT(upload_table(h, t.twiddle, &tw));
@@ -432,6 +434,7 @@
     else if (n == "log_trans_band") setd(t.log_trans_band);
     else if (n == "log_trans_pack") setd(t.log_trans_pack);
     else if (n == "freqs") setd(t.freqs);
+    else if (n == "bin_edges") setd(t.bin_edges);
     else if (n == "twiddle") setd(t.twiddle);
     else if (n == "tuning_edges") setd(h->tuning_edges);
     else if (n == "mel_dense") { src = t.mel_dense.data(); count = (int64_t)t.mel_dense.size(); esz = 4; }
@@ -539,6 +542,7 @@
         return count;
     }
     else if (n == "logunv") { src = lw.logunv.p; count = F; }
+    else if (n == "obs_seg") { src = lw.obs_seg.p; count = F; esz = 4; }
     else if (n == "states") { src = lw.states.p; count = F; esz = 4; }
     else if (n == "melpow") { src = lw.melpow.p; count = F * h->tab.n_mels; esz = 4; }
     else if (n == "rake_raw") { src = lw.rake_raw.p; count = F; esz = 1; }
@@ -633,6 +637,31 @@
     } catch (...) { return abi_fail(h); }
 }
 
+int aegis_debug_pitch_bins(aegis_handle *h, const double *periods, int64_t n, int16_t *bin_table, int16_t *bin_exact, uint8_t *fell_through) {
+    try {
+    if (!h) return AEGIS_ERR_INVALID;
+    if (n < 0 || (n > 0 && (!periods || !bin_table || !bin_exact || !fell_through))) { h->err = "bad argument"; return AEGIS_ERR_INVALID; }
+    if (n == 0) return AEGIS_OK;
+    DEVICE_ONLY(h);
+    std::lock_guard<std::mutex> lock(h->mu);
+    HIPCHK(h, hipSetDevice(h->device));
+    int rc;
+    if ((rc = ensure(h, h->dbg_bins, (size_t)n * 13)) != AEGIS_OK) return rc;
+    hipStream_t s = h->stream;
+    double *d_per = static_cast<double *>(h->dbg_bins.p);
+    int16_t *d_fast = reinterpret_cast<int16_t *>(d_per + n), *d_exact = d_fast + n;
+    uint8_t *d_fell = reinterpret_cast<uint8_t *>(d_exact + n);
+    HIPCHK(h, hipMemcpyAsync(d_per, periods, (size_t)n * 8, hipMemcpyHostToDevice, s));
+    launch_pitch_bins(base_params(h->tab), h->dt, d_per, n, d_fast, d_exact, d_fell, s);
+    HIPCHK(h, hipGetLastError());
+    HIPCHK(h, hipMemcpyAsync(bin_table, d_fast, (size_t)n * 2, hipMemcpyDeviceToHost, s));
+    HIPCHK(h, hipMemcpyAsync(bin_exact, d_exact, (size_t)n * 2, hipMemcpyDeviceToHost, s));
+    HIPCHK(h, hipMemcpyAsync(fell_through, d_fell, (size_t)n, hipMemcpyDeviceToHost, s));
+    HIPCHK(h, hipStreamSynchronize(s));
+    return AEGIS_OK;
+    } catch (...) { return abi_fail(h); }
+}
+
 int aegis_debug_set_observations(aegis_handle *h, const double *logobs, const double *logunv, int64_t F) {
     try {
     if (!h) return AEGIS_ERR_INVALID;
diff --git a/spectrogram-midi_amd/csrc/aegis_internal.h b/spectrogram-midi_amd/csrc/aegis_internal.h
--- a/spectrogram-midi_amd/csrc/aegis_internal.h
+++ b/spectrogram-midi_amd/csrc/aegis_internal.h
@@ -31,6 +31,7 @@
     hipStream_t stream = nullptr;
     hipStream_t stream2 = nullptr;
     bool troughs_off = false;
+    bool bin_table_off = false;
     bool cmnd_off = false;
     bool debug_stages = false;
     hipStream_t stream4 = nullptr;
@@ -53,7 +54,7 @@
         DevBuf sample_off, sample_len, out_off, frame_off, order, sel_off, vstate, chunk_lo, chunk_flag, clip_tb;
         DevBuf seg64, seg32, seg_col, seg_map, seg_i32, colhist, colG, colkg, clip_flag, flag_order, tube_buf, tube_at, tube_count;
     } work[2];
-    DevBuf vstats, rk_raw, abort_flag, finite_flag;
+    DevBuf vstats, rk_raw, abort_flag, finite_flag, dbg_bins;
     struct Inject { bool armed = false; int64_t F = 0; DevBuf obs, unv; } inject;
     struct InjectD { bool armed = false; int64_t F = 0; DevBuf d; } inject_d;
     uint32_t chunk_gen = 0;
diff --git a/spectrogram-midi_amd/csrc/aegis_stream.hip b/spectrogram-midi_amd/csrc/aegis_stream.hip
--- a/spectrogram-midi_amd/csrc/aegis_stream.hip
+++ b/spectrogram-midi_amd/csrc/aegis_stream.hip
@@ -19,7 +19,7 @@
     p.n_clips = 1;
     p.dfn = static_cast<double *>(st->dfn.p); p.lag_stride = h->lag_stride;
     p.yin = nullptr; p.yin_stride = h->yin_stride;
-    p.cmnd_in_frame = cmnd_in_frame(h); p.troughs = troughs_in_frame(h);
+    p.cmnd_in_frame = cmnd_in_frame(h); p.troughs = troughs_in_frame(h); p.bin_table = h->bin_table_off ? 0 : 1;
     p.logobs = static_cast<double *>(st->logobs.p); p.obs_stride = h->obs_stride;
     p.logunv = static_cast<double *>(st->logunv.p);
     p.obs_seg = static_cast<int32_t *>(st->obs_seg.p);
diff --git a/spectrogram-midi_amd/csrc/bin_decide.h b/spectrogram-midi_amd/csrc/bin_decide.h
--- /dev/null
+++ b/spectrogram-midi_amd/csrc/bin_decide.h
@@ -0,0 +1,74 @@
+#pragma once
+#include <cmath>
+
+#if defined(__HIPCC__) || defined(__CUDACC__)
+#define BIN_HD __host__ __device__ inline
+#else
+#define BIN_HD inline
+#endif
+
+namespace aegis {
+
+constexpr double kBinGuard = 9.31322574615478515625e-10;
+
+BIN_HD double bin_thr(int i) { return i >= 100 ? 1.0 : (double)i * 0.01; }
+
+BIN_HD int threshold_index_loops(double h) {
+    int g;
+    if (!(h < 1.0)) g = 100;
+    else if (h <= 0.0) g = 0;
+    else g = (int)(h * 100.0);
+    while (g < 100 && !(h < bin_thr(g + 1))) ++g;
+    while (g > 0 && h < bin_thr(g)) --g;
+    return g;
+}
+BIN_HD int threshold_index(double h) {
+    int g;
+    if (!(h < 1.0)) g = 100;
+    else if (h <= 0.0) g = 0;
+    else g = (int)(h * 100.0);
+    const bool up = g < 100 && !(h < bin_thr(g + 1)), down = g > 0 && h < bin_thr(g);
+    return g + (up ? 1 : (down ? -1 : 0));
+}
+
+BIN_HD int bin_exact(double period, int sr, double fmin, int B) {
+    const double f0c = (double)sr / period;
+    double r = rint(120.0 * log2(f0c / fmin));
+    r = !(r >= 0.0) ? 0.0 : (r > (double)B ? (double)B : r);
+    return (int)r;
+}
+
+BIN_HD float bin_guess_scale(int sr, double fmin) { return (float)((double)sr / fmin); }
+
+BIN_HD int bin_guess(double period, float scale, int B) {
+#if defined(__HIP_DEVICE_COMPILE__)
+    const float x = 120.0f * __builtin_amdgcn_logf(scale * __builtin_amdgcn_rcpf((float)period));
+#else
+    const float x = 120.0f * log2f(scale * (1.0f / (float)period));
+#endif
+    const int g = (int)fminf(fmaxf(rintf(x), 0.0f), 1024.0f);
+    return g < B ? g : B;
+}
+
+BIN_HD bool bin_accept(double period, int g, const double *E, int B) {
+    const double hi = g == 0 ? INFINITY : E[g] * (1.0 - kBinGuard);
+    const double lo = g == B ? 0.0 : E[g + 1] * (1.0 + kBinGuard);
+    return period < hi && period > lo;
+}
+BIN_HD int bin_first(double period, float scale, const double *E, int B) {
+    const int g = bin_guess(period, scale, B);
+    return bin_accept(period, g, E, B) ? g : -1;
+}
+
+BIN_HD int bin_fast(double period, float scale, const double *E, int B, bool *retried) {
+    *retried = false;
+    if (!(period > 0.0) || !(period < INFINITY)) return -1;
+    const int g = bin_guess(period, scale, B);
+    if (bin_accept(period, g, E, B)) return g;
+    *retried = true;
+    const int n = (g > 0 && !(period < E[g] * (1.0 - kBinGuard))) ? g - 1 : g + 1;
+    if (n <= B && bin_accept(period, n, E, B)) return n;
+    return -1;
+}
+
+}
diff --git a/spectrogram-midi_amd/csrc/kernels.h b/spectrogram-midi_amd/csrc/kernels.h
--- a/spectrogram-midi_amd/csrc/kernels.h
+++ b/spectrogram-midi_amd/csrc/kernels.h
@@ -26,6 +26,7 @@
     const double *lt_band;
     const double *lt_pack;
     const double *freqs;
+    const double *bin_edges;
     const double2 *twiddle;
 };
 
@@ -49,6 +50,7 @@
     int32_t min_period, max_period, n_lags;
     int32_t n_bins, half_width, width, n_cls;
     double fmin;
+    float bin_scale;
     double log_tiny;
     double log_pinit_v, log_pinit_u;
     uint32_t stages;
@@ -105,6 +107,7 @@
     int32_t hybrid_step;
     double *dfn;   int32_t lag_stride;
     int32_t cmnd_in_frame;
+    int32_t bin_table;
     int32_t troughs;
     double *yin;   int32_t yin_stride;
     double *logobs; int32_t obs_stride;
@@ -133,6 +136,7 @@
 int trough_row_doubles_host(int n_lags);
 void launch_pyin_obs(const PassParams &p, const DevTables &t, hipStream_t s);
 void launch_inject_obs(const PassParams &p, const double *src_obs, const double *src_unv, hipStream_t s);
+void launch_pitch_bins(const PassParams &p, const DevTables &t, const double *periods, int64_t n, int16_t *fast, int16_t *exact, uint8_t *fell, hipStream_t s);
 int pyin_obs_waves(const PassParams &p);
 hipError_t launch_viterbi(const PassParams &p, const DevTables &t, const double *host_lt_band, hipStream_t s);
 hipError_t launch_viterbi_split(const PassParams &p, const DevTables &t, const double *host_lt_band, const int32_t *seg_order, int n_spec,
diff --git a/spectrogram-midi_amd/csrc/obs.hip b/spectrogram-midi_amd/csrc/obs.hip
--- a/spectrogram-midi_amd/csrc/obs.hip
+++ b/spectrogram-midi_amd/csrc/obs.hip
@@ -1,4 +1,5 @@
 #include "kernels.h"
+#include "bin_decide.h"
 #include "frame_walk.h"
 #include "pass_geometry.h"
 #include "wave_ops.h"
@@ -18,9 +19,11 @@
     const int YN = (MAX(nl, B) + 1) & ~1;                                   \
     const int DN = ((mp) + 1 + 32 + 1) & ~1;                                \
     const int UN = (MAX(DN, 2 * KM + (4 * KM + 7) / 8) + 1) & ~1;           \
-    const int TN = (2 * (KM + 1) + 101 + 1) & ~1;
+    const int TN = (2 * (KM + 1) + 101 + (B) + 2 + 1) & ~1;
+#if defined(AEGIS_ABLATE) && (AEGIS_ABLATE & (256 | 1024))
+__device__ long long g_obs_dbg[16];
+#endif
 #if defined(AEGIS_ABLATE) && (AEGIS_ABLATE & 256)
-__device__ long long g_obs_dbg[16];
 #define OBS_TICK(k) { const long long now__ = clock64(); oacc[k] += now__ - olast; olast = now__; }
 #else
 #define OBS_TICK(k)
@@ -34,6 +37,7 @@
     double *bfact = reinterpret_cast<double *>(osm);
     double *bexp = bfact + (KM + 1);
     double *bcum = bexp + (KM + 1);
+    double *bedge = bcum + 101;
     double *y = bfact + TN + (size_t)wid * (YN + UN);
     double *row = y;
     double *dd = y + YN;
@@ -49,6 +53,7 @@
     for (int i = threadIdx.x; i < 100; i += blockDim.x) beta_s[i] = tb.beta_probs[i];
     for (int i = threadIdx.x; i <= KM; i += blockDim.x) { bfact[i] = tb.boltz_fact[i]; bexp[i] = tb.boltz_exp[i]; }
     for (int i = threadIdx.x; i <= 100; i += blockDim.x) bcum[i] = tb.beta_cumsum[i];
+    for (int i = threadIdx.x; i < B + 2; i += blockDim.x) bedge[i] = tb.bin_edges[i];
     __syncthreads();
 
     int64_t f = 0, fo = 0, sel_end = 0;
@@ -175,7 +180,8 @@
     }
 
     OBS_TICK(3)
-    double vp = 0.0;
+    double vp = 0.0, unv = 0.0, logu = 0.0;
+    bool have_logu = false;
     unsigned segm = 0;
     const int rounds = (K + 63) >> 6;
     const bool ahead = p.troughs && it + 1 < frames_per_wave && fsel + 1 < sel_end;
@@ -193,15 +199,7 @@
                 if (q < rounds) {
                     const int k = q * 64 + lane;
                     if (k < K) {
-                        const double h = th[k];
-                        int g;
-                        if (!(h < 1.0)) g = 100;
-                        else if (h <= 0.0) g = 0;
-                        else g = (int)(h * 100.0);
-                        auto thr = [](int i) { return i >= 100 ? 1.0 : (double)i * 0.01; };
-                        while (g < 100 && !(h < thr(g + 1))) ++g;
-                        while (g > 0 && h < thr(g)) --g;
-                        jk[q] = g;
+                        jk[q] = threshold_index(th[k]);
                     }
                 }
             }
@@ -293,6 +291,19 @@
                 }
             }
 
+            auto period_of = [&](int k) {
+                const int i = ti[k];
+                double shift = 0.0;
+                if (p.troughs) shift = tsh[k];
+                else if (i > 0 && i < nl - 1) {
+                    const double ym = y[i - 1], y0 = y[i], yp = y[i + 1];
+                    const double a = yp + ym - 2.0 * y0;
+                    const double b = (yp - ym) / 2.0;
+                    if (fabs(b) < fabs(a)) shift = -b / a;
+                }
+                return (double)(p.min_period + i) + shift;
+            };
+            bool unsure = false;
     #pragma unroll
             for (int q = 0; q < MAXR; ++q) {
                 const int k = q * 64 + lane;
@@ -300,25 +311,48 @@
                     const double pr = acc[q];
                     int bin = -1;
                     if (pr != 0.0) {
-                        const int i = ti[k];
-                        double shift = 0.0;
-                        if (p.troughs) shift = tsh[k];
-                        else if (i > 0 && i < nl - 1) {
-                            const double ym = y[i - 1], y0 = y[i], yp = y[i + 1];
-                            const double a = yp + ym - 2.0 * y0;
-                            const double b = (yp - ym) / 2.0;
-                            if (fabs(b) < fabs(a)) shift = -b / a;
-                        }
-                        const double period = (double)(p.min_period + i) + shift;
-                        const double f0c = (double)p.sr / period;
-                        double r = rint(120.0 * log2(f0c / p.fmin));
-                        r = !(r >= 0.0) ? 0.0 : (r > (double)B ? (double)B : r);
-                        bin = (int)r;
+                        bin = bin_first(period_of(k), p.bin_scale, bedge, B);
+                        if (bin < 0 || !p.bin_table) { bin = -2; unsure = true; }
                     }
                     tp[k] = pr;
                     tbin[k] = (int16_t)bin;
                 }
             }
+            const unsigned long long unsure_m = __ballot(unsure);
+            if (__builtin_expect(unsure_m != 0ull, 0)) {
+    #if defined(AEGIS_ABLATE) && (AEGIS_ABLATE & 1024)
+                int n_exact = 0;
+    #endif
+                int sr_c = p.sr, B_c = B;
+                double fmin_c = p.fmin;
+                asm volatile("" : "+s"(sr_c), "+s"(B_c), "+s"(fmin_c));
+    #pragma unroll 1
+                for (int q = 0; q < rounds; ++q) {
+                    const int k = q * 64 + lane;
+                    if (k < K && tbin[k] == -2) {
+                        const double period = period_of(k);
+                        bool retried;
+                        int bin = p.bin_table ? bin_fast(period, p.bin_scale, bedge, B_c, &retried) : -1;
+                        if (bin < 0) {
+                            bin = bin_exact(period, sr_c, fmin_c, B_c);
+    #if defined(AEGIS_ABLATE) && (AEGIS_ABLATE & 1024)
+                            ++n_exact;
+    #endif
+                        }
+                        tbin[k] = (int16_t)bin;
+                    }
+                }
+    #if defined(AEGIS_ABLATE) && (AEGIS_ABLATE & 1024)
+                if (n_exact) atomicAdd(reinterpret_cast<unsigned long long *>(&g_obs_dbg[11]), (unsigned long long)n_exact);
+    #endif
+            }
+    #if defined(AEGIS_ABLATE) && (AEGIS_ABLATE & 1024)
+            {
+                int n_bins_asked = 0;
+                for (int q = 0; q < rounds; ++q) { const int k = q * 64 + lane; if (k < K && tbin[k] >= 0) ++n_bins_asked; }
+                if (n_bins_asked) atomicAdd(reinterpret_cast<unsigned long long *>(&g_obs_dbg[10]), (unsigned long long)n_bins_asked);
+            }
+    #endif
         }
         OBS_TICK(6)
         if (ahead) {
@@ -335,9 +369,11 @@
         wave_sync();
         for (int b = lane; b < B; b += 64) row[b] = p.log_tiny;
         wave_sync();
+        bool winq[MAXR];
+        double prq[MAXR];
+    #pragma unroll
+        for (int q = 0; q < MAXR; ++q) { winq[q] = false; prq[q] = 0.0; }
         if (K > 0) {
-            bool winq[MAXR];
-            double prq[MAXR];
             unsigned lseg = 0;
             int binq[MAXR];
             unsigned long long hasm[MAXR];
@@ -349,7 +385,6 @@
             }
     #pragma unroll
             for (int q = 0; q < MAXR; ++q) {
-                winq[q] = false; prq[q] = 0.0;
                 const int bin = binq[q];
                 if (bin >= 0 && bin < B) {
                     const unsigned long long above = lane < 63 ? hasm[q] >> (lane + 1) : 0ull;
@@ -361,7 +396,7 @@
                             if (hasm[q2]) k2 = q2 * 64 + (int)__ffsll((long long)hasm[q2]) - 1;
                     }
                     const bool win = (k2 < 0) || ((int)tbin[k2 < 0 ? 0 : k2] != bin);
-                    if (win) { prq[q] = tp[q * 64 + lane]; row[bin] = log(prq[q] + DBL_MIN); lseg |= 1u << (bin >> 6); }
+                    if (win) { prq[q] = tp[q * 64 + lane]; lseg |= 1u << (bin >> 6); }
                     winq[q] = win;
                 }
             }
@@ -383,14 +418,34 @@
             for (int sg = 0; sg * 64 < B; ++sg)
                 if (__ballot((lseg >> sg) & 1u)) segm |= 1u << sg;
         }
+        unv = (1.0 - vp) / (double)B;
+        if (K > 0) {
+            const double ua = unv + DBL_MIN;
+    #pragma unroll
+            for (int q = 0; q < MAXR; ++q) {
+                const bool last = q == rounds - 1;
+                if (q < rounds && (winq[q] || last)) {
+                    const double r = log(winq[q] ? prq[q] + DBL_MIN : ua);
+                    if (winq[q]) row[(int)tbin[q * 64 + lane]] = r;
+                    if (last) {
+                        const unsigned long long idle = ~__ballot(winq[q]);
+                        if (idle) {
+                            const int l = (int)__builtin_ctzll(idle);
+                            logu = __hiloint2double(__builtin_amdgcn_readlane(__double2hiint(r), l), __builtin_amdgcn_readlane(__double2loint(r), l));
+                            have_logu = true;
+                        }
+                    }
+                }
+            }
+        }
     };
     if (rounds <= 2) tail(std::integral_constant<int, 2>{});
     else tail(std::integral_constant<int, kMaxRounds>{});
     wave_sync();
     OBS_TICK(7)
     Kn = -1;
+    __builtin_amdgcn_s_waitcnt(kWaitVmcnt0);
     if (ahead) {
-        __builtin_amdgcn_s_waitcnt(kWaitVmcnt0);
         Kn = __builtin_amdgcn_readfirstlane((int)__double_as_longlong(nK));
         if (Kn > 128) Kn = -1;
     #pragma unroll
@@ -399,14 +454,14 @@
             if (k < Kn) { th[k] = nh[q]; ti[k] = nix[q]; }
         }
     }
-    const double unv = (1.0 - vp) / (double)B;
+    if (!have_logu) logu = log(unv + DBL_MIN);
     if (unv == 0.0) segm = 0x40000000u | ((1u << ((B + 63) >> 6)) - 1u);
     double *__restrict__ orow = p.logobs + f * (int64_t)p.obs_stride;
     for (int b = lane, sg = 0; b < B; b += 64, ++sg)
         if ((segm >> sg) & 1u) orow[b] = row[b];
     if (lane == 0) {
         p.obs_seg[f] = (int32_t)segm;
-        p.logunv[f] = log(unv + DBL_MIN);
+        p.logunv[f] = logu;
         if (p.out_vprob != nullptr) p.out_vprob[fo] = vp;
     }
     #pragma unroll
@@ -420,7 +475,7 @@
     if (blockIdx.x == 100 && threadIdx.x == 0) { for (int k = 0; k < 9; ++k) g_obs_dbg[k] = oacc[k]; g_obs_dbg[9] = frames_per_wave; }
 #endif
 }
-#if defined(AEGIS_ABLATE) && (AEGIS_ABLATE & 256)
+#if defined(AEGIS_ABLATE) && (AEGIS_ABLATE & (256 | 1024))
 hipError_t obs_debug_fetch(long long *dst) { return hipMemcpyFromSymbol(dst, HIP_SYMBOL(g_obs_dbg), sizeof(long long) * 16); }
 #else
 hipError_t obs_debug_fetch(long long *dst) { for (int i = 0; i < 16; ++i) dst[i] = 0; return hipSuccess; }
@@ -473,6 +528,22 @@
         p.logunv[f] = unv;
     }
 }
+__global__ __launch_bounds__(256) void pitch_bins_kernel(const double *__restrict__ periods, int64_t n, const double *__restrict__ edges, int sr,
+                                                         double fmin, float scale, int B, int16_t *__restrict__ fast, int16_t *__restrict__ exact,
+                                                         uint8_t *__restrict__ fell) {
+    const int64_t i = (int64_t)blockIdx.x * blockDim.x + threadIdx.x;
+    if (i >= n) return;
+    bool retried;
+    const int b = bin_fast(periods[i], scale, edges, B, &retried);
+    fast[i] = (int16_t)b;
+    exact[i] = (int16_t)bin_exact(periods[i], sr, fmin, B);
+    fell[i] = b < 0 ? 1 : 0;
+}
+void launch_pitch_bins(const PassParams &p, const DevTables &t, const double *periods, int64_t n, int16_t *fast, int16_t *exact, uint8_t *fell, hipStream_t s) {
+    if (n == 0) return;
+    hipLaunchKernelGGL(pitch_bins_kernel, dim3((unsigned)((n + 255) / 256)), dim3(256), 0, s, periods, n, t.bin_edges, p.sr, p.fmin, p.bin_scale,
+                       p.n_bins, fast, exact, fell);
+}
 void launch_inject_obs(const PassParams &p, const double *src_obs, const double *src_unv, hipStream_t s) {
     if (p.n_sel == 0) return;
     hipLaunchKernelGGL(inject_obs_kernel, dim3((unsigned)((p.n_sel + 3) / 4)), dim3(256), 0, s, p, src_obs, src_unv);
diff --git a/spectrogram-midi_amd/csrc/tables.cpp b/spectrogram-midi_amd/csrc/tables.cpp
--- a/spectrogram-midi_amd/csrc/tables.cpp
+++ b/spectrogram-midi_amd/csrc/tables.cpp
@@ -221,6 +221,9 @@
         }
         freqs.resize(B);
         for (int i = 0; i < B; ++i) freqs[i] = fmin * std::pow(2.0, (double)i / (12 * bps));
+        bin_edges.resize(B + 2);
+        for (int b = 0; b <= B + 1; ++b)
+            bin_edges[b] = (double)((long double)sr / ((long double)fmin * exp2l(((long double)b - 0.5L) / 120.0L)));
     }
 
     twiddle.resize((size_t)2 * n_fft);
diff --git a/spectrogram-midi_amd/csrc/tables.h b/spectrogram-midi_amd/csrc/tables.h
--- a/spectrogram-midi_amd/csrc/tables.h
+++ b/spectrogram-midi_amd/csrc/tables.h
@@ -38,6 +38,7 @@
     std::vector<double> log_trans_band;
     std::vector<double> log_trans_pack;
     std::vector<double> freqs;
+    std::vector<double> bin_edges;
     std::vector<double> twiddle;
 
     std::string build(int sr, int hop, int n_fft, int n_mels, double fmin, double fmax);
```
